# ArthurBrussee/brush

Measured on AMD Instinct MI355X. Metric: train views/sec @ 1M Gaussians, 1080p (fwd + L1/SSIM loss + bwd + Adam per view), higher is better.
Workload: dtype f32

## Files before the change

brush_amd/_ffi.py:

```python
import ctypes as C
import os

_DIR = os.path.dirname(os.path.abspath(__file__))
LIB_PATH = os.environ.get("BRUSH_HIP_LIB") or os.path.join(_DIR, "libbrush_hip.so")

FLAG_MIP = 1
FLAG_BWD_INFO = 2
FLAG_SMOOTH_CUTOFF = 4
FLAG_SLICED_LISTS = 8

fp = C.POINTER(C.c_float)
u32p = C.POINTER(C.c_uint32)


class BhCamera(C.Structure):
    _fields_ = [
        ("vm", C.c_float * 12),
        ("fx", C.c_float), ("fy", C.c_float), ("cx", C.c_float), ("cy", C.c_float),
        ("lim_pos_x", C.c_float), ("lim_pos_y", C.c_float),
        ("lim_neg_x", C.c_float), ("lim_neg_y", C.c_float),
        ("cam_pos", C.c_float * 3),
        ("img_w", C.c_uint32), ("img_h", C.c_uint32),
        ("tile_row_begin", C.c_uint32), ("tile_row_end", C.c_uint32),
        ("model", C.c_uint32), ("dist", C.c_float * 8), ("half_max_render_fov", C.c_float),
# ... 210 lines not shown
dp = C.POINTER(C.c_double)
POSE_SYMBOLS = {
    "bh_render_backward_pose_saved": (C.c_int, [C.c_void_p, C.POINTER(BhRenderOut)] + [C.c_void_p] * 9),
    "bh_train_set_pose_grad": (C.c_int, [C.c_void_p, C.c_void_p]),
    "bh_pose_twist": (C.c_int, [fp, fp, dp]),
    "bh_camera_apply_twist": (C.c_int, [C.POINTER(BhCamera), dp]),
}

EXPOSURE_SYMBOLS = {
    "bh_exposure_create": (C.c_int, [C.c_void_p, C.c_uint32, C.POINTER(C.c_void_p)]),
    "bh_exposure_destroy": (C.c_int, [C.c_void_p, C.c_void_p]),
    "bh_exposure_set_params": (C.c_int, [C.c_void_p, C.c_void_p, C.c_uint32, C.c_uint32, fp]),
    "bh_exposure_get_params": (C.c_int, [C.c_void_p, C.c_void_p, C.c_uint32, C.c_uint32, fp]),
    "bh_exposure_get_grad": (C.c_int, [C.c_void_p, C.c_void_p, C.c_uint32, C.c_uint32, fp]),
    "bh_exposure_get_state": (C.c_int, [C.c_void_p, C.c_void_p, C.c_uint32, dp, dp, u32p]),
    "bh_exposure_set_state": (C.c_int, [C.c_void_p, C.c_void_p, C.c_uint32, dp, dp, C.c_uint32]),
    "bh_exposure_set_adam": (C.c_int, [C.c_void_p, C.c_void_p, C.c_double, C.c_double, C.c_double, C.c_double]),
    "bh_exposure_apply": (C.c_int, [C.c_void_p, C.c_void_p, C.c_uint32, C.c_void_p, C.c_uint32, C.c_uint32, C.c_void_p]),
    "bh_exposure_backward": (C.c_int, [C.c_void_p, C.c_void_p, C.c_uint32, C.c_void_p, C.c_void_p, C.c_uint32, C.c_uint32, C.c_void_p, C.c_int]),
    "bh_train_set_exposure": (C.c_int, [C.c_void_p, C.c_void_p]),
}

DEPTH_LOSS_L1, DEPTH_LOSS_DISPARITY = 0, 1


class BhDepthTarget(C.Structure):
    _fields_ = [("gt", C.c_void_p), ("h", C.c_uint32), ("w", C.c_uint32), ("kind", C.c_uint32), ("weight", C.c_float),
                ("scale", C.c_float), ("offset", C.c_float)]


DEPTH_LOSS_SYMBOLS = {
    "bh_depth_loss_value_and_grad": (C.c_int, [C.c_void_p, C.c_void_p, C.POINTER(BhDepthTarget), C.c_void_p, C.c_void_p]),
    "bh_train_set_depth": (C.c_int, [C.c_void_p, C.POINTER(BhDepthTarget)]),
    "bh_eval_depth_metrics": (C.c_int, [C.c_void_p, C.c_void_p, C.POINTER(BhDepthTarget), C.c_void_p]),
}

NORMAL_ACCUMULATED, NORMAL_UNIT = 0, 1
NORMAL_SYMBOLS = {
    "bh_splat_normals": (C.c_int, [C.c_void_p, C.POINTER(BhCamera), C.c_void_p, C.c_uint64, C.c_void_p]),
    "bh_render_normal": (C.c_int, [C.c_void_p, C.POINTER(BhRenderOut), C.c_void_p, C.c_uint32, C.c_void_p]),
    "bh_render_backward_normal_saved": (C.c_int, [C.c_void_p, C.POINTER(BhRenderOut), C.c_void_p, C.c_void_p, C.c_uint32, C.c_void_p, C.c_uint32]
                                        + [C.c_void_p] * 7),
    "bh_depth_to_normal": (C.c_int, [C.c_void_p, C.POINTER(BhCamera), C.c_void_p, C.c_uint32, C.c_uint32, C.c_void_p]),
    "bh_depth_to_normal_backward": (C.c_int, [C.c_void_p, C.POINTER(BhCamera), C.c_void_p, C.c_void_p, C.c_uint32, C.c_uint32, C.c_void_p]),
}

class BhNormalTermConfig(C.Structure):
    _fields_ = [("weight", C.c_float), ("reserved", C.c_uint32 * 3)]


NORMAL_LOSS_SYMBOLS = {
    "bh_normal_consistency_value_and_grad": (C.c_int, [C.c_void_p, C.POINTER(BhCamera), C.c_void_p, C.c_void_p, C.c_void_p, C.c_uint32, C.c_uint32,
                                                       C.c_float, C.c_uint32, C.c_void_p, C.c_void_p, C.c_void_p]),
    "bh_train_set_normal": (C.c_int, [C.c_void_p, C.POINTER(BhNormalTermConfig)]),
}

DISTORTION_Z, DISTORTION_NDC = 0, 1


class BhDistortionConfig(C.Structure):
    _fields_ = [("kind", C.c_uint32), ("near_z", C.c_float), ("far_z", C.c_float), ("reserved", C.c_uint32)]


class BhDistortionTermConfig(C.Structure):
    _fields_ = [("weight", C.c_float), ("kind", C.c_uint32), ("near_z", C.c_float), ("far_z", C.c_float)]


DISTORTION_SYMBOLS = {
    "bh_render_distortion": (C.c_int, [C.c_void_p, C.POINTER(BhRenderOut), C.POINTER(BhDistortionConfig), C.c_void_p]),
    "bh_render_distortion_moments": (C.c_int, [C.c_void_p, C.POINTER(BhRenderOut), C.POINTER(BhDistortionConfig), C.c_void_p]),
    "bh_render_backward_distortion_saved": (C.c_int, [C.c_void_p, C.POINTER(BhRenderOut), C.c_void_p, C.c_void_p, C.c_uint32, C.c_void_p, C.c_uint32,
                                                      C.c_void_p, C.POINTER(BhDistortionConfig)] + [C.c_void_p] * 7),
    "bh_distortion_loss": (C.c_int, [C.c_void_p, C.c_void_p, C.c_uint32, C.c_uint32, C.c_uint32, C.c_float, C.c_void_p]),
    "bh_train_set_distortion": (C.c_int, [C.c_void_p, C.POINTER(BhDistortionTermConfig)]),
}

ABI_VERSION = 7
STRUCT_MIRRORS = (BhCamera, BhRenderOut, BhLossConfig, BhTrainConfig, BhTrainState, BhTrainBatch, BhTrainStats, BhRefineConfig, BhRefineStats, BhPlyInfo)

_lib = None
_lib_th = None
TEST_HOOKS_LIB_PATH = os.path.join(_DIR, "libbrush_hip_testhooks.so")
TEST_HOOK_SYMBOLS = {"bh_debug_fill_train_scratch": (C.c_int, [C.c_void_p, C.c_uint32]),
                     "bh_debug_split_counts": (C.c_int, [C.c_void_p, C.POINTER(C.c_uint32)])}


class BrushHipError(RuntimeError):
    pass


def _bind(path, symbols):
    if not os.path.exists(path):
        raise BrushHipError(
            "%s not found: build it with `python -c 'import __graft_entry__ as g; g.build()'` "
            "(hipcc --offload-arch=gfx950). There is no CPU fallback." % path)
    lib = C.CDLL(path)
    for name, (res, args) in symbols.items():
        fn = getattr(lib, name)
        fn.restype = res
        fn.argtypes = args
    if lib.bh_abi_version() != ABI_VERSION:
        raise BrushHipError("%s speaks ABI %d, this binding ABI %d" % (path, lib.bh_abi_version(), ABI_VERSION))
    for i, mirror in enumerate(STRUCT_MIRRORS):
        if lib.bh_struct_size(i) != C.sizeof(mirror):
            raise BrushHipError("%s: sizeof(%s) is %d in the library, %d in this binding" % (path, mirror.__name__, lib.bh_struct_size(i), C.sizeof(mirror)))
    return lib


def load():
    global _lib
    if _lib is None:
        _lib = _bind(LIB_PATH, dict(SYMBOLS, **LPIPS_SYMBOLS, **COMPRESSED_PLY_SYMBOLS, **IMAGE_SYMBOLS, **DEPTH_SYMBOLS, **POSE_SYMBOLS, **EXPOSURE_SYMBOLS, **DEPTH_LOSS_SYMBOLS, **NORMAL_SYMBOLS, **NORMAL_LOSS_SYMBOLS, **DISTORTION_SYMBOLS))
    return _lib


def load_test_hooks():
    global _lib_th
    if _lib_th is None:
        _lib_th = _bind(TEST_HOOKS_LIB_PATH, dict(SYMBOLS, **LPIPS_SYMBOLS, **COMPRESSED_PLY_SYMBOLS, **IMAGE_SYMBOLS, **DEPTH_SYMBOLS, **POSE_SYMBOLS, **EXPOSURE_SYMBOLS, **DEPTH_LOSS_SYMBOLS, **NORMAL_SYMBOLS, **NORMAL_LOSS_SYMBOLS, **DISTORTION_SYMBOLS,
                                                   **TEST_HOOK_SYMBOLS))
    return _lib_th
```

brush_amd/csrc/api.hip:

```cpp
#include <cmath>
#include <cstdlib>
#include <cstdio>
#include <algorithm>
#include <cstring>
#include <new>

#include "context.h"
#include "device_rng.h"

namespace bh {

int launch_image_loss_fused(bh_ctx* ctx, const float* img_hwc4, const uint32_t* gt, uint32_t h, uint32_t w, const BhLossConfig& cfg,
                            bool alpha_match, float dl_rgb, float dl_alpha, float* loss_out, float* v_output, float* loss_host = nullptr,
                            uint32_t* started_host = nullptr, uint32_t started_tag = 0);
int launch_image_loss_fused_window(bh_ctx* ctx, const float* img_hwc4, const uint32_t* gt, uint32_t h, uint32_t w, const BhLossConfig& cfg,
                                   bool alpha_match, float dl_rgb, float dl_alpha, uint32_t tile_y0, uint32_t tile_y1, float* loss_out,
                                   float* v_output, float* loss_host = nullptr, uint32_t* started_host = nullptr, uint32_t started_tag = 0);

__global__ __launch_bounds__(256) void zero_two_kernel(float4* __restrict__ a, size_t na, float4* __restrict__ b, size_t nb) {
    const size_t stride = (size_t)gridDim.x * 256;
    const float4 z = make_float4(0.0f, 0.0f, 0.0f, 0.0f);
    for (size_t i = (size_t)blockIdx.x * 256 + threadIdx.x; i < na + nb; i += stride) {
        if (i < na) a[i] = z;
        else b[i - na] = z;
    }
}

int set_error(bh_ctx* ctx, int code, const std::string& msg) {
    if (ctx) ctx->last_error = msg;
    return code;
}

int check_hip(bh_ctx* ctx, hipError_t e, const char* what) {
    if (e == hipSuccess) return 0;
    std::string m = std::string(what) + ": " + hipGetErrorString(e);
    (void)hipGetLastError();
    return set_error(ctx, e == hipErrorOutOfMemory ? BH_ERR_OOM : BH_ERR_HIP, m);
}

static inline void cpu_relax() {
#if defined(__x86_64__) || defined(__i386__)
    __builtin_ia32_pause();
#elif defined(__aarch64__)
    __asm__ __volatile__("yield");
#endif
}
int wait_host_tag(bh_ctx* ctx, const volatile uint32_t* word, uint32_t want, const char* what) {
    for (uint64_t it = 1; it < (1ull << 21); ++it) {
        if (*word == want) return 0;
        if ((it & 0x3FFFull) == 0ull) {
            const hipError_t q = hipStreamQuery(ctx->stream);
            if (q == hipSuccess) break;
            if (q != hipErrorNotReady) return check_hip(ctx, q, what);
        }
        cpu_relax();
    }
    if (*word == want) return 0;
    BH_HIP(ctx, hipEventRecord(ctx->readback_ev, ctx->stream));
    BH_HIP(ctx, hipEventSynchronize(ctx->readback_ev));
    if (*word == want) return 0;
    return set_error(ctx, BH_ERR_STATE, std::string(what) + ": the kernel that signals the host never stored its tag");
}

void* ensure(bh_ctx* ctx, Slot s, size_t bytes) {
    Buffer& b = ctx->slots[s];
    if (bytes == 0) bytes = 16;
    if (b.cap >= bytes) return b.ptr;
    if (b.ptr) {
        (void)hipStreamSynchronize(ctx->stream);
        (void)hipFree(b.ptr);
        b.ptr = nullptr;
        b.cap = 0;
    }
    {
        int best = -1;
        for (size_t i = 0; i < ctx->pool.size(); ++i)
            if (ctx->pool[i].cap >= bytes && ctx->pool[i].cap <= 2 * bytes + 4096 && (best < 0 || ctx->pool[i].cap < ctx->pool[(size_t)best].cap)) best = (int)i;
        if (best >= 0) {
            b = ctx->pool[(size_t)best];
            ctx->pool.erase(ctx->pool.begin() + best);
            return b.ptr;
        }
    }
    size_t cap = bytes + bytes / 4;
    cap = (cap + 255) & ~(size_t)255;
    void* p = nullptr;
    hipError_t e = hipMalloc(&p, cap);
    if (e != hipSuccess) {
        (void)hipGetLastError();
        cap = (bytes + 255) & ~(size_t)255;
        e = hipMalloc(&p, cap);
    }
    if (e != hipSuccess) {
        char msg[160];
        snprintf(msg, sizeof msg, "hipMalloc(%zu bytes) for scratch slot %d failed: %s", cap, (int)s, hipGetErrorString(e));
        (void)hipGetLastError();
        set_error(ctx, BH_ERR_OOM, msg);
        return nullptr;
    }
    b.ptr = p;
// ... 193 lines not shown
        BH_TRY(finish_far_slice(ctx, nullptr));
    }
    BH_HIP(ctx, hipStreamSynchronize(ctx->stream));
    deliver_pending_loss(ctx);
    return 0;
}

int bh_profile_enable(bh_ctx* ctx, int on) {
    if (!ctx) return BH_ERR_INVALID_ARG;
    ctx->prof.level = on < 0 ? 0 : (on > 2 ? 1 : on);
    return 0;
}

int bh_profile_fetch(bh_ctx* ctx, const char** names, float* ms, uint32_t* calls, int cap) {
    if (!ctx) return BH_ERR_INVALID_ARG;
    prof_resolve(ctx);
    Profiler& p = ctx->prof;
    const int n = p.count < cap ? p.count : cap;
    for (int i = 0; i < n; ++i) {
        names[i] = p.names[i];
        ms[i] = p.ms[i];
        calls[i] = p.calls[i];
    }
    p.count = 0;
    return n;
}

namespace {
bool parse_u32(const char* v, uint32_t lo, uint32_t hi, uint32_t* out) {
    if (!v || !*v) return false;
    char* end = nullptr;
    const unsigned long long x = strtoull(v, &end, 10);
    if (*end != '\0' || x < lo || x > hi) return false;
    *out = (uint32_t)x;
    return true;
}
bool parse_flag(const char* v, bool* out) {
    uint32_t x = 0;
    if (!parse_u32(v, 0, 1, &x)) return false;
    *out = x != 0;
    return true;
}
struct Option { const char* name; const char* help; bool (*apply)(bh_ctx* c, const char* v); };
const Option kOptions[] = {
    {"cut_min_pairs", "u32: a view whose last frame had fewer pairs keeps complete lists (= bh_set_list_cut_threshold)",
     [](bh_ctx* c, const char* v) { return parse_u32(v, 0, 0xFFFFFFFFu, &c->cut_min_pairs); }},
    {"cut_margin_pct", "0..10000: base margin behind a tile's last useful splat, % of its depth rank (default 150)",
     [](bh_ctx* c, const char* v) { return parse_u32(v, 0, 10000, &c->knob_cut_margin_pct); }},
    {"cut_margin_fixed", "0|1: the margin is cut_margin_pct for every frame instead of adaptive",
     [](bh_ctx* c, const char* v) { return parse_flag(v, &c->knob_fixed_margin); }},
    {"cut_ctrl", "up:down:floor:gap_exp — the margin controller's constants (default 1.5:0.998:0.5:0.3333)", [](bh_ctx* c, const char* v) {
        float a = 0, b = 0, d = 0, e = 0;
        if (sscanf(v, "%f:%f:%f:%f", &a, &b, &d, &e) != 4 || !(a >= 1.0f && b > 0.0f && b <= 1.0f && d > 0.0f && e >= 0.0f && e <= 1.0f)) return false;
        c->ctrl_up = a; c->ctrl_down = b; c->ctrl_floor = d; c->ctrl_gap_exp = e;
        return true;
    }},
    {"cut_sort_all", "0|1: with per-tile cuts, still depth-sort every visible splat",
     [](bh_ctx* c, const char* v) { return parse_flag(v, &c->knob_cut_sort_all); }},
    {"auto_exact_share", "0..1: a view whose last cut frame listed more than this share of its pairs renders complete lists (default 0.9; 0 = never)", [](bh_ctx* c, const char* v) {
        char* end = nullptr;
        const float x = strtof(v, &end);
        if (end == v || *end != '\0' || !(x >= 0.0f && x <= 1.0f)) return false;
        c->auto_exact_share = x;
        return true;
    }},
    {"no_view_hash", "0|1: frames without a view id share ONE table instead of being keyed by their camera",
     [](bh_ctx* c, const char* v) { return parse_flag(v, &c->knob_no_view_hash); }},
    {"k16_order", "0 index order | 1 by the view's last per-tile work | 2 dealt: the forward blend's tile order",
     [](bh_ctx* c, const char* v) { return parse_u32(v, 0, 2, &c->knob_k16_order); }},
    {"band_mode", "0|1: XCD bands of the blend kernels — contiguous eighths of the tile range, or dealt in chunks of 8 adjacent tiles (default 1)",
     [](bh_ctx* c, const char* v) { return parse_u32(v, 0, 1, &c->knob_band_mode); }},
    {"k16_waves", "0..8: forward blend: resident one-wave tiles per SIMD (0 = 8 = all resident at once; fewer: the lighter tiles are dispatched as the heavier ones finish)",
     [](bh_ctx* c, const char* v) { return parse_u32(v, 0, 8, &c->knob_k16_waves); }},
    {"k16_split", "0..1000: forward blend: a tile whose forecast work is at least max(256, k16_split / 100 x its band's mean) is blended by four quadrant waves (default 250; 0: no tile is split)",
     [](bh_ctx* c, const char* v) { return parse_u32(v, 0, 1000, &c->knob_k16_split); }},
    {"k16_split_of_max", "0..100: ... and at least this many percent of its band's heaviest tile (default 45)",
     [](bh_ctx* c, const char* v) { return parse_u32(v, 0, 100, &c->knob_k16_split_of_max); }},
    {"k16_split_min", "1..1023: a tile below this many blended splats (forecast) is never split (default 256)",
     [](bh_ctx* c, const char* v) { return parse_u32(v, 1, 1023, &c->knob_k16_split_min); }},
    {"k5_exact_spw", "16|32|64: splats per wave of the list builder for complete lists",
     [](bh_ctx* c, const char* v) { uint32_t u = 0; if (!parse_u32(v, 16, 64, &u) || !(u == 16 || u == 32 || u == 64)) return false; c->knob_k5_exact_spw = u; return true; }},
    {"bwd_jobs", "0|1: the blend backward works on checkpointed 128-entry segments of the tiles' lists (default 1) or on whole tiles",
     [](bh_ctx* c, const char* v) { return parse_flag(v, &c->knob_bwd_jobs); }},
    {"bwd_wide_rows", "0|1: the blend backward addresses the gradient accumulator in 64 bits, as it does by itself from 2^32 bytes of accumulator on (default 0)",
     [](bh_ctx* c, const char* v) { return parse_flag(v, &c->knob_bwd_wide_rows); }},
    {"no_lpt", "0|1: the blend backward takes its tiles in index order",
     [](bh_ctx* c, const char* v) { return parse_flag(v, &c->knob_no_lpt); }},
    {"lpt_classes", "log|linear: work classes of the backward's longest-first tile order — two per octave of blended splats, or 1/64 of the mean list length wide",
     [](bh_ctx* c, const char* v) { const std::string w(v); if (w == "log") { c->knob_lpt_linear = false; return true; } if (w == "linear") { c->knob_lpt_linear = true; return true; } return false; }},
    {"generic_depth_sort", "0|1: depth order by the generic radix sort + scan instead of the fused split sort",
     [](bh_ctx* c, const char* v) { return parse_flag(v, &c->knob_generic_depth_sort); }},
    {"dsort_splitters", "0|1: the fused depth sort splits at the 254 depth quantiles of the view's previous frame (default 1) or always linearly over the frame's key range",
     [](bh_ctx* c, const char* v) { return parse_flag(v, &c->knob_dsort_splitters); }},
    {"tile_sort", "auto|bucket|lsd: the forward's tile sort (auto: bucket sort unless the view's pairs are concentrated in few tiles)",
     [](bh_ctx* c, const char* v) { const std::string w(v); if (w == "auto") { c->knob_tile_sort = 0; return true; } if (w == "bucket") { c->knob_tile_sort = 1; return true; } if (w == "lsd") { c->knob_tile_sort = 2; return true; } return false; }},
    {"spec_k5", "0|1: queue the list builder before the host has read the frame's counts (default 1; 0: behind the count readback)",
     [](bh_ctx* c, const char* v) { return parse_flag(v, &c->knob_spec_k5); }},
    {"event_waits", "0|1: the host's mid-step waits use events behind the kernels instead of polled tag words",
     [](bh_ctx* c, const char* v) { return parse_flag(v, &c->knob_event_waits); }},
    {"readback_copy", "0|1: counts and gate word reach the host through copy launches",
     [](bh_ctx* c, const char* v) { return parse_flag(v, &c->knob_readback_copy); }},
    {"force_exchange", "0|1: a one-rank communicator still walks the whole gradient-exchange path (overhead measurement)",
     [](bh_ctx* c, const char* v) { return parse_flag(v, &c->knob_force_exchange); }},
    {"zero_grads", "0|1: the single-GPU train step zero-fills its gradient span like the exchange path",
     [](bh_ctx* c, const char* v) { return parse_flag(v, &c->knob_zero_grads); }},
    {"loss_bands", "0|1: the fused loss's blocks take their tiles by XCD column bands (1) or row-major (0)",
     [](bh_ctx* c, const char* v) { return parse_u32(v, 0, 1, &c->knob_loss_bands); }},
    {"update_rows", "0|64|128|256: splats per block of the update kernel (0 = default)",
     [](bh_ctx* c, const char* v) { uint32_t u = 0; if (!parse_u32(v, 0, 256, &u) || !(u == 0 || u == 64 || u == 128 || u == 256)) return false; c->knob_update_rows = u; return true; }},
    {"no_dormant", "0|1: the update kernel fetches and updates dormant splats like everyone else",
     [](bh_ctx* c, const char* v) { return parse_flag(v, &c->knob_no_dormant); }},
    {"sort_kpt", "0|4|8|16: keys per thread of the generic radix sort (0 = default)",
     [](bh_ctx* c, const char* v) { uint32_t u = 0; if (!parse_u32(v, 0, 16, &u) || !(u == 0 || u == 4 || u == 8 || u == 16)) return false; c->knob_sort_kpt = u; return true; }},
    {"grad_allreduce", "ring|direct: the dense gradient block's collective — ncclAllReduce, or reduce-scatter + all-gather over grouped send/recv",
     [](bh_ctx* c, const char* v) { const std::string w(v); if (w == "ring") { c->knob_direct_allreduce = false; return true; } if (w == "direct") { c->knob_direct_allreduce = true; return true; } return false; }},
    {"update_sparse", "0..256: an update block with at most this many non-dormant rows fetches them in one round trip (0: never; 256: every block that may skip dormant rows; default 64 at SH degree 0, else 0)",
     [](bh_ctx* c, const char* v) { uint32_t u = 0; if (!parse_u32(v, 0, 256, &u)) return false; c->knob_update_sparse = (int)u; return true; }},
};
constexpr int kOptionCount = (int)(sizeof(kOptions) / sizeof(kOptions[0]));
}

extern "C" int bh_option_count(void) { return kOptionCount; }
extern "C" const char* bh_option_name(int i) { return i >= 0 && i < kOptionCount ? kOptions[i].name : nullptr; }
extern "C" const char* bh_option_help(int i) { return i >= 0 && i < kOptionCount ? kOptions[i].help : nullptr; }

extern "C" int bh_set_option(bh_ctx* ctx, const char* key, const char* value) {
    if (!ctx) return BH_ERR_INVALID_ARG;
    if (!key || !value) return set_error(ctx, BH_ERR_INVALID_ARG, "set_option: null key or value");
    const std::string k(key);
    for (const Option& o : kOptions) {
        if (k != o.name) continue;
        if (!o.apply(ctx, value)) return set_error(ctx, BH_ERR_INVALID_ARG, "set_option: bad value '" + std::string(value) + "' for '" + k + "'");
        return 0;
    }
    return set_error(ctx, BH_ERR_INVALID_ARG, "set_option: unknown key '" + k + "' (bh_option_name lists the keys)");
}

namespace {
struct Kb4Law {
    double k[4];
    explicit Kb4Law(const float* d) { for (int i = 0; i < 4; ++i) k[i] = d ? (double)d[i] : 0.0; }
    double value(double th) const {
        const double t2 = th * th, t3 = t2 * th, t5 = t3 * t2, t7 = t5 * t2, t9 = t7 * t2;
        return th + k[0] * t3 + k[1] * t5 + k[2] * t7 + k[3] * t9;
    }
    double slope(double th) const {
        const double t2 = th * th, t4 = t2 * t2, t6 = t4 * t2, t8 = t6 * t2;
        return 1.0 + 3.0 * k[0] * t2 + 5.0 * k[1] * t4 + 7.0 * k[2] * t6 + 9.0 * k[3] * t8;
    }
    double invert(double target) const {
        if (target <= 0.0) return 0.0;
        const double pi = 3.14159265358979323846;
        double th = target < pi - 1e-6 ? target : pi - 1e-6;
        for (int it = 0; it < 50; ++it) {
            const double fp = slope(th);
            if (std::fabs(fp) < 1e-12) break;
            double next = th - (value(th) - target) / fp;
            next = next < 0.0 ? 0.0 : (next > pi ? pi : next);
            const bool done = std::fabs(next - th) < 1e-12;
            th = next;
            if (done) break;
        }
        return th;
    }
};
struct Rt8Law {
// ... 258 lines not shown
            BH_HIP(ctx, hipMemcpyAsync(hslots, counters, counter_read_bytes, hipMemcpyDeviceToHost, ctx->stream));
            BH_HIP(ctx, hipEventRecord(ctx->readback_ev, ctx->stream));
        }
        {
            ProfScope ps(ctx, "DepthSort");
            if (fused_scan) {
                cum_early = (uint32_t*)ensure(ctx, SLOT_CUM_TILES_HIT, npad * 4);
                if (!cum_early) return BH_ERR_OOM;
                if (poll_tag && ++ctx->readback_tag == 0u) ctx->readback_tag = 1u;
                bool* spl_written = nullptr;
                uint32_t* spl = view_splitters(view, cut_active, &spl_written);
                BH_TRY(depth_sort_scan(ctx, depth_keys, counters + COUNTER_MINMAX_WORD, cut_active ? near_counts : isect_counts, n, depths_sorted, f.gfc, cum_early,
                                       sums_on_device ? counters : nullptr, ctx->host_counters + 16, ctx->readback_ev, poll_tag ? ctx->readback_tag : 0u,
                                       sums_on_device ? dev_sums : nullptr, spl, spl_written));
            } else {
                BH_TRY(radix_argsort(ctx, depth_keys, nullptr, n, 32, depths_sorted, f.gfc));
            }
        }
        if (poll_tag && ctx->knob_spec_k5 && !(want_sliced && ctx->slice_fraction > 0.0f)) {
            const size_t cap_pairs = std::min(ctx->slots[SLOT_TILE_IDS].cap, ctx->slots[SLOT_ISECT_GIDS].cap) / 4;
            if (cap_pairs >= 4096) {
                spec_projected = (float*)ensure(ctx, SLOT_PROJECTED, npad * 9 * 4);
                spec_vc = f.bwd_info ? (float4*)ensure(ctx, SLOT_V_COMBINED, npad * 10 * 4 + 16) : nullptr;
                if (!spec_projected || (f.bwd_info && !spec_vc)) return BH_ERR_OOM;
                spec_tile_ids = (uint32_t*)ctx->slots[SLOT_TILE_IDS].ptr;
                spec_isect_gids = (uint32_t*)ctx->slots[SLOT_ISECT_GIDS].ptr;
                spec_pair_cap = (uint32_t)std::min<size_t>(cap_pairs, 0xFFFFFFFEull);
                ProfScope ps(ctx, "MapGaussiansToIntersect");
                BH_TRY(launch_map_gaussians(ctx, n, f.u, f.proj_by_gid, f.gfc, spec_projected, cum_early, spec_tile_ids, spec_isect_gids, spec_vc,
                                            spec_vc ? (uint32_t)(((size_t)n * 10 + 3) / 4) : 0u, 0xFFFFFFFFu, cut_active ? slice_tab : nullptr,
                                            cut_active ? vtab : nullptr, cut_active ? depths_sorted : nullptr, dev_sums + (cut_active ? 3 : 0), spec_pair_cap));
                k5_queued = true;
            }
        }
        if (poll_tag) BH_TRY(wait_host_tag(ctx, reinterpret_cast<const volatile uint32_t*>(hslots) + HOST_SUM_WORDS - 1u, ctx->readback_tag, "count readback"));
        else BH_HIP(ctx, hipEventSynchronize(ctx->readback_ev));
        if (ctx->gate_learn) {
            ctx->gate_learn = false;
            ctx->far_direct = reinterpret_cast<const volatile uint32_t*>(ctx->host_counters)[HOST_GATE_WORD] != 0u;
        }
        unsigned long long hc[4] = {0ull, 0ull, 0ull, 0ull};
        if (sums_on_device) {
            const volatile unsigned long long* hs = hslots;
            for (uint32_t c = 0; c < COUNTER_K1_U64; ++c) hc[c] = hs[c];
        } else {
            for (uint32_t k = 0; k < COUNTER_SLOTS; ++k)
                for (uint32_t c = 0; c < COUNTER_K1_U64; ++c) hc[c] += hslots[COUNTER_K1_U64 * k + c];
        }
        if (hc[1] > 0xFFFFFFFFull) return set_error(ctx, BH_ERR_UNSUPPORTED, "more than 2^32-1 tile intersections");
        nv_true = (uint32_t)hc[0];
        f.ni = (uint32_t)hc[1];
        near_total = cut_active ? (uint32_t)hc[2] : f.ni;
        f.nv = cut_active ? (uint32_t)hc[3] : nv_true;
    } else {
        BH_HIP(ctx, hipMemsetAsync(tile_offsets, 0, ((size_t)f.num_tiles * 2 + LPT_HEADER_WORDS) * 4, ctx->stream));
        if (visible_words) BH_HIP(ctx, hipMemsetAsync(f.visible, 0, visible_words * 4, ctx->stream));
    }

    const size_t nvpad = f.nv ? f.nv : 1, nipad = f.ni ? f.ni : 1;
    f.cum = fused_scan ? cum_early : (uint32_t*)ensure(ctx, SLOT_CUM_TILES_HIT, nvpad * 4);
    f.projected = (float*)ensure(ctx, SLOT_PROJECTED, nvpad * 9 * 4);
    f.tile_ids = (uint32_t*)ensure(ctx, SLOT_TILE_IDS, nipad * 4);
    f.isect_gids = (uint32_t*)ensure(ctx, SLOT_ISECT_GIDS, nipad * 4);
    f.tile_ids_sorted = (uint32_t*)ensure(ctx, SLOT_TILE_IDS_SORTED, nipad * 4);
    f.isect_gids_sorted = (uint32_t*)ensure(ctx, SLOT_ISECT_GIDS_SORTED, nipad * 4);
    const size_t pixels = (size_t)f.u.img_w * f.u.img_h;
    void* out_img = ensure(ctx, SLOT_OUT_IMG, pixels * (f.bwd_info ? 16 : 4));
    if (!f.cum || !f.projected || !f.tile_ids || !f.isect_gids || !f.tile_ids_sorted || !f.isect_gids_sorted || !out_img)
        return BH_ERR_OOM;
    if (k5_queued && ((cut_active ? near_total : f.ni) > spec_pair_cap || f.projected != spec_projected || f.tile_ids != spec_tile_ids || f.isect_gids != spec_isect_gids))
        k5_queued = false;

    f.budget = want_sliced && f.ni > 0 ? list_budget(ctx, cut_active ? view : nullptr, near_total, f.ni) : f.ni;
    const bool sliced = f.budget < f.ni;
    const bool by_cut = cut_active && sliced;
    const uint32_t* zcut_lists = cut_active ? vtab : nullptr;
    f.slice_info = slice_tab;
    f.done_bits = slice_tab ? slice_tab + SLICE_CTRL_WORDS : nullptr;
    f.tile_offsets_far = slice_tab ? slice_tab + SLICE_CTRL_WORDS + slice_bit_words : nullptr;
    f.far_group_totals = slice_tab ? slice_tab + SLICE_CTRL_WORDS + slice_bit_words + (size_t)f.num_tiles * 2 : nullptr;
    while (f.tile_bits < 32 && (f.num_tiles >> f.tile_bits) != 0) f.tile_bits++;
    if (bwd_jobs) {
        const uint32_t listed = cut_active ? near_total : f.ni;
        const uint32_t ckpt_cap = (uint32_t)std::min<uint64_t>((uint64_t)listed / BWD_SEG + f.num_tiles + 1u, BWD_CKPT_MAX_SLOTS);
        f.rs.jobs.ckpt = (float4*)ensure(ctx, SLOT_BWD_CKPT, (size_t)ckpt_cap * 256 * sizeof(float4));
        f.rs.jobs.ckpt_cap = ckpt_cap;
        f.rs.jobs.top_cap = band_slots(f.num_tiles) + ckpt_cap;
        f.rs.jobs.top_list = (uint32_t*)ensure(ctx, SLOT_BWD_TOPLIST, (size_t)8 * f.rs.jobs.top_cap * 4);
        if (!f.rs.jobs.ckpt || !f.rs.jobs.top_list) return BH_ERR_OOM;
    }
    if (view) {
        f.rs.zcut = vtab;
        f.rs.depth_keys_sorted = depths_sorted;
        f.rs.nv = f.nv;
        f.rs.cut_active = by_cut;
        f.rs.margin_pct = cut_margin_pct(ctx, view);
        f.rs.work = vtab + (size_t)f.num_tiles;
        f.rs.order = tile_order;
        f.rs.order_mode = ctx->knob_k16_order;
        f.rs.split = tile_split;
#ifdef BH_TEST_HOOKS
        ctx->last_split = tile_split;
#endif
    }
    const uint32_t win_tiles = f.u.tile_bw * (f.u.tile_y1 - f.u.tile_y0);
    const float class_width_raw = (float)f.ni / (float)(win_tiles ? win_tiles : 1u) / 64.0f;
    f.class_width = ctx->knob_lpt_linear ? (class_width_raw < 8.0f ? 8.0f : class_width_raw) : 0.0f;
    f.lpt = (f.bwd_info && !ctx->knob_no_lpt) ? tile_offsets + (size_t)f.num_tiles * 2 : nullptr;
    f.out_f32 = f.bwd_info ? (float*)out_img : nullptr;
    f.out_u8 = f.bwd_info ? nullptr : (uint32_t*)out_img;

    bool offsets_done = false;
    if (f.nv > 0) {
        if (!fused_scan) {
            ProfScope ps(ctx, "PrefixSumGaussHits");
            BH_TRY(prefix_sum(ctx, cut_active ? near_counts : isect_counts, f.gfc, f.nv, f.cum, false));
        }
        if (f.ni == 0) {
            ProfScope ps(ctx, "ProjectVisible");
            BH_TRY(launch_project_visible(ctx, f.nv, f.proj_by_gid, f.gfc, f.projected));
        }
        if (f.ni > 0) {
            {
                ProfScope ps(ctx, "MapGaussiansToIntersect");
                float4* vc = nullptr;
                if (f.bwd_info) {
                    vc = (float4*)ensure(ctx, SLOT_V_COMBINED, (size_t)f.nv * 10 * 4 + 16);
                    if (!vc) return BH_ERR_OOM;
                }
                if (zcut_lists && near_total == 0u) {
                } else if (k5_queued && (!f.bwd_info || vc == spec_vc)) {
                    ctx->clears.k5_cleared_accum(vc != nullptr);
                } else {
                    ctx->clears.k5_cleared_accum(vc != nullptr);
                    BH_TRY(launch_map_gaussians(ctx, f.nv, f.u, f.proj_by_gid, f.gfc, f.projected, f.cum, f.tile_ids, f.isect_gids, vc, vc ? (uint32_t)(((size_t)f.nv * 10 + 3) / 4) : 0u,
                                                (sliced && !by_cut) ? f.budget : 0xFFFFFFFFu, (sliced || zcut_lists) ? f.slice_info : nullptr, zcut_lists,
                                                zcut_lists ? depths_sorted : nullptr));
                }
            }
            {
                ProfScope ps(ctx, "TileSort");
                if ((zcut_lists || !sliced) && tile_sort_supported(f.tile_bits, zcut_lists ? near_total : f.ni) && !(ctx->knob_tile_sort == 2u)) {
                    BH_TRY(tile_sort_offsets(ctx, f.tile_ids, f.isect_gids, zcut_lists ? near_total : f.ni, f.tile_bits, f.num_tiles, f.tile_ids_sorted, f.isect_gids_sorted,
                                             tile_offsets, f.ni));
                    offsets_done = true;
                } else
                if (zcut_lists) BH_TRY(radix_argsort_dev(ctx, f.tile_ids, f.isect_gids, near_total, nullptr, nullptr, nullptr, f.tile_bits, f.tile_ids_sorted, f.isect_gids_sorted, f.ni));
                else if (sliced) BH_TRY(radix_argsort_dev(ctx, f.tile_ids, f.isect_gids, f.budget, f.slice_info + 1, nullptr, nullptr, f.tile_bits, f.tile_ids_sorted, f.isect_gids_sorted, f.ni));
                else BH_TRY(radix_argsort(ctx, f.tile_ids, f.isect_gids, f.ni, f.tile_bits, f.tile_ids_sorted, f.isect_gids_sorted));
            }
        }
    }
    if (!offsets_done) {
        ProfScope ps(ctx, "GetTileOffsets");
        if (zcut_lists) BH_TRY(launch_tile_offsets(ctx, f.tile_ids_sorted, near_total, f.num_tiles, tile_offsets, true));
        else if (sliced) BH_TRY(launch_tile_offsets_dev(ctx, f.tile_ids_sorted, f.budget, f.slice_info + 1, nullptr, nullptr, f.num_tiles, tile_offsets));
        else BH_TRY(launch_tile_offsets(ctx, f.tile_ids_sorted, f.ni, f.num_tiles, tile_offsets, true));
    }
    if (!sliced) {
        ProfScope ps(ctx, "Rasterize");
        BH_TRY(launch_rasterize(ctx, f.u, f.bg, f.bwd_info, f.smooth, f.isect_gids_sorted, tile_offsets, f.projected, f.gfc, f.out_f32, f.out_u8, f.visible, f.lpt,
                                f.class_width, 0, &f.rs));
    } else {
        auto* state = (float*)ensure(ctx, SLOT_SLICE_STATE, pixels * 16);
        f.far_counts = (uint32_t*)ensure(ctx, SLOT_SLICE_COUNTS, nvpad * 4);
        f.far_block_totals = (uint32_t*)ensure(ctx, SLOT_SLICE_CUM, (nvpad / 256 + 2) * 4);
        if (!state || !f.far_counts || !f.far_block_totals) return BH_ERR_OOM;
        f.rs.done_bits = f.done_bits;
        f.rs.unsat_count = f.slice_info + 2;
        if (!ctx->knob_readback_copy) {
            f.rs.gate_host = ctx->host_counters + HOST_GATE_WORD;
            *reinterpret_cast<volatile uint32_t*>(f.rs.gate_host) = 0u;
        }
        f.rs.state = state;
        f.rs.offsets_near = tile_offsets;
        f.rs.live_bands = f.slice_info + 4;
        {
            ProfScope ps(ctx, "Rasterize");
            BH_TRY(launch_rasterize(ctx, f.u, f.bg, f.bwd_info, f.smooth, f.isect_gids_sorted, tile_offsets, f.projected, f.gfc, f.out_f32, f.out_u8, f.visible, f.lpt,
                                    f.class_width, 1, &f.rs));
        }
        FarJob& j = ctx->far_job;
        j.frame = f;
        j.by_cut = by_cut;
        j.view = by_cut ? view : nullptr;
        j.view_shared = req.view_id == 0u && ctx->knob_no_view_hash;
        if (by_cut) j.req = req;
        if (ctx->knob_readback_copy)
            BH_HIP(ctx, hipMemcpyAsync(ctx->host_counters + HOST_GATE_WORD, f.slice_info + 2, 4, hipMemcpyDeviceToHost, ctx->stream));
        if (ctx->far_direct && !by_cut) {
            BH_TRY(enqueue_far_slice(ctx, j));
            ctx->gate_learn = true;
        } else {
            if (++ctx->gate_tag == 0u) ctx->gate_tag = 1u;
            j.gate_tag = ctx->gate_tag;
            ctx->gate_signal_queued = false;
            j.gate_event_recorded = !(req.defer_decision && !ctx->knob_event_waits && !ctx->knob_readback_copy);
            if (j.gate_event_recorded) BH_HIP(ctx, hipEventRecord(ctx->gate_ev, ctx->stream));
            j.pending = true;
            if (!req.defer_decision) {
                bool again = false;
                BH_TRY(finish_far_slice(ctx, &again));
                if (by_cut && again) {
                    *out = ctx->latest.out;
                    return 0;
                }
            }
        }
    }

    BhRenderOut r{};
    r.num_visible = nv_true;
    r.num_listed_splats = f.nv;
    r.num_intersections = f.ni;
    r.num_tiles = f.num_tiles;
    r.tile_bw = f.u.tile_bw;
    r.tile_bh = f.u.tile_bh;
    r.flags = flags;
    r.out_img = f.bwd_info ? (float*)out_img : nullptr;
    r.out_img_packed = f.bwd_info ? nullptr : (uint32_t*)out_img;
    r.visible = f.bwd_info ? f.visible : nullptr;
    r.max_radius = max_radius;
    r.tile_offsets = tile_offsets;
    r.projected = f.projected;
    r.compact_gid_from_isect = f.isect_gids_sorted;
    r.tile_id_from_isect = f.tile_ids_sorted;
    r.global_from_compact_gid = f.gfc;
    r.cum_tiles_hit = f.cum;
    r.intersect_counts = isect_counts;
    r.depths_sorted = (float*)depths_sorted;
    r.tile_offsets_far = sliced ? f.tile_offsets_far : nullptr;
    r.list_budget = f.budget;
    r.generation = ++ctx->generation;
    ctx->clears.stamp(r.generation);
    *out = r;
    ForwardState& latest = ctx->latest;
    latest.out = r;
    latest.uniforms = f.u;
    latest.n = n; latest.sh_degree = sh_degree; latest.flags = flags;
    latest.bg[0] = f.bg[0]; latest.bg[1] = f.bg[1]; latest.bg[2] = f.bg[2];
    latest.lpt = f.lpt;
    latest.jobs = f.rs.jobs;
    ctx->have_forward = true;
    if (view) view_rendered(view, f.ni);
    return 0;
}

extern "C" {

int bh_set_list_slicing(bh_ctx* ctx, float near_share) {
    if (!ctx) return BH_ERR_INVALID_ARG;
    if (near_share != near_share || near_share > 1.0f) return set_error(ctx, BH_ERR_INVALID_ARG, "set_list_slicing: the near slice's share must be <= 1 (<= 0: automatic)");
    ctx->slice_fraction = near_share > 0.0f ? near_share : 0.0f;
    return 0;
}

int bh_set_list_cut_threshold(bh_ctx* ctx, uint32_t min_pairs) {
    if (!ctx) return BH_ERR_INVALID_ARG;
    ctx->cut_min_pairs = min_pairs;
    return 0;
}

int bh_set_view_id(bh_ctx* ctx, uint32_t view_id) {
    if (!ctx) return BH_ERR_INVALID_ARG;
    ctx->view_id = view_id;
    return 0;
}

int bh_forget_views(bh_ctx* ctx) {
    if (!ctx) return BH_ERR_INVALID_ARG;
    BH_HIP(ctx, hipSetDevice(ctx->device));
    if (ctx->far_job.pending) BH_TRY(finish_far_slice(ctx, nullptr));
    if (ctx->dsort_spl) { BH_HIP(ctx, hipMemsetAsync(ctx->dsort_spl, 0, DSORT_SPL_STRIDE * 4, ctx->stream)); ctx->dsort_spl_written = false; }
    if (ctx->views.empty()) return 0;
    BH_HIP(ctx, hipStreamSynchronize(ctx->stream));
    deliver_pending_loss(ctx);
    for (auto& kv : ctx->views)
        if (kv.second.zcut) (void)hipFree(kv.second.zcut);
    ctx->views.clear();
    ctx->casual_views = 0;
    for (uint64_t& k : ctx->seen_keys) k = 0ull;
    ctx->far_job.view = nullptr;
    ctx->margin_scale = 1.0f;
    return 0;
}

float bh_last_list_share(bh_ctx* ctx) { return ctx ? ctx->last_slice_share : 0.0f; }
uint32_t bh_far_slices_queued(bh_ctx* ctx) { return ctx ? ctx->far_launches : 0u; }
uint32_t bh_view_table_count(bh_ctx* ctx) { return ctx ? (uint32_t)ctx->views.size() : 0u; }

}

namespace bh {

int backward_impl(bh_ctx* ctx, const ForwardState& fs, const float* v_output, const float* transforms, const float* sh_coeffs,
                  const float* raw_opacities, float* v_transforms, float* v_sh_coeffs, float* v_raw_opacities, float* v_refine_weight,
                  size_t span_floats, bool want_refine, const DepthTerm* depth, float* v_viewmat, const NormalTerm* normal,
                  const DistortionTerm* distortion) {
    const BhRenderOut& r = fs.out;
    const uint32_t n = fs.n, nv = r.num_listed_splats, C = (fs.sh_degree + 1) * (fs.sh_degree + 1);
    const size_t nvpad = nv ? nv : 1;
    auto* v_combined = (float*)ensure(ctx, SLOT_V_COMBINED, nvpad * 10 * 4 + 16);
    if (!v_combined) return BH_ERR_OOM;
    bool row_marks = false;
    const float* scatter_v_z = nullptr;
    {
        ProfScope ps(ctx, "ZeroGradBuffers");
        const bool one_span = n > 0 && span_floats;
        const bool vc_done = ctx->clears.take_accum(r.generation);
        const GradClears::Span span = ctx->clears.take_span(r.generation);
        row_marks = span == GradClears::ROW_MARKS;
        if (row_marks && !one_span) return set_error(ctx, BH_ERR_STATE, "internal: row-marked gradients without the train step's gradient span");
        const bool span_done = one_span && span != GradClears::NONE;
        if (one_span && (span_floats & 3u) == 0 && (reinterpret_cast<uintptr_t>(v_transforms) & 15u) == 0) {
            const size_t na = vc_done ? 0 : (nvpad * 10 + 3) / 4, nb = span_done ? 0 : span_floats / 4;
            if (na + nb) {
                hipLaunchKernelGGL(zero_two_kernel, dim3(2048), dim3(256), 0, ctx->stream, reinterpret_cast<float4*>(v_combined), na,
                                   reinterpret_cast<float4*>(v_transforms), nb);
                BH_LAUNCH_CHECK(ctx, "zero_two_kernel");
            }
        } else {
            if (!vc_done) BH_HIP(ctx, hipMemsetAsync(v_combined, 0, nvpad * 10 * 4, ctx->stream));
            if (n > 0) {
                if (one_span) {
                    BH_HIP(ctx, hipMemsetAsync(v_transforms, 0, span_floats * 4, ctx->stream));
                } else {
                    BH_HIP(ctx, hipMemsetAsync(v_transforms, 0, (size_t)n * 10 * 4, ctx->stream));
                    BH_HIP(ctx, hipMemsetAsync(v_sh_coeffs, 0, (size_t)n * C * 3 * 4, ctx->stream));
                    BH_HIP(ctx, hipMemsetAsync(v_raw_opacities, 0, (size_t)n * 4, ctx->stream));
                    BH_HIP(ctx, hipMemsetAsync(v_refine_weight, 0, (size_t)n * 4, ctx->stream));
                }
            }
        }
    }
    {
        ProfScope ps(ctx, "RasterizeBackwards", true);
        if (r.num_intersections > 0 && v_output)
            BH_TRY(launch_rasterize_backward(ctx, fs.uniforms, fs.bg, fs.flags & BH_FLAG_SMOOTH_CUTOFF,
                                             r.compact_gid_from_isect, r.tile_offsets, r.projected, r.out_img, v_output, v_combined, fs.lpt,
                                             r.tile_offsets_far, want_refine, &fs.jobs, nv));
        if (depth) BH_TRY(launch_depth_backward(ctx, fs, *depth, v_combined));
        if (normal) BH_TRY(launch_normal_backward(ctx, fs, *normal, transforms, v_combined));
        if (distortion) BH_TRY(launch_distortion_backward(ctx, fs, *distortion, v_combined, depth ? (float*)ctx->slots[SLOT_DEPTH].ptr : nullptr, &scatter_v_z));
    }
    {
        ProfScope ps(ctx, "ProjectBackwards");
        BH_TRY(launch_project_backward(ctx, fs.uniforms, nv, fs.flags & BH_FLAG_MIP, fs.sh_degree, transforms, sh_coeffs,
                                       raw_opacities, r.global_from_compact_gid, v_combined, v_transforms, v_sh_coeffs,
                                       v_raw_opacities, v_refine_weight, row_marks, r.projected));
        if (depth || distortion) BH_TRY(launch_depth_vz_scatter(ctx, fs, v_transforms, row_marks, v_sh_coeffs, v_raw_opacities, v_refine_weight, scatter_v_z));
        if (normal) BH_TRY(launch_normal_vn_scatter(ctx, fs, transforms, v_transforms, row_marks, v_sh_coeffs, v_raw_opacities, v_refine_weight));
    }
    if (v_viewmat) {
        ProfScope ps(ctx, "PoseGrad");
        BH_TRY(launch_pose_grad(ctx, fs.uniforms, nv, fs.flags & BH_FLAG_MIP, fs.sh_degree, transforms, sh_coeffs, r.global_from_compact_gid,
                                v_combined, v_viewmat));
    }
    return 0;
}

int find_saved_bwd_forward(bh_ctx* ctx, const BhRenderOut* saved, int not_bwd_code, const char* who, const ForwardState** fs) {
    if (!(saved->flags & BH_FLAG_BWD_INFO)) return set_error(ctx, not_bwd_code, std::string(who) + ": the saved forward was not a BH_FLAG_BWD_INFO forward");
    BH_HIP(ctx, hipSetDevice(ctx->device));
    if (ctx->far_job.pending) BH_TRY(finish_far_slice(ctx, nullptr));
    for (const Retained& rt : ctx->retained)
        if (rt.fs.out.generation == saved->generation && rt.fs.out.out_img == saved->out_img) { *fs = &rt.fs; return 0; }
    if (ctx->have_forward && saved->generation == ctx->latest.out.generation && saved->out_img == ctx->latest.out.out_img) { *fs = &ctx->latest; return 0; }
    char msg[288];
    snprintf(msg, sizeof msg, "%s: forward #%llu is stale (the context's buffers now hold forward #%llu); call bh_render_retain "
                              "on a forward that must outlive the next one", who, (unsigned long long)saved->generation, (unsigned long long)ctx->generation);
    return set_error(ctx, BH_ERR_STATE, msg);
}

static const Slot kRetainSlots[RETAIN_SLOTS] = {SLOT_OUT_IMG, SLOT_VISIBLE, SLOT_MAX_RADIUS, SLOT_TILE_OFFSETS, SLOT_PROJECTED, SLOT_ISECT_GIDS_SORTED,
                                                SLOT_TILE_IDS_SORTED, SLOT_GLOBAL_FROM_COMPACT, SLOT_CUM_TILES_HIT, SLOT_ISECT_COUNTS, SLOT_DEPTHS_SORTED,
                                                SLOT_SLICE, SLOT_BWD_CKPT, SLOT_BWD_TOPLIST};

}

extern "C" {

int bh_render_backward(bh_ctx* ctx, const float* v_output, const float* transforms, const float* sh_coeffs,
                       const float* raw_opacities, float* v_transforms, float* v_sh_coeffs, float* v_raw_opacities,
                       float* v_refine_weight) {
    if (!ctx) return BH_ERR_INVALID_ARG;
    if (!ctx->have_forward || !(ctx->latest.flags & BH_FLAG_BWD_INFO))
        return set_error(ctx, BH_ERR_STATE, "render_backward needs a preceding BH_FLAG_BWD_INFO forward on this context");
    if (!v_output || !v_transforms || !v_sh_coeffs || !v_raw_opacities || !v_refine_weight)
        return set_error(ctx, BH_ERR_INVALID_ARG, "render_backward: null argument");
    BH_HIP(ctx, hipSetDevice(ctx->device));
    if (ctx->far_job.pending) BH_TRY(finish_far_slice(ctx, nullptr));
    return backward_impl(ctx, ctx->latest, v_output, transforms, sh_coeffs, raw_opacities, v_transforms, v_sh_coeffs, v_raw_opacities,
                         v_refine_weight, 0, true);
}

int bh_render_backward_saved(bh_ctx* ctx, const BhRenderOut* saved, const float* v_output, const float* transforms, const float* sh_coeffs,
                             const float* raw_opacities, float* v_transforms, float* v_sh_coeffs, float* v_raw_opacities,
                             float* v_refine_weight) {
    if (!ctx) return BH_ERR_INVALID_ARG;
    if (!saved || !v_output || !v_transforms || !v_sh_coeffs || !v_raw_opacities || !v_refine_weight)
        return set_error(ctx, BH_ERR_INVALID_ARG, "render_backward_saved: null argument");
    const ForwardState* fs = nullptr;
    BH_TRY(find_saved_bwd_forward(ctx, saved, BH_ERR_STATE, "render_backward_saved", &fs));
    return backward_impl(ctx, *fs, v_output, transforms, sh_coeffs, raw_opacities, v_transforms, v_sh_coeffs, v_raw_opacities, v_refine_weight,
                         0, true);
}

int bh_render_retain(bh_ctx* ctx, const BhRenderOut* out) {
    if (!ctx || !out) return BH_ERR_INVALID_ARG;
    BH_HIP(ctx, hipSetDevice(ctx->device));
    if (ctx->far_job.pending) BH_TRY(finish_far_slice(ctx, nullptr));
    if (!ctx->have_forward || out->generation != ctx->latest.out.generation || out->out_img != ctx->latest.out.out_img || out->out_img_packed != ctx->latest.out.out_img_packed)
        return set_error(ctx, BH_ERR_STATE, "render_retain: only the context's most recent forward can be retained (and only once)");
    Retained rt;
    rt.fs = ctx->latest;
    for (int i = 0; i < RETAIN_SLOTS; ++i) {
        rt.blocks[i] = ctx->slots[kRetainSlots[i]];
        ctx->slots[kRetainSlots[i]] = Buffer{};
    }
    ctx->retained.push_back(rt);
    ctx->have_forward = false;
    ctx->latest.lpt = nullptr;
    return 0;
// ... 103 lines not shown
    BH_HIP(ctx, hipSetDevice(ctx->device));
    return launch_gather_stats(ctx, refine_weight_norm, vis_weight, max_screen_size, refine_weight, visible, screen_radius, n);
}

void bh_philox4x32_10(const uint32_t ctr[4], const uint32_t key[2], uint32_t out[4]) {
    const Philox4 r = philox4x32_10(ctr[0], ctr[1], ctr[2], ctr[3], key[0], key[1]);
    out[0] = r.x; out[1] = r.y; out[2] = r.z; out[3] = r.w;
}

void bh_sample_background(uint64_t seed, uint32_t step, const float base[3], float strength, float out[3]) {
    float u[3] = {0.5f, 0.5f, 0.5f};
    if (strength > 0.0f) {
        const Philox4 r = philox4x32_10(0u, step, 0u, RNG_STREAM_BACKGROUND, (uint32_t)seed, (uint32_t)(seed >> 32));
        u[0] = unit_open(r.x); u[1] = unit_open(r.y); u[2] = unit_open(r.z);
    }
    for (int k = 0; k < 3; ++k) {
        const float v = strength > 0.0f ? base[k] + (2.0f * u[k] - 1.0f) * strength : base[k];
        out[k] = v < 0.0f ? 0.0f : (v > 1.0f ? 1.0f : v);
    }
}

int bh_normal_samples(bh_ctx* ctx, uint64_t seed, uint32_t step, uint64_t n, float* out) {
    if (!ctx) return BH_ERR_INVALID_ARG;
    if (n > 0 && !out) return set_error(ctx, BH_ERR_INVALID_ARG, "normal_samples: null argument");
    if (n > 0xFFFFFFFFull) return set_error(ctx, BH_ERR_INVALID_ARG, "normal_samples: n must fit 32 bits (the splat index is one counter word)");
    BH_HIP(ctx, hipSetDevice(ctx->device));
    return launch_normal_samples(ctx, out, n, seed, step);
}

int bh_fold_min_scale(bh_ctx* ctx, const float* transforms, const float* raw_opacities, const float* min_scale, uint32_t n,
                      float* out_transforms, float* out_raw_opacities) {
    if (!ctx) return BH_ERR_INVALID_ARG;
    if (n > 0 && (!transforms || !raw_opacities || !min_scale || !out_transforms || !out_raw_opacities))
        return set_error(ctx, BH_ERR_INVALID_ARG, "fold_min_scale: null argument");
    BH_HIP(ctx, hipSetDevice(ctx->device));
    return launch_fold_min_scale(ctx, transforms, raw_opacities, min_scale, n, out_transforms, out_raw_opacities);
}

int bh_fold_min_scale_backward(bh_ctx* ctx, const float* transforms, const float* raw_opacities, const float* min_scale, uint32_t n,
                               float* v_transforms, float* v_raw_opacities) {
    if (!ctx) return BH_ERR_INVALID_ARG;
    if (n > 0 && (!transforms || !raw_opacities || !min_scale || !v_transforms || !v_raw_opacities))
        return set_error(ctx, BH_ERR_INVALID_ARG, "fold_min_scale_backward: null argument");
    BH_HIP(ctx, hipSetDevice(ctx->device));
    return launch_fold_min_scale_backward(ctx, transforms, raw_opacities, min_scale, n, v_transforms, v_raw_opacities);
}

int bh_compute_min_scale(bh_ctx* ctx, const float* transforms, uint32_t n, const float* view_cams, uint32_t num_views, float factor,
                         float* out) {
    if (!ctx) return BH_ERR_INVALID_ARG;
    if (!(factor > 0.0f) || num_views == 0) return set_error(ctx, BH_ERR_INVALID_ARG, "compute_min_scale: needs factor > 0 and at least one view camera");
    if (!view_cams || (n > 0 && (!transforms || !out))) return set_error(ctx, BH_ERR_INVALID_ARG, "compute_min_scale: null argument");
    BH_HIP(ctx, hipSetDevice(ctx->device));
    return launch_compute_min_scale(ctx, transforms, n, view_cams, num_views, factor, out);
}

}

extern "C" int bh_tile_sort_offsets(bh_ctx* ctx, const uint32_t* tile_ids, const uint32_t* compact_gids, uint32_t n, uint32_t num_tiles,
                                    uint32_t* tile_ids_sorted, uint32_t* compact_gids_sorted, uint32_t* tile_offsets) {
    if (!ctx) return BH_ERR_INVALID_ARG;
    if (!tile_offsets || (n > 0 && (!tile_ids || !compact_gids || !tile_ids_sorted || !compact_gids_sorted)))
        return set_error(ctx, BH_ERR_INVALID_ARG, "tile_sort_offsets: null argument");
    if (num_tiles == 0) return set_error(ctx, BH_ERR_INVALID_ARG, "tile_sort_offsets: num_tiles == 0");
    BH_HIP(ctx, hipSetDevice(ctx->device));
    uint32_t bits = 0;
    while (bits < 32 && (num_tiles >> bits) != 0) bits++;
    BH_HIP(ctx, hipMemsetAsync(tile_offsets, 0, (size_t)num_tiles * 2 * 4, ctx->stream));
    if (n == 0) return 0;
    if (tile_sort_supported(bits, n) && !(ctx->knob_tile_sort == 2u))
        return tile_sort_offsets(ctx, tile_ids, compact_gids, n, bits, num_tiles, tile_ids_sorted, compact_gids_sorted, tile_offsets);
    BH_TRY(radix_argsort(ctx, tile_ids, compact_gids, n, bits, tile_ids_sorted, compact_gids_sorted));
    return launch_tile_offsets(ctx, tile_ids_sorted, n, num_tiles, tile_offsets, true);
}

#ifdef BH_TEST_HOOKS
extern "C" int bh_debug_split_counts(bh_ctx* ctx, uint32_t* out) {
    if (!ctx || !out) return BH_ERR_INVALID_ARG;
    if (!ctx->last_split) return 0;
    BH_HIP(ctx, hipSetDevice(ctx->device));
    BH_HIP(ctx, hipMemcpyAsync(out, ctx->last_split, 8 * 4, hipMemcpyDeviceToHost, ctx->stream));
    BH_HIP(ctx, hipStreamSynchronize(ctx->stream));
    return 1;
}
extern "C" int bh_debug_fill_train_scratch(bh_ctx* ctx, uint32_t pattern) {
    if (!ctx) return BH_ERR_INVALID_ARG;
    const Buffer& s = ctx->slots[SLOT_GRADS];
    if (!s.ptr || s.cap < 4) return set_error(ctx, BH_ERR_STATE, "debug_fill_train_scratch: no train step on this context yet");
    BH_HIP(ctx, hipSetDevice(ctx->device));
    BH_HIP(ctx, hipMemsetD32Async(reinterpret_cast<hipDeviceptr_t>(s.ptr), (int)pattern, s.cap / 4, ctx->stream));
    return 0;
}
#endif

static int train_step_impl(bh_ctx* ctx, const BhTrainConfig* cfg, BhTrainState* st, const BhTrainBatch* batch,
                           bh_grad_hook hook, void* hook_user, float grad_scale, BhTrainStats* stats);

extern "C" int bh_train_step(bh_ctx* ctx, const BhTrainConfig* cfg, BhTrainState* st, const BhTrainBatch* batch,
                             bh_grad_hook hook, void* hook_user, float grad_scale, BhTrainStats* stats) {
    if (!ctx) return BH_ERR_INVALID_ARG;
    const int rc = train_step_impl(ctx, cfg, st, batch, hook, hook_user, grad_scale, stats);
    if (rc != 0) {
        drop_far_job(ctx);
        ctx->have_forward = false;
        ctx->clears.begin_forward();
    }
    return rc;
}

static int train_step_impl(bh_ctx* ctx, const BhTrainConfig* cfg, BhTrainState* st, const BhTrainBatch* batch,
                           bh_grad_hook hook, void* hook_user, float grad_scale, BhTrainStats* stats) {
    if (!cfg || !st || !batch || !stats) return set_error(ctx, BH_ERR_INVALID_ARG, "train_step: null argument");
    if (!st->transforms || !st->sh_coeffs || !st->raw_opacities || !st->m1_transforms || !st->m2_transforms || !st->m1_sh ||
        !st->m2_sh || !st->m1_opac || !st->m2_opac || !st->refine_weight_norm || !st->vis_weight || !st->max_screen_size ||
        !batch->gt_packed)
        return set_error(ctx, BH_ERR_INVALID_ARG, "train_step: null state tensor");
    bh_exposure* const exposure = ctx->exposure;
    if (exposure) {
        if (batch->view_id == 0u || batch->view_id > exposure_views(exposure))
            return set_error(ctx, BH_ERR_INVALID_ARG, "train_step: with an exposure table the batch's view_id must be 1 .. n_views");
        const ViewUniforms eu = make_uniforms(batch->camera);
        if (batch->image_hook || eu.tile_y0 != 0u || eu.tile_y1 != eu.tile_bh)
            return set_error(ctx, BH_ERR_INVALID_ARG, "train_step: the exposure term needs the whole frame on this rank (no tile-row partition)");
    }
    const BhDepthTarget* const depth_target = (ctx->depth_attached && ctx->depth_target.weight > 0.0f) ? &ctx->depth_target : nullptr;
    if (depth_target) {
        if (!depth_target->gt) return set_error(ctx, BH_ERR_INVALID_ARG, "train_step: the depth target has no depth map");
        if (depth_target->h != batch->camera.img_h || depth_target->w != batch->camera.img_w)
            return set_error(ctx, BH_ERR_INVALID_ARG, "train_step: the depth target's size differs from the camera's");
        if (depth_target->kind > BH_DEPTH_LOSS_DISPARITY) return set_error(ctx, BH_ERR_INVALID_ARG, "train_step: unknown depth loss kind");
        const ViewUniforms du = make_uniforms(batch->camera);
        if (batch->image_hook || du.tile_y0 != 0u || du.tile_y1 != du.tile_bh)
            return set_error(ctx, BH_ERR_INVALID_ARG, "train_step: the depth term needs the whole frame on this rank (no tile-row partition)");
        if (ctx->pose_grad)
            return set_error(ctx, BH_ERR_INVALID_ARG, "train_step: a depth target and a pose-gradient buffer cannot be attached together (the pose pass does not carry the depth term's gradient)");
    }
    const bool normal_wanted = ctx->normal_attached && ctx->normal_term.weight > 0.0f;
    if (normal_wanted) {
        if (batch->camera.model != BH_CAMERA_PINHOLE)
            return set_error(ctx, BH_ERR_INVALID_ARG, "train_step: the normal term needs a pinhole camera (the normals of a depth map are defined for it alone)");
        const ViewUniforms nu = make_uniforms(batch->camera);
        if (batch->image_hook || nu.tile_y0 != 0u || nu.tile_y1 != nu.tile_bh)
            return set_error(ctx, BH_ERR_INVALID_ARG, "train_step: the normal term needs the whole frame on this rank (no tile-row partition)");
        if (ctx->pose_grad)
            return set_error(ctx, BH_ERR_INVALID_ARG, "train_step: a normal term and a pose-gradient buffer cannot be attached together (the pose pass does not carry the normal term's gradient)");
    }
    const bool distortion_wanted = ctx->distortion_attached;
    if (distortion_wanted) {
        const ViewUniforms xu = make_uniforms(batch->camera);
        if (batch->image_hook || xu.tile_y0 != 0u || xu.tile_y1 != xu.tile_bh)
            return set_error(ctx, BH_ERR_INVALID_ARG, "train_step: the distortion term needs the whole frame on this rank (no tile-row partition)");
        if (ctx->pose_grad)
            return set_error(ctx, BH_ERR_INVALID_ARG, "train_step: a distortion term and a pose-gradient buffer cannot be attached together (the pose pass does not carry the distortion term's gradient)");
    }
    BH_HIP(ctx, hipSetDevice(ctx->device));
    const uint32_t n = st->n, C = (st->sh_degree + 1) * (st->sh_degree + 1);
    const uint32_t W = batch->camera.img_w, H = batch->camera.img_h;
    const uint32_t step = st->step_count + 1;

    auto pad4 = [](size_t x) { return (x + 3) & ~(size_t)3; };
    const size_t o_tr = pad4(n), o_sh = o_tr + pad4((size_t)n * 10), o_op = o_sh + pad4((size_t)n * 3 * C), o_ref = o_op + pad4(n);
    const size_t exch_count = o_ref + pad4(n);
    auto* exch = (float*)ensure(ctx, SLOT_GRADS, (exch_count ? exch_count : 4) * 4);
    auto* s_radius = (float*)ensure(ctx, SLOT_STATS, (size_t)(n ? n : 1) * 4);
    if (!exch || !s_radius) return BH_ERR_OOM;
    float* s_visible = exch;
    float* s_refine = exch + o_ref;

    const float* r_transforms = st->transforms;
    const float* r_raw_opac = st->raw_opacities;
    if (st->min_scale && n > 0) {
        ProfScope ps(ctx, "FoldMinScale");
        auto* ft = (float*)ensure(ctx, SLOT_FOLDED_TRANSFORMS, (size_t)n * 10 * 4);
        auto* fo = (float*)ensure(ctx, SLOT_FOLDED_RAW_OPAC, (size_t)n * 4);
        if (!ft || !fo) return BH_ERR_OOM;
        BH_TRY(launch_fold_min_scale(ctx, st->transforms, st->raw_opacities, st->min_scale, n, ft, fo));
        r_transforms = ft;
        r_raw_opac = fo;
    }

    BhRenderOut ro;
    ForwardRequest fwd;
    fwd.cam = batch->camera;
    fwd.n = n; fwd.sh_degree = st->sh_degree;
    fwd.flags = BH_FLAG_BWD_INFO | (cfg->render_mip ? BH_FLAG_MIP : 0) | (cfg->exact_lists ? 0 : BH_FLAG_SLICED_LISTS);
    fwd.transforms = r_transforms; fwd.sh_coeffs = st->sh_coeffs; fwd.raw_opacities = r_raw_opac;
    fwd.bg[0] = batch->background[0]; fwd.bg[1] = batch->background[1]; fwd.bg[2] = batch->background[2];
    fwd.view_id = batch->view_id;
    fwd.visible = s_visible;
    fwd.visible_floats = o_tr;
    fwd.max_radius = s_radius;
    fwd.grad_begin = exch + o_tr;
    fwd.grad_floats = exch_count - o_tr;
    const bool exchanging = hook || (ctx->comm && (ctx->comm_world > 1 || ctx->knob_force_exchange));
    const ViewUniforms win_u = make_uniforms(batch->camera);
    const bool window_partial = win_u.tile_y0 != 0u || win_u.tile_y1 != win_u.tile_bh;
    const bool native_tiles = !batch->image_hook && window_partial && ctx->comm != nullptr && !hook && (batch->strip_loss || ctx->comm_world > 1);
    if (native_tiles && !batch->strip_loss)
        return set_error(ctx, BH_ERR_INVALID_ARG, "train_step: a tile-row window without an image hook needs strip_loss = 1 (the library exchanges the strips' halos, not whole frames)");
    const bool tile_mode = batch->image_hook != nullptr || native_tiles;
    const bool lpips_on = ctx->lpips != nullptr && ctx->lpips_weight > 0.0f;
    if (lpips_on && (tile_mode || window_partial))
        return set_error(ctx, BH_ERR_INVALID_ARG, "train_step: the LPIPS term needs the whole frame on this rank (no tile-row partition)");
    const bool masked_grads = !exchanging && !tile_mode && !ctx->knob_zero_grads && n > 0;
    if (masked_grads) {
        fwd.grad_begin = exch + o_ref;
        fwd.grad_floats = exch_count - o_ref;
    }
    fwd.defer_decision = !tile_mode;
    BH_TRY(render_forward(ctx, fwd, &ro));

    if (tile_mode) {
        ProfScope ps(ctx, "ImageExchange");
        const ViewUniforms& wu = win_u;
        const uint32_t r0 = wu.tile_y0 * TILE_WIDTH, r1 = wu.tile_y1 * TILE_WIDTH < H ? wu.tile_y1 * TILE_WIDTH : H;
        if (native_tiles) BH_TRY(comm_exchange_strip_halos(ctx, ro.out_img, H, W, r0, r1));
        else if (batch->image_hook(batch->image_hook_user, ro.out_img, H, W, r0, r1) != 0) return set_error(ctx, BH_ERR_STATE, "image hook failed");
    }

    const bool ssim_on = cfg->ssim_weight > 0.0f;
    BhLossConfig lc{};
    lc.l1_weight = ssim_on ? 1.0f - cfg->ssim_weight : 1.0f;
    lc.ssim_weight = ssim_on ? -cfg->ssim_weight : 0.0f;
    const bool bg_nonzero = batch->background[0] != 0.0f || batch->background[1] != 0.0f || batch->background[2] != 0.0f;
    lc.composite_bg = (batch->has_alpha && bg_nonzero) ? 1 : 0;
    lc.bg[0] = batch->background[0]; lc.bg[1] = batch->background[1]; lc.bg[2] = batch->background[2];
    lc.mask = batch->alpha_is_mask ? 1 : 0;
    const bool alpha_match = batch->has_alpha && !batch->alpha_is_mask && cfg->match_alpha_weight > 0.0f;
    const size_t hw = (size_t)W * H;
    auto* v_output = (float*)ensure(ctx, SLOT_V_OUTPUT, hw * 16);
    auto* loss_dev = (float*)ensure(ctx, SLOT_LOSS_SCALAR, 16);
    if (!v_output || !loss_dev) return BH_ERR_OOM;
    float* exposed = nullptr;
    if (exposure && !(exposed = (float*)ensure(ctx, SLOT_EXPOSED, hw * 16))) return BH_ERR_OOM;
    float* loss_host = reinterpret_cast<float*>(ctx->host_counters) + HOST_LOSS_WORD;
    const float dl_rgb = 1.0f / (float)(hw * 3);
    const float dl_alpha = alpha_match ? cfg->match_alpha_weight / (float)hw : 0.0f;
    auto queue_loss = [&]() -> int {
        uint32_t* started_host = nullptr;
        uint32_t started_tag = 0u;
        if (ctx->far_job.pending && !ctx->far_job.gate_event_recorded && !ctx->gate_signal_queued) {
            started_host = ctx->host_counters + HOST_GATE_TAG_WORD;
            started_tag = ctx->far_job.gate_tag;
            ctx->gate_signal_queued = true;
        }
        if (tile_mode && batch->strip_loss) {
            const ViewUniforms wu = make_uniforms(batch->camera);
            return launch_image_loss_fused_window(ctx, ro.out_img, batch->gt_packed, H, W, lc, alpha_match, dl_rgb, dl_alpha, wu.tile_y0, wu.tile_y1,
                                                  loss_dev, v_output, loss_host, started_host, started_tag);
        }
        if (exposed) {
            ProfScope ps(ctx, "Exposure");
            BH_TRY(launch_exposure_apply(ctx, exposure, batch->view_id, ro.out_img, H, W, exposed));
        }
        return launch_image_loss_fused(ctx, exposed ? exposed : ro.out_img, batch->gt_packed, H, W, lc, alpha_match, dl_rgb, dl_alpha, loss_dev, v_output, loss_host, started_host,
                                       started_tag);
    };
#ifdef BH_TEST_HOOKS
    if (ctx->knob_fail_loss_at && ++ctx->train_steps_seen == ctx->knob_fail_loss_at)
        return set_error(ctx, BH_ERR_OOM, "train_step: injected failure between the forward and the loss (BH_TEST_FAIL_LOSS_AT)");
#endif
    if (far_job_decides_first(ctx)) {
        BH_TRY(finish_far_slice(ctx, nullptr));
        ro = ctx->latest.out;
    }
    BH_TRY(queue_loss());
    if (ctx->far_job.pending) {
        bool far_ran = false;
        BH_TRY(finish_far_slice(ctx, &far_ran));
        if (far_ran) {
            ro = ctx->latest.out;
            BH_TRY(queue_loss());
        }
    }
    if (lpips_on) BH_TRY(lpips_train_term(ctx, exposed ? exposed : ro.out_img, batch->gt_packed, H, W, lc.composite_bg ? lc.bg : nullptr, v_output, loss_dev, loss_host));
    if (exposed) {
        ProfScope ps(ctx, "Exposure");
        BH_TRY(launch_exposure_backward(ctx, exposure, batch->view_id, ro.out_img, v_output, H, W, v_output, true));
    }

    DepthTerm depth_term;
    NormalTerm normal_term;
    const bool frame_listed = ctx->latest.out.num_intersections > 0 && n > 0;
    const bool depth_on = depth_target != nullptr && frame_listed;
    const bool normal_on = normal_wanted && frame_listed;
    if (depth_on || normal_on) {
        ProfScope ps(ctx, "DepthTerm");
        auto* e_map = (float*)ensure(ctx, SLOT_DEPTH_TERM, (hw * 2 + 4) * 4);
        if (!e_map) return BH_ERR_OOM;
        float* v_depth = e_map + hw;
        BH_TRY(launch_depth_forward(ctx, ctx->latest, BH_DEPTH_EXPECTED, e_map));
        if (depth_on) BH_TRY(launch_depth_loss(ctx, e_map, *depth_target, v_depth + hw, v_depth, loss_dev, loss_host));
        depth_term.v_depth = v_depth;
        depth_term.mode = BH_DEPTH_EXPECTED;
        if (normal_on) {
            ProfScope pn(ctx, "NormalTerm");
            auto* n_map = (float*)ensure(ctx, SLOT_NORMAL_TERM, (hw * 6 + 4) * 4);
            if (!n_map) return BH_ERR_OOM;
            float* v_normal = n_map + hw * 3;
            BH_TRY(launch_normal_map(ctx, ctx->latest, r_transforms, BH_NORMAL_ACCUMULATED, n_map));
            BH_TRY(launch_normal_loss(ctx, batch->camera, n_map, e_map, ctx->latest.out.out_img, H, W, ctx->normal_term.weight, depth_on,
                                      v_normal + hw * 3, v_normal, v_depth, loss_dev, loss_host));
            normal_term.v_normal = v_normal;
            normal_term.mode = BH_NORMAL_ACCUMULATED;
        }
    }
    DistortionTerm distortion_term;
    const bool distortion_on = distortion_wanted && frame_listed && ctx->latest.out.num_listed_splats > 0;
    if (distortion_on) {
        ProfScope pd(ctx, "DistortionTerm");
        auto* moments = (float*)ensure(ctx, SLOT_DISTORTION_TERM, (hw * 4 + 4) * 4);
        if (!moments) return BH_ERR_OOM;
        const BhDistortionTermConfig& dc = ctx->distortion_term;
        distortion_term.kind = dc.kind;
        distortion_term.near_z = dc.near_z;
        distortion_term.far_z = dc.far_z;
        distortion_term.gain = (float)((double)dc.weight / (double)hw);
        BH_TRY(launch_distortion_map(ctx, ctx->latest, distortion_term, true, moments));
        BH_TRY(launch_distortion_loss(ctx, moments, H, W, 4u, dc.weight, moments + hw * 4, loss_dev, loss_host));
        distortion_term.moments = moments;
    }

    auto sum_over_ranks = [&](float* p, uint64_t cnt) -> int {
        if (hook) return hook(hook_user, p, cnt) == 0 ? 0 : set_error(ctx, BH_ERR_STATE, "gradient hook failed");
        return comm_allreduce(ctx, p, cnt, false);
    };
    const bool keyed = exchanging && batch->exchange_mode == 1 && n > 0;
    uint32_t* union_idx = nullptr;
    float* compact = nullptr;
    bool flags_on_side = false;
    if (keyed) {
        ProfScope ps(ctx, "FlagExchange");
        const uint32_t nblk = (n + 4095u) / 4096u;
        auto* blocks = (uint32_t*)ensure(ctx, SLOT_EXCH_BLOCKS, ((size_t)nblk + 2) * 4);
        union_idx = (uint32_t*)ensure(ctx, SLOT_EXCH_IDX, (size_t)n * 4);
        if (!blocks || !union_idx) return BH_ERR_OOM;
        flags_on_side = !hook && ctx->comm_stream != nullptr;
        hipStream_t main_stream = ctx->stream;
        if (flags_on_side) {
// ... 94 lines not shown
```

brush_amd/csrc/context.h:

```cpp
#pragma once
#include <hip/hip_runtime.h>
#include <stdint.h>

#include <memory>
#include <string>
#include <unordered_map>
#include <vector>

#include "../../include/brush_hip.h"
#include "../../include/brush_hip_lpips.h"
#include "../../include/brush_hip_image.h"
#include "../../include/brush_hip_exposure.h"
#include "../../include/brush_hip_depth_loss.h"
#include "../../include/brush_hip_normal_loss.h"
#include "../../include/brush_hip_distortion.h"
#include "device_math.h"

namespace bh {

enum Slot : int {
    SLOT_COUNTERS = 0,
    SLOT_DEPTH_KEYS,
    SLOT_ISECT_COUNTS,
    SLOT_MAX_RADIUS,
// ... 38 lines not shown
    SLOT_SLICE_STATE,
    SLOT_SLICE_COUNTS,
    SLOT_SLICE_CUM,
    SLOT_NEAR_COUNTS,
    SLOT_TILE_ORDER,
    SLOT_LOD_GRADS,
    SLOT_LOD_FOLDED,
    SLOT_LOD_LOSS,
    SLOT_LOD_SORT,
    SLOT_KNN,
    SLOT_EVAL,
    SLOT_LPIPS,
    SLOT_PLY_COMPRESS,
    SLOT_IMAGE,
    SLOT_DEPTH,
    SLOT_POSE,
    SLOT_EXPOSURE,
    SLOT_EXPOSED,
    SLOT_DEPTH_LOSS,
    SLOT_DEPTH_TERM,
    SLOT_NORMAL,
    SLOT_NORMAL_LOSS,
    SLOT_NORMAL_TERM,
    SLOT_DISTORTION,
    SLOT_DISTORTION_LOSS,
    SLOT_DISTORTION_TERM,
    SLOT_COUNT
};

struct Buffer {
    void* ptr = nullptr;
    size_t cap = 0;
};

constexpr int MAX_PROF = 32;

constexpr uint32_t COUNTER_SLOTS = 128;
constexpr uint32_t COUNTER_K1_U64 = 4;
constexpr size_t COUNTER_SET_BYTES = COUNTER_SLOTS * 8 * COUNTER_K1_U64 + COUNTER_SLOTS * 8;
constexpr uint32_t COUNTER_SET_U64 = (uint32_t)(COUNTER_SET_BYTES / 8);
constexpr uint32_t COUNTER_MINMAX_WORD = COUNTER_SLOTS * 2 * COUNTER_K1_U64;
constexpr uint32_t SLICE_CTRL_WORDS = 8;
constexpr uint32_t SORT_GROUP_BLOCKS = 32;
constexpr uint32_t FAR_GROUP_BLOCKS = 64;
constexpr size_t COUNTER_READ_BYTES = COUNTER_SLOTS * 8 * COUNTER_K1_U64;
constexpr uint32_t HOST_SUM_WORDS = 2 * COUNTER_K1_U64 + 1;
constexpr size_t HOST_LOSS_WORD = 16 + COUNTER_READ_BYTES / 4;
constexpr size_t HOST_GATE_WORD = HOST_LOSS_WORD + 16;
constexpr size_t HOST_GATE_TAG_WORD = HOST_GATE_WORD + 1;
constexpr size_t HOST_COUNTERS_BYTES = 64 + COUNTER_READ_BYTES + 64 + 64;

struct Profiler {
    int level = 0;
    const char* names[MAX_PROF];
    float ms[MAX_PROF];
    uint32_t calls[MAX_PROF];
    int count = 0;
    struct Pending { int idx; hipEvent_t a, b; };
    std::vector<Pending> pending;
    std::vector<hipEvent_t> pool;
    hipEvent_t ext_a = nullptr, ext_b = nullptr;
};

constexpr uint32_t ZCUT_ALL = 0xFFFFFFFEu;
BH_DEV bool zcut_near(uint32_t key, uint32_t cut) { return (key >> 1) <= (cut >> 1); }
struct ViewState {
    uint32_t* zcut = nullptr;
    uint32_t tile_bw = 0, tile_bh = 0;
    bool seeded = false;
    uint32_t exact_frames = 0;
    uint32_t penalty = 0;
    uint64_t last_used = 0;
    uint32_t gap = 0;
    uint32_t last_pairs = 0;
    uint32_t complete_frames = 0;
    bool spl_written[2] = {false, false};
    bool casual = false;
};
constexpr uint32_t CUT_MIN_PAIRS = 1500000u;
constexpr uint32_t LPT_CLASSES = 64;
constexpr uint32_t LPT_HEADER_WORDS = 8 * LPT_CLASSES + 64;
constexpr uint32_t BWD_SEG = 128;
constexpr uint32_t BWD_MAX_SEGS = 64;
struct BwdJobs {
    float4* ckpt = nullptr;
    uint32_t ckpt_cap = 0;
    uint32_t* top_list = nullptr;
    uint32_t top_cap = 0;
};
constexpr uint32_t BAND_CHUNK = 4;
inline __host__ __device__ uint32_t band_slots(uint32_t num_tiles) {
    const uint32_t p = (num_tiles + 7u) / 8u;
    return ((p + BAND_CHUNK - 1u) / BAND_CHUNK) * BAND_CHUNK;
}
inline __host__ __device__ uint32_t band_tile(uint32_t band, uint32_t i, uint32_t per, uint32_t mode) {
    return mode ? ((i / BAND_CHUNK) * 8u + band) * BAND_CHUNK + (i % BAND_CHUNK) : band * per + i;
}
BH_DEV uint32_t tile_of_block(uint32_t b, uint32_t num_tiles, uint32_t band_mode) {
    const uint32_t per = band_slots(num_tiles);
    const uint32_t i = b >> 3;
    return i < per ? band_tile(b & 7u, i, per, band_mode) : 0xFFFFFFFFu;
}
constexpr uint32_t SPLIT_MAX = 128;
constexpr uint32_t SPLIT_MIN_WORK = 256;
constexpr uint32_t SPLIT_TAIL_WORDS = 8u + 8u * SPLIT_MAX * 4u;
constexpr uint32_t BWD_CKPT_MAX_SLOTS = 96u * 1024u;
constexpr uint32_t DSORT_SPL_STRIDE = 260;
constexpr uint32_t VIEW_SPL_WORDS = 2 * DSORT_SPL_STRIDE;
constexpr size_t MAX_VIEW_STATES = 4096;
constexpr uint64_t DIRECT_ALLREDUCE_MIN_FLOATS = 1u << 16;
constexpr uint32_t AUTO_EXACT_FRAMES = 12;
constexpr size_t CASUAL_VIEW_STATES = 32;
constexpr size_t SEEN_KEYS = 64;
constexpr size_t VIEW_TABLE_BYTES = (size_t)256 << 20;

struct RasterSlice {
    uint32_t* done_bits = nullptr;
    uint32_t* unsat_count = nullptr;
    uint32_t* gate_host = nullptr;
    float* state = nullptr;
    const uint32_t* offsets_near = nullptr;
    uint32_t* zcut = nullptr;
    const uint32_t* depth_keys_sorted = nullptr;
    uint32_t nv = 0;
    bool cut_active = false;
    uint32_t* live_bands = nullptr;
    uint32_t* work = nullptr;
    const uint32_t* order = nullptr;
    uint32_t order_mode = 1;
    uint32_t* split = nullptr;
    uint32_t margin_pct = 150;
    BwdJobs jobs{};
};

struct ForwardRequest {
    BhCamera cam{};
    uint32_t n = 0, sh_degree = 0, flags = 0;
    const float* transforms = nullptr;
    const float* sh_coeffs = nullptr;
    const float* raw_opacities = nullptr;
    float bg[3] = {0, 0, 0};
    uint32_t view_id = 0;
    float* visible = nullptr;
    float* max_radius = nullptr;
    size_t visible_floats = 0;
    float* grad_begin = nullptr;
    size_t grad_floats = 0;
    bool defer_decision = false;
    bool allow_cut = true;
};

struct Frame {
    ViewUniforms u{};
    float bg[3] = {0, 0, 0};
    bool bwd_info = false, smooth = false;
    uint32_t nv = 0, ni = 0, budget = 0, num_tiles = 0, tile_bits = 0;
    float* proj_by_gid = nullptr;
    uint32_t* gfc = nullptr;
    float* projected = nullptr;
    uint32_t* cum = nullptr;
    uint32_t* slice_info = nullptr;
    uint32_t* done_bits = nullptr;
    uint32_t* tile_offsets_far = nullptr;
    uint32_t* far_counts = nullptr;
    uint32_t* far_block_totals = nullptr;
    uint32_t* far_group_totals = nullptr;
    uint32_t* tile_ids = nullptr;
    uint32_t* isect_gids = nullptr;
    uint32_t* tile_ids_sorted = nullptr;
    uint32_t* isect_gids_sorted = nullptr;
    float* out_f32 = nullptr;
    uint32_t* out_u8 = nullptr;
    float* visible = nullptr;
    uint32_t* lpt = nullptr;
    float class_width = 8.0f;
    RasterSlice rs{};
};

struct FarJob {
    bool pending = false;
    Frame frame{};
    bool gate_event_recorded = false;
    uint32_t gate_tag = 0;
    bool by_cut = false;
    ViewState* view = nullptr;
    bool view_shared = false;
    ForwardRequest req{};
};

struct GradClears {
    enum Span : uint8_t { NONE = 0, ZEROED, ROW_MARKS };
    Span span = NONE;
    bool accum = false;
    uint64_t generation = 0;
    void begin_forward() { span = NONE; accum = false; generation = 0; }
    void k1_cleared_span() { span = ZEROED; }
    void k5_cleared_accum(bool yes) { accum = yes; }
    void stamp(uint64_t gen) { generation = gen; }
    void mark_rows() { span = ROW_MARKS; }
    bool valid_for(uint64_t gen) const { return generation != 0 && generation == gen; }
    Span take_span(uint64_t gen) { const Span s = valid_for(gen) ? span : NONE; span = NONE; return s; }
    bool take_accum(uint64_t gen) { const bool a = valid_for(gen) && accum; accum = false; return a; }
};

struct ForwardState {
    BhRenderOut out{};
    ViewUniforms uniforms{};
    uint32_t n = 0, sh_degree = 0, flags = 0;
    float bg[3] = {0, 0, 0};
    uint32_t* lpt = nullptr;
    BwdJobs jobs{};
};
constexpr int RETAIN_SLOTS = 14;
struct Retained {
    ForwardState fs;
    Buffer blocks[RETAIN_SLOTS];
};

struct DepthTerm {
    const float* v_depth = nullptr;
    uint32_t mode = 0;
};

struct NormalTerm {
    const float* v_normal = nullptr;
    uint32_t mode = 0;
};

struct DistortionTerm {
    const float* v_distortion = nullptr;
    float gain = 0.0f;
    uint32_t kind = 0;
    float near_z = 0.0f, far_z = 0.0f;
    const float* moments = nullptr;
};

}


struct bh_ctx {
    int device = 0;
    hipStream_t stream = nullptr;
    bool owns_stream = false;
    std::string last_error;
    bh::Buffer slots[bh::SLOT_COUNT];
    uint32_t* host_counters = nullptr;
    hipEvent_t readback_ev = nullptr;
    hipEvent_t gate_ev = nullptr;
    bool counters_ready = false;
    uint32_t counter_phase = 0;
    bool have_forward = false;
    bh::ForwardState latest;
    uint64_t generation = 0;
    std::vector<bh::Retained> retained;
    std::vector<bh::Buffer> pool;
    bh::GradClears clears;
    float* pending_loss_dst = nullptr;
    void* image_tab_host = nullptr;
    size_t image_tab_cap = 0;
    hipEvent_t image_tab_ev = nullptr;
    const bh_lpips* lpips = nullptr;
    float lpips_weight = 0.0f;
    float* pose_grad = nullptr;
    bool depth_attached = false;
    BhDepthTarget depth_target{};
    bool normal_attached = false;
    BhNormalTermConfig normal_term{};
    bool distortion_attached = false;
    BhDistortionTermConfig distortion_term{};
    bh_exposure* exposure = nullptr;
    std::vector<bh_exposure*> exposures;
    void* comm = nullptr;
    hipStream_t comm_stream = nullptr;
    hipEvent_t comm_ev = nullptr;
    int comm_rank = 0, comm_world = 1;
    float slice_fraction = 0.0f;
    float last_slice_share = 1.0f;
    bool far_direct = false;
    uint32_t readback_tag = 0;
    uint32_t gate_tag = 0;
    bool gate_signal_queued = false;
    bool gate_learn = false;
    uint32_t far_launches = 0;
    std::unordered_map<uint64_t, bh::ViewState> views;
    uint64_t seen_keys[bh::SEEN_KEYS] = {};
    uint32_t seen_pos = 0;
    uint32_t casual_views = 0;
    uint32_t view_id = 0;
    uint64_t view_clock = 0;
    float margin_scale = 1.0f;
    float ctrl_up = 1.5f, ctrl_down = 0.998f, ctrl_floor = 0.5f, ctrl_gap_exp = 1.0f / 3.0f;
    uint32_t cut_min_pairs = bh::CUT_MIN_PAIRS;
    bool knob_spec_k5 = true;
    bool knob_event_waits = false;
    bool knob_readback_copy = false;
    bool knob_no_view_hash = false;
    bool knob_fixed_margin = false;
    bool knob_cut_sort_all = false;
    uint32_t knob_band_mode = 1;
    uint32_t knob_k16_waves = 0;
    uint32_t knob_k16_split = 250;
    uint32_t knob_k16_split_min = bh::SPLIT_MIN_WORK;
    uint32_t knob_k16_split_of_max = 45;
    const uint32_t* last_split = nullptr;
    uint32_t knob_k16_order = 1;
    uint32_t knob_cut_margin_pct = 150;
    bh::FarJob far_job;
    uint32_t refine_n = 0, refine_new_n = 0;
    bool dsort_lds_raised = false;
    uint32_t* sort_groups = nullptr;
    size_t sort_groups_cap = 0, sort_groups_dirty = 0;
    uint32_t sort_groups_cur = 0;
    uint32_t* dsort_spl = nullptr;
    bool dsort_spl_written = false;
    bool knob_dsort_splitters = true;
    bool adam_lds_raised = false;
    uint32_t update_lds_raised = 0;
    size_t lds_optin_max = 0;
    bool knob_no_lpt = false;
    bool knob_bwd_wide_rows = false;
    bool knob_bwd_jobs = true;
    bool knob_lpt_linear = false;
    bool knob_force_exchange = false;
    bool knob_break_allreduce = false;
    bool knob_generic_depth_sort = false;
    bool knob_zero_grads = false;
    uint32_t knob_fail_loss_at = 0;
    uint32_t train_steps_seen = 0;
    uint32_t knob_loss_bands = 1;
    uint32_t knob_tile_sort = 0;
    float auto_exact_share = 0.9f;
    bool knob_direct_allreduce = false;
    uint32_t knob_k5_exact_spw = 32;
    bool knob_no_dormant = false;
    int knob_update_sparse = -1;
    uint32_t knob_update_rows = 0;
    uint32_t knob_sort_kpt = 0;
    const void* marks_m2_sh = nullptr; const void* marks_m1_t = nullptr; uint32_t marks_n = 0, marks_step = 0;
    bh::Profiler prof;
};

namespace bh {

int set_error(bh_ctx* ctx, int code, const std::string& msg);
int forward_impl(bh_ctx* ctx, const ForwardRequest& req, BhRenderOut* out);
int wait_host_tag(bh_ctx* ctx, const volatile uint32_t* word, uint32_t want, const char* what);
int find_saved_bwd_forward(bh_ctx* ctx, const BhRenderOut* saved, int not_bwd_code, const char* who, const ForwardState** fs);
int backward_impl(bh_ctx* ctx, const ForwardState& fs, const float* v_output, const float* transforms, const float* sh_coeffs,
                  const float* raw_opacities, float* v_transforms, float* v_sh_coeffs, float* v_raw_opacities, float* v_refine_weight,
                  size_t span_floats, bool want_refine, const DepthTerm* depth = nullptr, float* v_viewmat = nullptr,
                  const NormalTerm* normal = nullptr, const DistortionTerm* distortion = nullptr);
int launch_depth_backward(bh_ctx* ctx, const ForwardState& fs, const DepthTerm& term, float* v_combined);
int launch_depth_vz_scatter(bh_ctx* ctx, const ForwardState& fs, float* v_transforms, bool mark_rows = false, float* v_sh_coeffs = nullptr,
                            float* v_raw_opacities = nullptr, float* v_refine_weight = nullptr, const float* v_z = nullptr);
int launch_depth_forward(bh_ctx* ctx, const ForwardState& fs, uint32_t mode, float* out_depth);
int launch_normal_backward(bh_ctx* ctx, const ForwardState& fs, const NormalTerm& term, const float* transforms, float* v_combined);
int launch_normal_vn_scatter(bh_ctx* ctx, const ForwardState& fs, const float* transforms, float* v_transforms, bool mark_rows = false,
                             float* v_sh_coeffs = nullptr, float* v_raw_opacities = nullptr, float* v_refine_weight = nullptr);
int launch_normal_map(bh_ctx* ctx, const ForwardState& fs, const float* transforms, uint32_t mode, float* out);
int launch_normal_loss(bh_ctx* ctx, const BhCamera& cam, const float* normal, const float* depth, const float* image, uint32_t h, uint32_t w, float weight,
                       bool accumulate_v_depth, float* loss, float* v_normal, float* v_depth, float* accum, float* accum_host);
int launch_distortion_backward(bh_ctx* ctx, const ForwardState& fs, const DistortionTerm& term, float* v_combined, float* depth_v_z, const float** v_z_out);
int launch_distortion_map(bh_ctx* ctx, const ForwardState& fs, const DistortionTerm& term, bool moments, float* out);
int check_distortion_kind(bh_ctx* ctx, uint32_t kind, float near_z, float far_z, const char* who);
int launch_distortion_loss(bh_ctx* ctx, const float* map, uint32_t h, uint32_t w, uint32_t channels, float weight, float* loss, float* accum,
                           float* accum_host);
int launch_depth_loss(bh_ctx* ctx, const float* depth, const BhDepthTarget& t, float* loss, float* v_depth, float* accum, float* accum_host);
int launch_loss_pair_final(bh_ctx* ctx, uint32_t rows, const double* partials, float c, float* loss, float* accum, float* accum_host);
int launch_pose_grad(bh_ctx* ctx, const ViewUniforms& u, uint32_t nv, bool mip, uint32_t sh_degree, const float* transforms,
                     const float* sh, const uint32_t* gid, const float* v_combined, float* v_viewmat);
uint32_t exposure_views(const bh_exposure* tab);
int launch_exposure_apply(bh_ctx* ctx, const bh_exposure* tab, uint32_t view, const float* img, uint32_t h, uint32_t w, float* out);
int launch_exposure_backward(bh_ctx* ctx, bh_exposure* tab, uint32_t view, const float* img, const float* v_exposed, uint32_t h, uint32_t w,
                             float* v_img, bool update);
void exposure_free_all(bh_ctx* ctx);

ViewState* frame_view(bh_ctx* ctx, const ForwardRequest& req, uint32_t tile_bw, uint32_t tile_bh, bool casual);
bool cut_this_frame(const bh_ctx* ctx, ViewState* vs, bool allow_cut);
uint32_t* view_table(const ViewState* vs);
uint32_t* view_splitters(ViewState* vs, bool cut, bool** written);
uint32_t cut_margin_pct(const bh_ctx* ctx, const ViewState* vs);
uint32_t list_budget(bh_ctx* ctx, ViewState* cut_view, uint32_t near_total, uint32_t ni);
void view_rendered(ViewState* vs, uint32_t ni);
int enqueue_far_slice(bh_ctx* ctx, const FarJob& j);
int finish_far_slice(bh_ctx* ctx, bool* launched);
bool far_job_decides_first(const bh_ctx* ctx);
void drop_far_job(bh_ctx* ctx);
inline void deliver_pending_loss(bh_ctx* ctx) {
    if (ctx->pending_loss_dst) {
        *ctx->pending_loss_dst = reinterpret_cast<const volatile float*>(ctx->host_counters)[HOST_LOSS_WORD];
        ctx->pending_loss_dst = nullptr;
    }
}
int check_hip(bh_ctx* ctx, hipError_t e, const char* what);
int lpips_train_term(bh_ctx* ctx, const float* img_hwc4, const uint32_t* gt_packed, uint32_t h, uint32_t w, const float* bg, float* v_output,
                     float* loss, float* loss_host);
std::string ply_header_comments(uint32_t sh_degree, bool render_mip, const float* up_axis);
enum ResizeOut : int { RESIZE_OUT_U8 = 0, RESIZE_OUT_PACKED = 1, RESIZE_OUT_PACKED_PREMUL = 2 };
size_t resize_table_bytes(uint32_t src, uint32_t dst, uint32_t filter);
void build_resize_table(uint32_t src, uint32_t dst, uint32_t filter, void* host);
using ResizeTable = std::shared_ptr<const std::vector<uint8_t>>;
ResizeTable resize_table(uint32_t src, uint32_t dst, uint32_t filter);
hipError_t enqueue_resize(hipStream_t st, const uint8_t* src, uint32_t w, uint32_t h, uint32_t channels, uint32_t nw, uint32_t nh,
// ... 21 lines not shown
        if (_rc != 0) return _rc; \
    } while (0)
#define BH_LAUNCH_CHECK(ctx, what)                                      \
    do {                                                                \
        hipError_t _e = hipGetLastError();                              \
        if (_e != hipSuccess) return bh::check_hip(ctx, _e, what);      \
    } while (0)

ViewUniforms make_uniforms(const BhCamera& c);


struct ForwardPrep {
    unsigned long long* next_counters = nullptr;
    uint32_t* visible = nullptr;
    uint32_t visible_words = 0;
    uint32_t* tile_table = nullptr;
    uint32_t tile_words = 0;
    float4* span = nullptr;
    uint32_t span_f4 = 0;
    uint32_t* slice_table = nullptr;
    uint32_t slice_words = 0;
    const uint32_t* order_work = nullptr;
    uint32_t* order_out = nullptr;
    uint32_t order_tiles = 0, order_tile_begin = 0;
    uint32_t order_mode = 1;
    uint32_t band_mode = 0;
    uint32_t* split_out = nullptr;
    float split_factor = 2.5f;
    uint32_t split_min = SPLIT_MIN_WORK;
    float split_of_max = 0.45f;
    bool list_all_visible = false;
};
int launch_project_forward(bh_ctx* ctx, const ViewUniforms& u, uint32_t n, bool mip, uint32_t sh_degree, const float* transforms,
                           const float* sh, const float* raw_opac, uint32_t* depth_keys, uint32_t* isect_counts, float* max_radius,
                           float* projected_by_gid, uint32_t* counters, const ForwardPrep& prep, uint32_t* zcut = nullptr,
                           uint32_t* near_counts = nullptr);
int launch_project_visible(bh_ctx* ctx, uint32_t nv, const float* projected_by_gid, const uint32_t* gid, float* projected);
int launch_map_gaussians(bh_ctx* ctx, uint32_t nv, const ViewUniforms& u, const float* projected_by_gid, const uint32_t* gid,
                         float* projected, const uint32_t* cum_tiles_hit, uint32_t* tile_ids, uint32_t* isect_gids,
                         float4* zero_span = nullptr, uint32_t zero_f4 = 0, uint32_t budget = 0xFFFFFFFFu, uint32_t* slice_info = nullptr,
                         const uint32_t* zcut = nullptr, const uint32_t* depth_keys_sorted = nullptr, const uint32_t* nv_dev = nullptr, uint32_t pair_cap = 0xFFFFFFFFu);
int launch_map_gaussians_far(bh_ctx* ctx, uint32_t nv, const ViewUniforms& u, const float* projected_by_gid, const uint32_t* gid,
                             float* projected, const uint32_t* cum_tiles_hit, uint32_t budget, const uint32_t* done_bits, const uint32_t* gate,
                             uint32_t* counts, uint32_t* block_totals, uint32_t* group_totals, uint32_t* slice_info, uint32_t* tile_ids, uint32_t* isect_gids);
int launch_project_backward(bh_ctx* ctx, const ViewUniforms& u, uint32_t nv, bool mip, uint32_t sh_degree,
                            const float* transforms, const float* sh, const float* raw_opac, const uint32_t* gid,
                            float* v_combined, float* v_transforms, float* v_sh, float* v_raw_opac,
                            float* v_refine, bool mark_written = false, const float* projected = nullptr);
struct SortGroups {
    uint32_t* sums = nullptr;
    uint32_t* stale = nullptr;
    uint32_t stale_words = 0;
};
inline uint32_t sort_group_count(uint32_t nblocks) { return (nblocks + SORT_GROUP_BLOCKS - 1u) / SORT_GROUP_BLOCKS; }
int sort_groups_next(bh_ctx* ctx, size_t words, SortGroups* out);
constexpr uint32_t SORT_DIRECT_GROUPS = 32;
inline bool sort_groups_scanned(uint32_t ngroups) { return ngroups > SORT_DIRECT_GROUPS; }
int sort_groups_scan(bh_ctx* ctx, uint32_t* sums, uint32_t ngroups, uint32_t tables, uint32_t* totals);
int radix_argsort(bh_ctx* ctx, const uint32_t* keys, const uint32_t* vals, uint32_t n, uint32_t bits,
                  uint32_t* out_keys, uint32_t* out_vals);
int radix_argsort_dev(bh_ctx* ctx, const uint32_t* keys, const uint32_t* vals, uint32_t n_max, const uint32_t* n_dev, const uint32_t* gate,
                      const uint32_t* out_base, uint32_t bits, uint32_t* out_keys, uint32_t* out_vals, uint32_t alloc_n = 0);
bool tile_sort_supported(uint32_t bits, uint32_t n);
int tile_sort_offsets(bh_ctx* ctx, const uint32_t* keys, const uint32_t* vals, uint32_t n, uint32_t bits, uint32_t num_tiles,
                      uint32_t* out_keys, uint32_t* out_vals, uint32_t* tile_offsets, uint32_t alloc_n = 0);
bool depth_sort_supported(uint32_t n);
int depth_sort_scan(bh_ctx* ctx, const uint32_t* keys, const uint32_t* minmax, const uint32_t* counts, uint32_t n, uint32_t* out_keys,
                    uint32_t* out_vals, uint32_t* cum, const uint32_t* rb_set = nullptr, uint32_t* rb_host = nullptr, hipEvent_t rb_done = nullptr,
                    uint32_t rb_tag = 0, uint32_t* rb_dev = nullptr, uint32_t* spl = nullptr, bool* spl_written = nullptr);
int prefix_sum(bh_ctx* ctx, const uint32_t* in, const uint32_t* gather, uint32_t n, uint32_t* out, bool exclusive, const uint32_t* gate = nullptr);
int launch_tile_offsets(bh_ctx* ctx, const uint32_t* tile_ids_sorted, uint32_t num_isect, uint32_t num_tiles,
                        uint32_t* tile_offsets, bool pre_zeroed = false);
int launch_tile_offsets_dev(bh_ctx* ctx, const uint32_t* tile_ids_sorted, uint32_t n_max, const uint32_t* n_dev, const uint32_t* gate,
                            const uint32_t* base, uint32_t num_tiles, uint32_t* tile_offsets);

int launch_rasterize(bh_ctx* ctx, const ViewUniforms& u, const float bg[3], bool bwd_info, bool smooth,
                     const uint32_t* isect_gids, uint32_t* tile_offsets, const float* projected,
                     const uint32_t* global_from_compact, float* out_img, uint32_t* out_packed, float* visible,
                     uint32_t* lpt, float class_width, int phase = 0, const RasterSlice* slice = nullptr);
int launch_rasterize_backward(bh_ctx* ctx, const ViewUniforms& u, const float bg[3], bool smooth,
                              const uint32_t* isect_gids, const uint32_t* tile_offsets, const float* projected,
                              const float* out_img, const float* v_output, float* v_combined, const uint32_t* lpt,
                              const uint32_t* tile_offsets_far = nullptr, bool want_refine = true, const BwdJobs* jobs = nullptr,
                              uint32_t accum_rows = 0u);
int launch_image_loss_forward(bh_ctx* ctx, const float* pred, const uint32_t* gt, uint32_t channels, uint32_t h,
                              uint32_t w, const BhLossConfig& cfg, float* loss_map);
int launch_image_loss_backward(bh_ctx* ctx, const float* pred, const uint32_t* gt, const float* dl_dmap,
                               float dl_const, uint32_t channels, uint32_t h, uint32_t w, const BhLossConfig& cfg,
                               float* dl_dpred);
int launch_adam(bh_ctx* ctx, float* param, const float* grad, float* m1, float* m2, uint64_t rows, uint32_t row_len,
                const float* col_scale, float lr, uint32_t t, bool reduce_m2, float beta1, float beta2, float eps);
struct NoiseArgs { uint64_t seed; uint32_t step; float scale, clamp_abs; };
struct UpdateCall {
    const float *g_transforms, *g_sh, *g_opac;
    const float *refine_weight, *visible, *screen_radius;
    float gscale;
    bool vis_clamp;
    float tab_t[10];
    float lr_sh, sh_rest_scale, lr_opac;
    uint32_t t;
    float beta1, beta2, eps;
    const NoiseArgs* noise;
    bool masked_rows;
};
int launch_train_update(bh_ctx* ctx, const BhTrainState* st, const UpdateCall& c);
int launch_gather_stats(bh_ctx* ctx, float* refine_weight_norm, float* vis_weight, float* max_screen_size,
                        const float* refine_weight, const float* visible, const float* screen_radius, uint64_t n);
int launch_mean_noise(bh_ctx* ctx, float* transforms, const float* raw_opac, const float* visible,
                      const float* samples, uint64_t n, float noise_scale, float clamp_abs, uint64_t seed = 0, uint32_t step = 0);
int launch_normal_samples(bh_ctx* ctx, float* out, uint64_t n, uint64_t seed, uint32_t step);

int launch_fold_min_scale(bh_ctx* ctx, const float* transforms, const float* raw_opac, const float* min_scale, uint32_t n,
                          float* out_transforms, float* out_raw_opac);
int launch_fold_min_scale_backward(bh_ctx* ctx, const float* transforms, const float* raw_opac, const float* min_scale, uint32_t n,
                                   float* v_transforms, float* v_raw_opac);
int launch_compute_min_scale(bh_ctx* ctx, const float* transforms, uint32_t n, const float* view_cams, uint32_t k, float factor, float* out);

int comm_allreduce(bh_ctx* ctx, float* buf, uint64_t count, bool max_op);
int comm_exchange_strip_halos(bh_ctx* ctx, float* img, uint32_t h, uint32_t w, uint32_t row_begin_px, uint32_t row_end_px);

int launch_union_index(bh_ctx* ctx, const float* visible_sum, uint32_t n, uint32_t* block_scratch , uint32_t* count_dev,
                       uint32_t* idx);
int launch_exchange_rows(bh_ctx* ctx, bool gather, const uint32_t* idx, uint32_t count, uint32_t c3, float* g_tr, float* g_sh, float* g_op,
                         float* g_ref , float* compact);

}
```

brush_amd/csrc/loss_fused.hip:

```cpp
#include <cmath>
#include <cstdio>
#include <cstring>

#include "context.h"

#pragma clang fp contract(fast)

namespace bh {

namespace {

constexpr int LB = 16;
constexpr int HALO = 5;
constexpr float SSIM_C1 = 0.01f * 0.01f;
constexpr float SSIM_C2 = 0.03f * 0.03f;
constexpr float INV_255 = 1.0f / 255.0f;

struct Taps { float w[11]; };

Taps gauss_taps() {
    Taps g;
    const float sigma = 1.5f;
    float sum = 0.0f;
    for (int i = 0; i < 11; ++i) {
        const float x = (float)i - 5.0f;
        g.w[i] = expf(-x * x / (2.0f * sigma * sigma));
        sum += g.w[i];
    }
    for (int i = 0; i < 11; ++i) g.w[i] /= sum;
    return g;
}

#define BH_TAP_0 0x1.0d957p-10f
#define BH_TAP_1 0x1.f1fe04p-8f
#define BH_TAP_2 0x1.26eb18p-5f
#define BH_TAP_3 0x1.bff1p-4f
#define BH_TAP_4 0x1.b43c4p-3f
#define BH_TAP_5 0x1.106562p-2f
constexpr float TAP_TABLE[11] = {BH_TAP_0, BH_TAP_1, BH_TAP_2, BH_TAP_3, BH_TAP_4, BH_TAP_5, BH_TAP_4, BH_TAP_3, BH_TAP_2, BH_TAP_1, BH_TAP_0};
BH_DEV constexpr float tap(int i) { return TAP_TABLE[i]; }
BH_DEV float in_vgpr(float x) {
    asm volatile("" : "+v"(x));
    return x;
}

int taps_mismatch() {
    const Taps g = gauss_taps();
    for (int i = 0; i < 11; ++i)
        if (memcmp(&g.w[i], &TAP_TABLE[i], sizeof(float)) != 0) return i;
    return -1;
}

struct FusedArgs {
    uint32_t h, w;
    float l1_w, ssim_w;
    float bg[3];
    int composite, mask, alpha_match;
    float dl_rgb, dl_alpha;
    uint32_t ty_base;
    uint32_t row_end;
    const float* sum_src;
    int sum_n;
    float* loss_out;
    float* loss_host;
    uint32_t* started_host;
    uint32_t started_tag;
    uint32_t gx, gy_blocks, band_w;
};

BH_DEV bool loss_tile(const FusedArgs& a, uint32_t& bx, uint32_t& by, uint32_t& linear) {
    if (a.band_w == 0u) {
        bx = blockIdx.x; by = blockIdx.y;
        linear = by * a.gx + bx;
        return true;
    }
    const uint32_t b = blockIdx.x, xcd = b & 7u, j = b >> 3;
    const uint32_t x0 = xcd * a.band_w;
    if (x0 >= a.gx) return false;
    const uint32_t wb = min(a.band_w, a.gx - x0);
    by = j / wb;
    bx = x0 + (j - by * wb);
    linear = b;
    return by < a.gy_blocks;
}

BH_DEV float gt_ch(uint32_t val, uint32_t c) { return (float)((val >> (c * 8u)) & 0xffu) * INV_255; }

}

namespace {
constexpr int TW = 16, TH = 32;
constexpr int SW = TW + 2 * HALO;
constexpr int SR = TH + 2 * HALO;
#define BH_LOSS_HP 88
#define BH_LOSS_H2P 24
constexpr int HP = BH_LOSS_HP;
constexpr int H2P = BH_LOSS_H2P;
}

__global__ __launch_bounds__(256) void loss_fused_forward_kernel(const float* __restrict__ img ,
                                                                const uint32_t* __restrict__ gt,
                                                                float* __restrict__ partials ,
                                                                float* __restrict__ block_sums , uint32_t gy, FusedArgs a) {
    __shared__ float2 s_tile[3][SR * SW];
    __shared__ float s_h[(SR - 1) * HP + TW * 5];
    float* s_red = s_h;
    if (a.started_host && blockIdx.x == 0 && blockIdx.y == 0 && threadIdx.x == 0 && threadIdx.y == 0)
        *reinterpret_cast<volatile uint32_t*>(a.started_host) = a.started_tag;
    uint32_t bx, by, blin;
    if (!loss_tile(a, bx, by, blin)) return;
    const int tx0 = (int)bx * TW, ty0 = (int)a.ty_base * LB + (int)by * TH;
    const int lx = threadIdx.x, ly = threadIdx.y;
    const int rank = ly * TW + lx;
    const size_t plane = (size_t)a.h * a.w;
    constexpr int TILE_LOADS = (SR * SW + 255) / 256;
    float lx3[TILE_LOADS][3];
    uint32_t lval[TILE_LOADS];
    bool lin[TILE_LOADS];
    const int pxx = tx0 + lx;
    const int py[2] = {ty0 + 2 * ly, ty0 + 2 * ly + 1};
    const bool inside[2] = {pxx < (int)a.w && py[0] < (int)a.h, pxx < (int)a.w && py[1] < (int)a.h};
    uint32_t own_val[2] = {0u, 0u};
#pragma unroll
    for (int k = 0; k < TILE_LOADS; ++k) {
        const int i = rank + 256 * k;
        const int r = i / SW, q = i - r * SW;
        const int y = ty0 + r - HALO, x = tx0 + q - HALO;
        lin[k] = i < SR * SW && y >= 0 && x >= 0 && y < (int)a.h && x < (int)a.w;
        const int yc = y < 0 ? 0 : (y >= (int)a.h ? (int)a.h - 1 : y), xc = x < 0 ? 0 : (x >= (int)a.w ? (int)a.w - 1 : x);
        const size_t p = (size_t)yc * a.w + (size_t)xc;
        const float* ip = &img[p * 4];
        lx3[k][0] = ip[0]; lx3[k][1] = ip[1]; lx3[k][2] = ip[2];
        lval[k] = gt[p];
    }
#pragma unroll
    for (int o = 0; o < 2; ++o) {
        const int yc = py[o] >= (int)a.h ? (int)a.h - 1 : py[o], xc = pxx >= (int)a.w ? (int)a.w - 1 : pxx;
        own_val[o] = gt[(size_t)yc * a.w + (size_t)xc];
    }
#pragma unroll
    for (int k = 0; k < TILE_LOADS; ++k) {
        const int i = rank + 256 * k;
        if (i < SR * SW) {
            float g0 = 0.f, g1 = 0.f, g2 = 0.f;
            if (!lin[k]) lx3[k][0] = lx3[k][1] = lx3[k][2] = 0.0f;
            if (lin[k]) {
                const uint32_t val = lval[k];
                const float ga = gt_ch(val, 3);
                g0 = gt_ch(val, 0); g1 = gt_ch(val, 1); g2 = gt_ch(val, 2);
                if (a.composite) {
                    g0 = g0 + (1.0f - ga) * a.bg[0];
                    g1 = g1 + (1.0f - ga) * a.bg[1];
                    g2 = g2 + (1.0f - ga) * a.bg[2];
                }
            }
            s_tile[0][i] = make_float2(lx3[k][0], g0);
            s_tile[1][i] = make_float2(lx3[k][1], g1);
            s_tile[2][i] = make_float2(lx3[k][2], g2);
        }
    }
    float ga[2] = {0.f, 0.f}, chain[2] = {0.f, 0.f};
#pragma unroll
    for (int o = 0; o < 2; ++o) {
        if (inside[o]) {
            ga[o] = gt_ch(own_val[o], 3);
            chain[o] = a.mask ? a.dl_rgb * ga[o] : a.dl_rgb;
        }
    }
    float acc_rgb = 0.0f;
    const float tap4 = in_vgpr(tap(4)), l1_w = in_vgpr(a.l1_w), ssim_w = in_vgpr(a.ssim_w);
#pragma unroll 1
    for (int c = 0; c < 3; ++c) {
        __syncthreads();
        const int probe_rows = SR * (TW / 2);
        for (int i = rank; i < probe_rows; i += 256) {
            const int r = i / (TW / 2), pair = i - r * (TW / 2);
            const float2* row = &s_tile[c][r * SW + 2 * pair];
            float x[12], y[12], xx[12], yy[12], xy[12];
#pragma unroll
            for (int k = 0; k < 12; ++k) {
                const float2 v = row[k];
                x[k] = v.x; y[k] = v.y;
                xx[k] = v.x * v.x; yy[k] = v.y * v.y; xy[k] = v.x * v.y;
            }
#pragma unroll
            for (int o = 0; o < 2; ++o) {
                const int cc = HALO + o;
                float sx = 0, sx2 = 0, sy = 0, sy2 = 0, sxy = 0;
#pragma unroll
                for (int d = 1; d < 6; ++d) {
                    const float wd = d == 1 ? tap4 : tap(5 - d);
// ... 173 lines not shown
            for (int i = rank; i < SR * SW; i += 256) {
                const int r = i / SW, q = i - r * SW;
                const int y = ty0 + r - HALO, x = tx0 + q - HALO;
                const bool in = y >= 0 && x >= 0 && y < (int)a.h && x < (int)a.w;
                const size_t p = in ? (size_t)y * a.w + (size_t)x : 0;
                s_part[0][i] = in ? pc[p] : 0.0f;
                s_part[1][i] = in ? pc[plane + p] : 0.0f;
                s_part[2][i] = in ? pc[2 * plane + p] : 0.0f;
            }
        }
        __syncthreads();
        {
            const float* src = &s_part[0][0] + (rank >> 3) * SW + 2 * (rank & 7);
            float* dst = &s_h2[0][0] + (rank >> 3) * H2P + 2 * (rank & 7);
#pragma unroll
            for (int n = 0; n < 4; ++n) {
                if (n == 3 && rank >= 8 * (3 * SR - 96)) break;
                const float2* row = reinterpret_cast<const float2*>(src + 32 * n * SW);
                float x[12];
#pragma unroll
                for (int k = 0; k < 6; ++k) {
                    const float2 t = row[k];
                    x[2 * k] = t.x; x[2 * k + 1] = t.y;
                }
                float res[2];
#pragma unroll
                for (int o = 0; o < 2; ++o) {
                    const int cc = HALO + o;
                    float acc = 0.0f;
#pragma unroll
                    for (int d = 1; d < 6; ++d) acc += (x[cc - d] + x[cc + d]) * (d == 1 ? tap4 : tap(5 - d));
                    acc += x[cc] * tap(5);
                    res[o] = acc;
                }
                *reinterpret_cast<float2*>(dst + 32 * n * H2P) = make_float2(res[0], res[1]);
            }
        }
        __syncthreads();
        float v[3][12];
#pragma unroll
        for (int j = 0; j < 3; ++j)
#pragma unroll
            for (int r = 0; r < 12; ++r) v[j][r] = s_h2[j][(2 * ly + r) * H2P + lx];
#pragma unroll
        for (int o = 0; o < 2; ++o) {
            float sres[3];
#pragma unroll
            for (int j = 0; j < 3; ++j) {
                float acc = 0.0f;
#pragma unroll
                for (int d = 1; d < 6; ++d) acc += (v[j][o + 5 - d] + v[j][o + 5 + d]) * (d == 1 ? tap4 : tap(5 - d));
                acc += v[j][o + 5] * tap(5);
                sres[j] = acc;
            }
            const float ga = gt_ch(val[o], 3);
            float chain_c = a.dl_rgb;
            if (a.mask) chain_c = chain_c * ga;
            float ge = gt_ch(val[o], c);
            if (a.composite) ge = ge + (1.0f - ga) * a.bg[c];
            const float p1 = c == 0 ? pv[o].x : (c == 1 ? pv[o].y : pv[o].z);
            const float ssim_grad = sres[0] + (2.0f * p1) * sres[1] + ge * sres[2];
            const float diff = p1 - ge;
            const float l1_sign = diff > 0.0f ? 1.0f : (diff < 0.0f ? -1.0f : 0.0f);
            out[o][c] = __builtin_fmaf(ssim_w, ssim_grad, l1_w * l1_sign * chain_c);
        }
    }
#pragma unroll
    for (int o = 0; o < 2; ++o) {
        if (!inside[o]) continue;
        if (a.alpha_match) {
            const float ga = gt_ch(val[o], 3);
            const float diff = pv[o].w - ga;
            const float sign = diff > 0.0f ? 1.0f : (diff < 0.0f ? -1.0f : 0.0f);
            float chain = a.dl_alpha;
            if (a.mask) chain = chain * ga;
            out[o][3] = sign * chain;
        }
        *reinterpret_cast<float4*>(&v_output[((size_t)py[o] * a.w + (size_t)pxx) * 4]) = make_float4(out[o][0], out[o][1], out[o][2], out[o][3]);
    }
}

int launch_image_loss_fused_window(bh_ctx* ctx, const float* img_hwc4, const uint32_t* gt, uint32_t h, uint32_t w, const BhLossConfig& cfg,
                                   bool alpha_match, float dl_rgb, float dl_alpha, uint32_t tile_y0, uint32_t tile_y1, float* loss_out,
                                   float* v_output, float* loss_host, uint32_t* started_host, uint32_t started_tag) {
    const uint32_t gx = (w + LB - 1) / LB, gy = (h + LB - 1) / LB;
    if (tile_y1 > gy) tile_y1 = gy;
    if (tile_y0 >= tile_y1) return set_error(ctx, BH_ERR_INVALID_ARG, "image loss: empty tile-row window");
    static const int bad_tap = taps_mismatch();
    if (bad_tap >= 0) {
        char msg[160];
        snprintf(msg, sizeof msg, "image loss: Gaussian tap %d is %a on this host, the kernels' table holds %a", bad_tap, (double)gauss_taps().w[bad_tap],
                 (double)TAP_TABLE[bad_tap]);
        return set_error(ctx, BH_ERR_UNSUPPORTED, msg);
    }
    const uint32_t a0 = tile_y0 > 0 ? tile_y0 - 1 : 0, a1 = tile_y1 < gy ? tile_y1 + 1 : gy;
    const dim3 block(TW, 16);
    const bool banded = ctx->knob_loss_bands != 0u && gx >= 16u;
    const size_t hw = (size_t)h * w;
    auto* partials = (float*)ensure(ctx, SLOT_LOSS_MAP, hw * 12 * sizeof(float));
    auto* block_sums = (float*)ensure(ctx, SLOT_MISC, (size_t)gx * gy * sizeof(float));
    if (!partials || !block_sums) return BH_ERR_OOM;
    FusedArgs a;
    a.h = h; a.w = w;
    a.l1_w = cfg.l1_weight; a.ssim_w = cfg.ssim_weight;
    a.bg[0] = cfg.bg[0]; a.bg[1] = cfg.bg[1]; a.bg[2] = cfg.bg[2];
    a.composite = cfg.composite_bg; a.mask = cfg.mask; a.alpha_match = alpha_match ? 1 : 0;
    a.dl_rgb = dl_rgb; a.dl_alpha = dl_alpha;
    {
        ProfScope ps(ctx, "ImageLoss");
        a.ty_base = a0;
        a.row_end = h;
        a.sum_src = nullptr; a.sum_n = 0; a.loss_out = nullptr; a.loss_host = nullptr;
        a.started_host = started_host; a.started_tag = started_tag;
        a.gx = gx; a.gy_blocks = (a1 - a0 + 1) / 2;
        a.band_w = banded ? (gx + 7u) / 8u : 0u;
        const dim3 grid_a = banded ? dim3(8u * a.band_w * a.gy_blocks) : dim3(gx, a.gy_blocks);
        hipLaunchKernelGGL(loss_fused_forward_kernel, grid_a, block, 0, ctx->stream, img_hwc4, gt, partials, block_sums, a1, a);
        BH_LAUNCH_CHECK(ctx, "loss_fused_forward_kernel");
    }
    {
        ProfScope ps(ctx, "ImageLossBackward");
        a.ty_base = tile_y0;
        a.row_end = tile_y1 * LB < h ? tile_y1 * LB : h;
        a.sum_src = block_sums + (size_t)tile_y0 * gx;
        a.sum_n = (int)((tile_y1 - tile_y0) * gx);
        a.loss_out = loss_out;
        a.loss_host = loss_host;
        a.started_host = nullptr; a.started_tag = 0;
        a.gy_blocks = (tile_y1 - tile_y0 + 1) / 2;
        const dim3 grid_b = banded ? dim3(8u * a.band_w * a.gy_blocks) : dim3(gx, a.gy_blocks);
        hipLaunchKernelGGL(loss_fused_backward_kernel, grid_b, block, 0, ctx->stream, img_hwc4, gt, partials, v_output, a);
        BH_LAUNCH_CHECK(ctx, "loss_fused_backward_kernel");
    }
    return 0;
}

int launch_image_loss_fused(bh_ctx* ctx, const float* img_hwc4, const uint32_t* gt, uint32_t h, uint32_t w, const BhLossConfig& cfg,
                            bool alpha_match, float dl_rgb, float dl_alpha, float* loss_out, float* v_output, float* loss_host, uint32_t* started_host,
                            uint32_t started_tag) {
    return launch_image_loss_fused_window(ctx, img_hwc4, gt, h, w, cfg, alpha_match, dl_rgb, dl_alpha, 0, (h + LB - 1) / LB, loss_out, v_output, loss_host,
                                          started_host, started_tag);
}

}
```

brush_amd/csrc/rasterize.hip:

```cpp
#include <hip/hip_ext.h>

#include <type_traits>

#include "context.h"
#include "device_blend.h"

namespace bh {

struct OffsetsDyn {
    const uint32_t* n_dev = nullptr;
    const uint32_t* gate = nullptr;
    const uint32_t* base = nullptr;
};
__global__ __launch_bounds__(256) void tile_offsets_kernel(const uint32_t* __restrict__ tile_ids, uint32_t num_isect,
                                                          uint32_t num_tiles, uint32_t* __restrict__ tile_offsets, OffsetsDyn dyn) {
    uint32_t ofs = 0;
    if (dyn.gate && *dyn.gate == 0u) return;
    if (dyn.n_dev) { const uint32_t v = *dyn.n_dev; num_isect = v < num_isect ? v : num_isect; }
    if (dyn.base) { ofs = *dyn.base; tile_ids += ofs; }
    const uint32_t i0 = (blockIdx.x * 256 + threadIdx.x) * 4u;
    if (i0 >= num_isect) return;
    uint32_t t[4];
    if (i0 + 4u <= num_isect && (ofs & 3u) == 0u) {
        const uint4 v = *reinterpret_cast<const uint4*>(&tile_ids[i0]);
        t[0] = v.x; t[1] = v.y; t[2] = v.z; t[3] = v.w;
    } else {
#pragma unroll
        for (uint32_t k = 0; k < 4u; ++k) t[k] = i0 + k < num_isect ? tile_ids[i0 + k] : 0xFFFFFFFFu;
    }
    uint32_t prev = i0 > 0u ? tile_ids[i0 - 1u] : 0xFFFFFFFFu;
#pragma unroll
    for (uint32_t k = 0; k < 4u; ++k) {
        const uint32_t i = i0 + k;
        if (i < num_isect) {
            const uint32_t tid = t[k];
            if (tid < num_tiles) {
                if (i == num_isect - 1u) tile_offsets[tid * 2 + 1] = ofs + i + 1u;
                if (i == 0u) {
                    tile_offsets[tid * 2] = ofs;
                } else if (tid != prev) {
                    if (prev < num_tiles) tile_offsets[prev * 2 + 1] = ofs + i;
                    tile_offsets[tid * 2] = ofs + i;
                }
            } else if (i > 0u && prev < num_tiles) {
                tile_offsets[prev * 2 + 1] = ofs + i;
            }
            prev = tid;
        }
    }
}

int launch_tile_offsets(bh_ctx* ctx, const uint32_t* tile_ids_sorted, uint32_t num_isect, uint32_t num_tiles,
                        uint32_t* tile_offsets, bool pre_zeroed) {
    if (!pre_zeroed) BH_HIP(ctx, hipMemsetAsync(tile_offsets, 0, ((size_t)num_tiles * 2 + 8 * LPT_CLASSES) * 4, ctx->stream));
    if (num_isect == 0) return 0;
    hipLaunchKernelGGL(tile_offsets_kernel, dim3((num_isect + 1023) / 1024), dim3(256), 0, ctx->stream, tile_ids_sorted, num_isect, num_tiles, tile_offsets, OffsetsDyn{});
    BH_LAUNCH_CHECK(ctx, "tile_offsets_kernel");
    return 0;
}

int launch_tile_offsets_dev(bh_ctx* ctx, const uint32_t* tile_ids_sorted, uint32_t n_max, const uint32_t* n_dev, const uint32_t* gate,
                            const uint32_t* base, uint32_t num_tiles, uint32_t* tile_offsets) {
    if (n_max == 0) return 0;
    OffsetsDyn dyn;
    dyn.n_dev = n_dev;
    dyn.gate = gate;
    dyn.base = base;
    hipLaunchKernelGGL(tile_offsets_kernel, dim3((n_max + 1023) / 1024), dim3(256), 0, ctx->stream, tile_ids_sorted, n_max, num_tiles, tile_offsets, dyn);
    BH_LAUNCH_CHECK(ctx, "tile_offsets_kernel");
    return 0;
}

struct RasterUniforms {
    uint32_t tile_bw, num_tiles, img_w, img_h;
    uint32_t tile_begin;
    float bg_r, bg_g, bg_b;
    float rcp_class_width;
    uint32_t band_mode;
};

BH_DEV uint32_t lpt_band_tiles(uint32_t num_tiles) { return band_slots(num_tiles); }
BH_DEV size_t lpt_list_offset(uint32_t num_tiles, uint32_t band, uint32_t cls) {
    return (size_t)LPT_HEADER_WORDS + ((size_t)band * LPT_CLASSES + cls) * lpt_band_tiles(num_tiles);
}
BH_DEV uint32_t ckpt_slot(uint32_t range_lo, uint32_t tile, uint32_t seg) { return range_lo / BWD_SEG + tile + seg - 1u; }
constexpr uint32_t JOB_TILE_MASK = 0x00FFFFFFu, JOB_SEG_SHIFT = 24u, JOB_SEG_MASK = 0x3Fu, JOB_LAST_BIT = 1u << 30;

constexpr int SPLAT_STRIDE = 12;
constexpr int BATCH = 64;
constexpr uint32_t SPLIT_GROUP = 4;



template <bool SMOOTH, bool HALF_CONIC, uint32_t GID_SCALE = 1u>
BH_DEV uint32_t stage_batch(const uint32_t* __restrict__ isect_gids, const float* __restrict__ projected,
                            uint32_t batch_start, uint32_t cnt, int lane, float* s_splat) {
    uint32_t cg = 0;
    if ((uint32_t)lane < cnt) {
        cg = isect_gids[batch_start + lane];
        const float* p = projected + (size_t)cg * 9;
        float v[9];
#pragma unroll
        for (int k = 0; k < 9; ++k) v[k] = p[k];
        const float cut = blend_sigma_cut<SMOOTH>(v[5]);
        const uint32_t gate = (v[6] >= 0.0f ? 1u : 0u) | (v[7] >= 0.0f ? 2u : 0u) | (v[8] >= 0.0f ? 4u : 0u);
        float4* d = reinterpret_cast<float4*>(s_splat + lane * SPLAT_STRIDE);
        const float diag = HALF_CONIC ? 0.5f : 1.0f;
        d[0] = make_float4(v[0], v[1], diag * v[2], v[3]);
        d[1] = make_float4(diag * v[4], v[5], __builtin_fmaxf(v[6], 0.0f), __builtin_fmaxf(v[7], 0.0f));
        d[2] = make_float4(__builtin_fmaxf(v[8], 0.0f), cut, u2f(gate), u2f(cg * GID_SCALE));
    }
    return cg;
}


struct SliceArgs {
    uint32_t* done_bits = nullptr;
    uint32_t* unsat_count = nullptr;
    uint32_t* gate_host = nullptr;
    float* state = nullptr;
    const uint32_t* offsets_near = nullptr;
    uint32_t* zcut = nullptr;
    const uint32_t* depth_keys_sorted = nullptr;
    uint32_t nv = 0;
    uint32_t cut_active = 0;
    uint32_t* live_bands = nullptr;
    uint32_t tile_bh = 0;
    uint32_t margin_pct = 150;
    const uint32_t* order = nullptr;
    uint32_t order_mode = 1;
    uint32_t* split = nullptr;
    uint32_t* work = nullptr;
    BwdJobs jobs{};
};

template <bool BWD_INFO, bool SMOOTH, int PHASE, int NQ>
BH_DEV void blend_tile(const RasterUniforms& u, const uint32_t* __restrict__ isect_gids, uint32_t* __restrict__ tile_offsets,
                       const float* __restrict__ projected, const uint32_t* __restrict__ global_from_compact, float* __restrict__ out_img,
                       uint32_t* __restrict__ out_packed, float* __restrict__ visible, uint32_t* __restrict__ lpt, const SliceArgs& sl,
                       float* s_splat, const uint32_t local_tile, const uint32_t qsel, uint32_t* split_row) {
    constexpr int NK = NQ == 4 ? 2 : 1;
    const uint32_t bidx = blockIdx.x;
    const uint32_t tile = u.tile_begin + local_tile;
    if (PHASE == 2) {
        if (*sl.unsat_count == 0u) return;
        if ((sl.done_bits[tile >> 5] >> (tile & 31u)) & 1u) return;
    }
    const int lane = threadIdx.x;
    const uint32_t tx0 = (tile % u.tile_bw) * TILE_WIDTH + (NQ == 1 ? 8u * (qsel & 1u) : 0u);
    const uint32_t ty0 = (tile / u.tile_bw) * TILE_WIDTH + (NQ == 1 ? 8u * (qsel >> 1) : 0u);
    const uint32_t px0 = tx0 + (lane & 7), py0 = ty0 + (lane >> 3);
    float pcx[NK], pcy[NK];
#pragma unroll
    for (int k = 0; k < NK; ++k) {
        pcx[k] = (float)(px0 + 8 * k) + 0.5f;
        pcy[k] = (float)(py0 + 8 * k) + 0.5f;
    }
    float tr[NQ], pr[NQ], pg[NQ], pb[NQ];
    auto any_live = [&]() {
        bool l = false;
#pragma unroll
        for (int q = 0; q < NQ; ++q) l = l || tr[q] > 0.0f;
        return l;
    };
#pragma unroll
    for (int q = 0; q < NQ; ++q) {
        const uint32_t px = px0 + 8 * (q & 1), py = py0 + 8 * (q >> 1);
        const bool inside = px < u.img_w && py < u.img_h;
        tr[q] = inside ? 1.0f : -1.0f;
        pr[q] = pg[q] = pb[q] = 0.0f;
        if (PHASE == 2 && inside) {
            const float4 st = *reinterpret_cast<const float4*>(&sl.state[((size_t)px + (size_t)py * u.img_w) * 4]);
            pr[q] = st.x; pg[q] = st.y; pb[q] = st.z; tr[q] = st.w;
        }
    }
    const uint32_t range_lo = tile_offsets[tile * 2];
    const uint32_t range_hi = tile_offsets[tile * 2 + 1];
    uint32_t last_useful = range_lo;
    uint32_t reached = range_lo;
    uint32_t sign_mask = 0x80000000u;
    asm volatile("" : "+v"(sign_mask));

    uint32_t batch_start = range_lo;
    for (; batch_start < range_hi; batch_start += BATCH) {
        const bool live = any_live();
        if (__ballot(live) == 0ull) break;
        const uint32_t cnt = min((uint32_t)BATCH, range_hi - batch_start);
        if (BWD_INFO && PHASE != 2) {
            const uint32_t done = batch_start - range_lo;
            if (sl.jobs.ckpt && done != 0u && (done % BWD_SEG) == 0u && done / BWD_SEG < BWD_MAX_SEGS) {
                const uint32_t slot = ckpt_slot(range_lo, tile, done / BWD_SEG);
                if (slot < sl.jobs.ckpt_cap) {
                    float4* ck = sl.jobs.ckpt + (size_t)slot * 256u + (uint32_t)lane;
// ... 198 lines not shown
                    const uint32_t r8 = (uint32_t)clampf(fr * 255.0f, 0.0f, 255.0f);
                    const uint32_t g8 = (uint32_t)clampf(fg * 255.0f, 0.0f, 255.0f);
                    const uint32_t b8 = (uint32_t)clampf(fb * 255.0f, 0.0f, 255.0f);
                    const uint32_t a8 = (uint32_t)clampf(fa * 255.0f, 0.0f, 255.0f);
                    out_packed[pix] = r8 | (g8 << 8) | (b8 << 16) | (a8 << 24);
                }
            }
        }
    };
    auto park_pixels = [&]() {
#pragma unroll
        for (int q = 0; q < NQ; ++q) {
            const uint32_t px = px0 + 8 * (q & 1), py = py0 + 8 * (q >> 1);
            if (px < u.img_w && py < u.img_h)
                *reinterpret_cast<float4*>(&sl.state[((size_t)px + (size_t)py * u.img_w) * 4]) = make_float4(pr[q], pg[q], pb[q], tr[q]);
        }
    };
    if (NQ == 1) {
        if (BWD_INFO && PHASE != 2 && sl.jobs.ckpt) {
            uint32_t done = ((batch_start - range_lo + BWD_SEG - 1u) / BWD_SEG) * BWD_SEG;
            if (done == 0u) done = BWD_SEG;
            for (; done < range_hi - range_lo && done / BWD_SEG < BWD_MAX_SEGS; done += BWD_SEG) {
                const uint32_t slot = ckpt_slot(range_lo, tile, done / BWD_SEG);
                if (slot >= sl.jobs.ckpt_cap) break;
                sl.jobs.ckpt[(size_t)slot * 256u + qsel * 64u + (uint32_t)lane] = make_float4(pr[0], pg[0], pb[0], tr[0]);
            }
        }
        if (PHASE == 1 && !near_complete) park_pixels();
        store_pixels();
        uint32_t ticket = 0u, m_useful = 0u, m_reached = 0u, m_unsat = 0u;
        if (lane == 0) {
            if (last_useful > range_lo) atomicMax(&split_row[1], last_useful);
            if (reached > range_lo) atomicMax(&split_row[2], reached);
            if (!saturated) atomicOr(&split_row[3], 1u);
            __threadfence();
            ticket = atomicAdd(&split_row[0], 1u);
            if (ticket == 3u) {
                m_useful = atomicOr(&split_row[1], 0u);
                m_reached = atomicOr(&split_row[2], 0u);
                m_unsat = atomicOr(&split_row[3], 0u);
            }
        }
        ticket = __builtin_amdgcn_readfirstlane(ticket);
        if (ticket != 3u) return;
        last_useful = max(range_lo, (uint32_t)__builtin_amdgcn_readfirstlane(m_useful));
        reached = max(range_lo, (uint32_t)__builtin_amdgcn_readfirstlane(m_reached));
        saturated = __builtin_amdgcn_readfirstlane(m_unsat) == 0u;
    }
    if (PHASE == 1 && !saturated && !near_complete) {
        if (NQ == 4) park_pixels();
        if (lane == 0) {
            if (BWD_INFO) tile_offsets[tile * 2 + 1] = last_useful;
            atomicAdd(sl.unsat_count, 1u);
            if (sl.gate_host) {
                *reinterpret_cast<volatile uint32_t*>(sl.gate_host) = 1u;
                __threadfence_system();
            }
            if (sl.live_bands) {
                const uint32_t ttx = tile % u.tile_bw, tty = tile / u.tile_bw;
                atomicOr(&sl.live_bands[0], 1u << ((ttx * 32u) / u.tile_bw));
                atomicOr(&sl.live_bands[1], 1u << ((tty * 32u) / sl.tile_bh));
            }
        }
        return;
    }

    if (NQ == 4) store_pixels();
    if (BWD_INFO && PHASE != 2 && lpt && sl.jobs.ckpt) {
        const uint32_t jwork = last_useful - range_lo;
        const uint32_t last_batch = reached > range_lo ? ((reached - 1u - range_lo) / BATCH) * BATCH : 0u;
        const uint32_t ck_span = NQ == 1 ? (range_hi > range_lo ? range_hi - 1u - range_lo : 0u) : last_batch;
        uint32_t n_ck = min(ck_span / BWD_SEG, BWD_MAX_SEGS - 1u);
        const uint32_t slot0 = ckpt_slot(range_lo, tile, 1u);
        n_ck = slot0 < sl.jobs.ckpt_cap ? min(n_ck, sl.jobs.ckpt_cap - slot0) : 0u;
        const uint32_t nj = min((jwork + BWD_SEG - 1u) / BWD_SEG, n_ck + 1u);
        if ((uint32_t)lane < nj) {
            const uint32_t lo = (uint32_t)lane * BWD_SEG;
            const bool last = (uint32_t)lane + 1u == nj;
            const uint32_t size = (last ? jwork : lo + BWD_SEG) - lo;
            const uint32_t cls = size >= BWD_SEG ? LPT_CLASSES - 1u : (size * (LPT_CLASSES - 1u)) / BWD_SEG;
            const uint32_t band = bidx & 7u;
            const uint32_t pos = atomicAdd(&lpt[band * LPT_CLASSES + cls], 1u);
            const uint32_t entry = local_tile | ((uint32_t)lane << JOB_SEG_SHIFT) | (last ? JOB_LAST_BIT : 0u);
            if (cls == LPT_CLASSES - 1u) sl.jobs.top_list[(size_t)band * sl.jobs.top_cap + pos] = entry;
            else lpt[lpt_list_offset(u.num_tiles, band, cls) + pos] = entry;
        }
    }
    if (lane == 0) {
        if (PHASE == 1) atomicOr(&sl.done_bits[tile >> 5], 1u << (tile & 31u));
        uint32_t work = (BWD_INFO ? last_useful : reached) - range_lo;
        if (PHASE == 2) {
            const uint32_t n_lo = sl.offsets_near[tile * 2], n_hi = sl.offsets_near[tile * 2 + 1];
            work += n_hi - n_lo;
        }
        if (sl.work) sl.work[tile] = work;
        if (BWD_INFO) {
            tile_offsets[tile * 2 + 1] = last_useful;
            if (lpt && !sl.jobs.ckpt) {
                uint32_t cls;
                if (u.rcp_class_width > 0.0f) {
                    cls = min(LPT_CLASSES - 1u, (uint32_t)((float)work * u.rcp_class_width));
                } else if (work < 8u) {
                    cls = 0u;
                } else {
                    const uint32_t p = 28u - (uint32_t)__builtin_clz(work);
                    cls = min(LPT_CLASSES - 1u, 1u + 8u * p + ((work >> p) & 7u));
                }
                const uint32_t list = (bidx & 7u) * LPT_CLASSES + cls;
                const uint32_t pos = atomicAdd(&lpt[list], 1u);
                lpt[lpt_list_offset(u.num_tiles, bidx & 7u, cls) + pos] = local_tile | JOB_LAST_BIT;
            }
        }
        if (sl.zcut) {
            uint32_t newcut = ZCUT_ALL;
            if (saturated && sl.nv) {
                const uint32_t stop = BWD_INFO ? last_useful : reached;
                uint32_t g = 0xFFFFFFFFu;
                if (stop > range_lo) g = isect_gids[stop - 1u];
                if (g != 0xFFFFFFFFu) {
                    const unsigned long long mraw = (unsigned long long)g * sl.margin_pct / 100ull;
                    const uint32_t margin = mraw > 128ull ? (mraw < 0x7FFFFFFFull ? (uint32_t)mraw : 0x7FFFFFFFu) : 128u;
                    const uint32_t g2 = (unsigned long long)g + margin < sl.nv ? g + margin : sl.nv - 1u;
                    newcut = sl.depth_keys_sorted[g2] & ~1u;
                }
            }
            sl.zcut[tile] = newcut;
        }
    }
}

template <bool BWD_INFO, bool SMOOTH, int PHASE>
__global__ __launch_bounds__(64, 8) void rasterize_kernel(RasterUniforms u, const uint32_t* __restrict__ isect_gids,
                                                      uint32_t* __restrict__ tile_offsets, const float* __restrict__ projected,
                                                      const uint32_t* __restrict__ global_from_compact,
                                                      float* __restrict__ out_img, uint32_t* __restrict__ out_packed,
                                                      float* __restrict__ visible, uint32_t* __restrict__ lpt, SliceArgs sl) {
    __shared__ __attribute__((aligned(16))) float s_splat[BATCH * SPLAT_STRIDE];
    const uint32_t bidx = blockIdx.x;
    uint32_t local_tile, qsel = 4u;
    uint32_t* split_row = nullptr;
    if (sl.order) {
        const uint32_t per = band_slots(u.num_tiles);
        uint32_t j = bidx >> 3;
        if (PHASE != 2 && sl.split) {
            const uint32_t band = bidx & 7u;
            const uint32_t h = sl.split[band];
            if (j < 4u * h) {
                qsel = j & 3u;
                j >>= 2;
                split_row = sl.split + 8u + (band * SPLIT_MAX + j) * 4u;
            } else {
                j -= 3u * h;
            }
        } else if (sl.order_mode == 2u) {
            const uint32_t seg = (per + 7u) / 8u;
            j = (j & 7u) * seg + (j >> 3);
        }
        local_tile = j < per ? sl.order[(bidx & 7u) * per + j] : 0xFFFFFFFFu;
    } else {
        local_tile = tile_of_block(bidx, u.num_tiles, u.band_mode);
    }
    if (local_tile >= u.num_tiles) return;
    if (PHASE != 2 && qsel < 4u)
        blend_tile<BWD_INFO, SMOOTH, PHASE, 1>(u, isect_gids, tile_offsets, projected, global_from_compact, out_img, out_packed, visible, lpt, sl, s_splat, local_tile, qsel, split_row);
    else
        blend_tile<BWD_INFO, SMOOTH, PHASE, 4>(u, isect_gids, tile_offsets, projected, global_from_compact, out_img, out_packed, visible, lpt, sl, s_splat, local_tile, 0u, nullptr);
}

template <bool BWD_INFO, bool SMOOTH>
static void launch_rasterize_phase(int phase, dim3 grid, uint32_t lds_pad, hipStream_t stream, const RasterUniforms& u, const uint32_t* isect_gids, uint32_t* tile_offsets,
                                   const float* projected, const uint32_t* gfc, float* out_img, uint32_t* out_packed, float* visible, uint32_t* lpt,
                                   const SliceArgs& sl) {
    const dim3 block(64);
    if (phase == 1) hipLaunchKernelGGL((rasterize_kernel<BWD_INFO, SMOOTH, 1>), grid, block, lds_pad, stream, u, isect_gids, tile_offsets, projected, gfc, out_img, out_packed, visible, lpt, sl);
    else if (phase == 2) hipLaunchKernelGGL((rasterize_kernel<BWD_INFO, SMOOTH, 2>), grid, block, lds_pad, stream, u, isect_gids, tile_offsets, projected, gfc, out_img, out_packed, visible, lpt, sl);
    else hipLaunchKernelGGL((rasterize_kernel<BWD_INFO, SMOOTH, 0>), grid, block, lds_pad, stream, u, isect_gids, tile_offsets, projected, gfc, out_img, out_packed, visible, lpt, sl);
}

int launch_rasterize(bh_ctx* ctx, const ViewUniforms& vu, const float bg[3], bool bwd_info, bool smooth,
                     const uint32_t* isect_gids, uint32_t* tile_offsets, const float* projected,
                     const uint32_t* global_from_compact, float* out_img, uint32_t* out_packed, float* visible,
                     uint32_t* lpt, float class_width, int phase, const RasterSlice* slice) {
    RasterUniforms u;
    u.band_mode = ctx->knob_band_mode;
    u.rcp_class_width = class_width > 0.0f ? 1.0f / (class_width > 1.0f ? class_width : 1.0f) : 0.0f;
    u.tile_bw = vu.tile_bw;
    u.num_tiles = vu.tile_bw * (vu.tile_y1 - vu.tile_y0);
    u.tile_begin = vu.tile_bw * vu.tile_y0;
    u.img_w = vu.img_w;
    u.img_h = vu.img_h;
    u.bg_r = bg[0]; u.bg_g = bg[1]; u.bg_b = bg[2];
    SliceArgs sl;
    if (slice) {
        sl.done_bits = slice->done_bits;
        sl.unsat_count = slice->unsat_count;
        sl.gate_host = phase == 1 ? slice->gate_host : nullptr;
        sl.state = slice->state;
        sl.offsets_near = slice->offsets_near;
        sl.zcut = slice->zcut;
        sl.depth_keys_sorted = slice->depth_keys_sorted;
        sl.nv = slice->nv;
        sl.cut_active = slice->cut_active ? 1u : 0u;
        sl.live_bands = slice->live_bands;
        sl.tile_bh = vu.tile_bh;
        sl.margin_pct = slice->margin_pct;
        sl.order = slice->order;
        sl.order_mode = slice->order_mode;
        sl.split = (phase != 2 && slice->order && slice->order_mode == 1u) ? slice->split : nullptr;
        sl.work = slice->work;
        if (bwd_info && phase != 2 && lpt) sl.jobs = slice->jobs;
    }
    if (sl.zcut && (!sl.depth_keys_sorted && sl.nv)) sl.zcut = nullptr;
    if (phase != 0 && (!sl.done_bits || !sl.unsat_count || !sl.state || (phase == 2 && !sl.offsets_near)))
        return set_error(ctx, BH_ERR_INVALID_ARG, "launch_rasterize: sliced phase without its scratch");
    uint32_t nblocks = band_slots(u.num_tiles) * 8u;
    if (sl.order && sl.order_mode == 2u) nblocks = ((band_slots(u.num_tiles) + 7u) / 8u) * 64u;
    if (sl.split) nblocks += 8u * 3u * SPLIT_MAX;
    const dim3 grid(nblocks);
    uint32_t lds_pad = 0;
    if (ctx->knob_k16_waves >= 1u && ctx->knob_k16_waves < 8u && sl.order && sl.order_mode == 1u && phase != 2) {
        const uint32_t per_block = (160u * 1024u) / (4u * ctx->knob_k16_waves);
        const uint32_t fixed = BATCH * SPLAT_STRIDE * 4u;
        lds_pad = per_block > fixed + 64u ? ((per_block - fixed - 64u) & ~63u) : 0u;
    }
    if (bwd_info && smooth) launch_rasterize_phase<true, true>(phase, grid, lds_pad, ctx->stream, u, isect_gids, tile_offsets, projected, global_from_compact, out_img, out_packed, visible, lpt, sl);
    else if (bwd_info) launch_rasterize_phase<true, false>(phase, grid, lds_pad, ctx->stream, u, isect_gids, tile_offsets, projected, global_from_compact, out_img, out_packed, visible, lpt, sl);
    else launch_rasterize_phase<false, false>(phase, grid, lds_pad, ctx->stream, u, isect_gids, tile_offsets, projected, global_from_compact, out_img, out_packed, visible, lpt, sl);
    BH_LAUNCH_CHECK(ctx, "rasterize_kernel");
    return 0;
}



BH_DEV float blend_exp_bwd(float x) {
    return exp_blend(x);
}

constexpr int BWD_WAVES = 5;
template <bool SMOOTH, bool REFINE, bool JOBS, bool WIDE>
__global__ __launch_bounds__(64, (BWD_WAVES - (SMOOTH ? 1 : 0) + (REFINE ? 0 : 1))) void rasterize_backward_kernel(RasterUniforms u, const uint32_t* __restrict__ isect_gids,
                                                               const uint32_t* __restrict__ tile_offsets,
                                                               const float* __restrict__ projected,
                                                               const float* __restrict__ out_img,
                                                               const float* __restrict__ v_output,
                                                               float* __restrict__ v_combined, const uint32_t* __restrict__ lpt,
                                                               const uint32_t* __restrict__ tile_offsets_far, BwdJobs jb) {
    __shared__ __attribute__((aligned(16))) float s_splat[BATCH * SPLAT_STRIDE];
  for (uint32_t jidx = blockIdx.x >> 3;; jidx += gridDim.x >> 3) {
    uint32_t local_tile, seg = 0u;
    bool to_end = true;
    if (lpt) {
        const uint32_t xcd = blockIdx.x & 7u;
        uint32_t j = jidx;
        const uint32_t* cnt = lpt + xcd * LPT_CLASSES;
        uint32_t cls = LPT_CLASSES;
        bool found = false;
        static_assert(LPT_CLASSES % 8u == 0u, "classes are walked in groups of eight");
        for (uint32_t base = LPT_CLASSES; base > 0u && !found; base -= 8u) {
            uint32_t k[8];
#pragma unroll
            for (uint32_t i = 0; i < 8u; ++i) k[i] = cnt[base - 1u - i];
#pragma unroll
            for (uint32_t i = 0; i < 8u; ++i) {
                if (!found) {
                    if (j < k[i]) { cls = base - 1u - i; found = true; }
                    else j -= k[i];
                }
            }
        }
        if (!found) return;
        const uint32_t entry = (JOBS && cls == LPT_CLASSES - 1u) ? jb.top_list[(size_t)xcd * jb.top_cap + j] : lpt[lpt_list_offset(u.num_tiles, xcd, cls) + j];
        local_tile = entry & JOB_TILE_MASK;
        if (JOBS) { seg = (entry >> JOB_SEG_SHIFT) & JOB_SEG_MASK; to_end = (entry & JOB_LAST_BIT) != 0u; }
    } else {
        local_tile = tile_of_block(blockIdx.x, u.num_tiles, u.band_mode);
        if (local_tile >= u.num_tiles) return;
    }
    const uint32_t tile = u.tile_begin + local_tile;
    uint32_t seg_lo0 = tile_offsets[tile * 2], seg_hi0 = tile_offsets[tile * 2 + 1];
    const uint32_t list_lo = seg_lo0;
    uint32_t seg_lo1 = 0, seg_hi1 = 0;
    if (!JOBS && tile_offsets_far) { seg_lo1 = tile_offsets_far[tile * 2]; seg_hi1 = tile_offsets_far[tile * 2 + 1]; }
    if (JOBS) {
        seg_lo0 += seg * BWD_SEG;
        if (!to_end) seg_hi0 = seg_lo0 + BWD_SEG;
        if (seg_hi0 <= seg_lo0) continue;
    } else if (seg_hi0 <= seg_lo0 && seg_hi1 <= seg_lo1) return;
    int lane = threadIdx.x;
    if (JOBS) asm volatile("" : "+v"(lane));
    const uint32_t tx0 = (tile % u.tile_bw) * TILE_WIDTH, ty0 = (tile / u.tile_bw) * TILE_WIDTH;
    const uint32_t px0 = tx0 + (lane & 7), py0 = ty0 + (lane >> 3);
    const float pcx[2] = {(float)px0 + 0.5f, (float)(px0 + 8) + 0.5f};
    const float pcy[2] = {(float)py0 + 0.5f, (float)(py0 + 8) + 0.5f};
    const float img_w_f = (float)u.img_w, img_h_f = (float)u.img_h;
    float sS[4], sw[4];
    float vox[4], voy[4], voz[4], w2q[4], h2q[4];
    float4 o4[4], vo4[4];
#pragma unroll
    for (int q = 0; q < 4; ++q) {
        const uint32_t px = px0 + 8 * (q & 1), py = py0 + 8 * (q >> 1);
        const uint32_t pxc = px < u.img_w ? px : u.img_w - 1u, pyc = py < u.img_h ? py : u.img_h - 1u;
        const size_t pix = ((size_t)pxc + (size_t)pyc * u.img_w) * 4;
        o4[q] = *reinterpret_cast<const float4*>(&out_img[pix]);
        vo4[q] = *reinterpret_cast<const float4*>(&v_output[pix]);
    }
#pragma unroll
    for (int q = 0; q < 4; ++q) {
        const uint32_t px = px0 + 8 * (q & 1), py = py0 + 8 * (q >> 1);
        if (px < u.img_w && py < u.img_h) {
            const float4 o = o4[q];
            const float4 vo = vo4[q];
            const float t_final = 1.0f - o.w;
            const float v_o_w = (vo.w - (u.bg_r * vo.x + u.bg_g * vo.y + u.bg_b * vo.z)) * t_final;
            sS[q] = __builtin_fmaf(o.z - t_final * u.bg_b, vo.z, __builtin_fmaf(o.y - t_final * u.bg_g, vo.y, (o.x - t_final * u.bg_r) * vo.x)) - v_o_w;
            sw[q] = 1.0f;
            vox[q] = vo.x; voy[q] = vo.y; voz[q] = vo.z;
            if (REFINE) {
                const float inv_fa = 1.0f / __builtin_fmaxf(o.w, 1.0e-5f);
                w2q[q] = (img_w_f * inv_fa) * (img_w_f * inv_fa);
                h2q[q] = (img_h_f * inv_fa) * (img_h_f * inv_fa);
            } else {
                w2q[q] = h2q[q] = 0.0f;
            }
        } else {
            sS[q] = sw[q] = 0.0f;
            vox[q] = voy[q] = voz[q] = 0.0f;
            w2q[q] = h2q[q] = 0.0f;
        }
    }
    if (JOBS && seg != 0u) {
        const float4* ck = jb.ckpt + (size_t)ckpt_slot(list_lo, tile, seg) * 256u + (uint32_t)lane;
        float4 c4[4];
#pragma unroll
        for (int q = 0; q < 4; ++q) c4[q] = ck[q * 64];
#pragma unroll
        for (int q = 0; q < 4; ++q) {
            sS[q] -= __builtin_fmaf(c4[q].z, voz[q], __builtin_fmaf(c4[q].y, voy[q], c4[q].x * vox[q]));
            sw[q] = (sw[q] != 0.0f && c4[q].w > 0.0f) ? c4[q].w : 0.0f;
        }
    }

    float aP = 0.f, aQ = 0.f, aR2 = 0.f, aR3 = 0.f, aR4 = 0.f, aCr = 0.f, aCg = 0.f, aCb = 0.f, aVs = 0.f, aRf = 0.f;
    const uint32_t ri = (uint32_t)lane & 15u, rrow = (uint32_t)lane >> 4;
    const uint32_t rsel = ((rrow & 1u) << 1) | (rrow >> 1);
    const uint32_t in_k2 = 0u - (((ri >> 2) & 1u) ^ 1u);
    const uint32_t comp4 = ((in_k2 & (8u + (rrow >> 1))) | (~in_k2 & ((ri >> 3) * 4u + rsel))) * 4u;
    const bool sends = ((ri & 3u) == 0u) & (ri != 8u) & ((ri != 0u) | ((rrow & 1u) == 0u));
    auto run_batch = [&](auto clamp_tag, const uint32_t cnt) {
        constexpr bool CLAMP = decltype(clamp_tag)::value;
        for (uint32_t t = 0; t < cnt; ++t) {
            const float4 s0 = *reinterpret_cast<const float4*>(&s_splat[t * SPLAT_STRIDE]);
            const float4 s1 = *reinterpret_cast<const float4*>(&s_splat[t * SPLAT_STRIDE + 4]);
            const float2 s2 = *reinterpret_cast<const float2*>(&s_splat[t * SPLAT_STRIDE + 8]);
            const float h00 = s0.z, c01 = s0.w, h11 = s1.x, color_a = s1.y;
            const float cr = s1.z, cgc = s1.w, cb = s2.x;
            const uint32_t cut_bits = f2u(s2.y);
            float dxp[2], dyp[2], a_xx[2], b_x[2], c_y[2], e_x[2], e_y[2];
#pragma unroll
            for (int k = 0; k < 2; ++k) {
                dxp[k] = pcx[k] - s0.x;
                e_x[k] = h00 * dxp[k];
                a_xx[k] = e_x[k] * dxp[k];
                b_x[k] = c01 * dxp[k];
                dyp[k] = pcy[k] - s0.y;
                c_y[k] = h11 * dyp[k];
                e_y[k] = c01 * dyp[k];
            }
            bool any = false;
#pragma unroll
            for (int q = 0; q < 4; ++q) {
                const int k = q & 1, m = q >> 1;
                const float half_qv = __builtin_fmaf(c_y[m], dyp[m], a_xx[k]);
                const float sigma = __builtin_fmaf(b_x[k], dyp[m], half_qv);
                const bool pre = sw[q] > 0.0f && f2u(sigma) <= cut_bits;
                if (__ballot(pre) != 0ull) {
                    const float gaussian = blend_exp_bwd(-sigma);
                    const float alpha_raw = color_a * gaussian;
                    const float alpha = CLAMP ? __builtin_fminf(0.999f, alpha_raw) : alpha_raw;
                    const float w_cut = SMOOTH ? alpha_cutoff_weight(alpha) : 1.0f;
                    const bool ok = pre && (SMOOTH ? (w_cut > 0.0f) : (alpha >= ALPHA_CUTOFF_MID));
                    const float alpha_eff = SMOOTH ? alpha * w_cut : alpha;
                    const float one_m = 1.0f - alpha_eff;
                    const float T = sw[q];
                    const float next_t = T * one_m;
                    const bool live = !(next_t <= 1.0e-4f);
                    sw[q] = (ok && !live) ? 0.0f : T;
                    if (ok && live) {
                        __asm__ volatile("" ::: "memory");
                        const float vis = alpha_eff * T;
                        aCr = __builtin_fmaf(vis, vox[q], aCr);
                        aCg = __builtin_fmaf(vis, voy[q], aCg);
                        aCb = __builtin_fmaf(vis, voz[q], aCb);
                        const float ra = __builtin_amdgcn_rcpf(one_m);
                        const float cv = __builtin_fmaf(cb, voz[q], __builtin_fmaf(cgc, voy[q], cr * vox[q]));
                        const float v_alpha_eff = __builtin_fmaf(T, cv, -sS[q]) * ra;
                        const float v_alpha = SMOOTH ? v_alpha_eff * (w_cut + alpha * alpha_cutoff_weight_deriv(alpha)) : v_alpha_eff;
                        const float v_sigma = (!CLAMP || alpha_raw <= 0.999f) ? -alpha * v_alpha : 0.0f;
                        const float ux = v_sigma * dxp[k], uy = v_sigma * dyp[m];
                        aP += ux;
                        aQ += uy;
                        aR2 = __builtin_fmaf(ux, dxp[k], aR2);
                        aR3 = __builtin_fmaf(ux, dyp[m], aR3);
                        aR4 = __builtin_fmaf(uy, dyp[m], aR4);
                        aVs += v_sigma;
                        if (REFINE) {
                            const float ex = __builtin_fmaf(2.0f, e_x[k], e_y[m]), ey = __builtin_fmaf(2.0f, c_y[m], b_x[k]);
                            const float n2 = __builtin_fmaf(h2q[q] * ey, ey, w2q[q] * (ex * ex));
                            aRf = __builtin_fmaf(__builtin_fabsf(v_sigma), __builtin_amdgcn_sqrtf(n2), aRf);
                        }
                        sS[q] = __builtin_fmaf(-vis, cv, sS[q]);
                        sw[q] = next_t;
                        any = true;
                    }
                }
            }
            if (__ballot(any) != 0ull) {
                const float h0 = swap32_add(aP, aQ), h1 = swap32_add(aR2, aR3), h2 = swap32_add(aR4, aCr);
                const float h3 = swap32_add(aCg, aCb), h4 = swap32_add(aVs, REFINE ? aRf : 0.0f);
                const float mine = row_allreduce3_folded(swap16_add(h0, h1), swap16_add(h2, h3), swap16_add(h4, 0.0f));
                const uint32_t row = f2u(s_splat[t * SPLAT_STRIDE + 11]);
                if (sends) {
                    if (!WIDE) unsafeAtomicAdd(reinterpret_cast<float*>(reinterpret_cast<char*>(v_combined) + (size_t)(uint32_t)(row + comp4)), mine);
                    else unsafeAtomicAdd(reinterpret_cast<float*>(reinterpret_cast<char*>(v_combined) + ((size_t)row * 40u + comp4)), mine);
                }
                aP = aQ = aR2 = aR3 = aR4 = aCr = aCg = aCb = aVs = aRf = 0.0f;
            }
        }
    };

#pragma nounroll
    for (int part = 0; part < (JOBS ? 1 : 2); ++part) {
        const uint32_t range_lo = part ? seg_lo1 : seg_lo0, range_hi = part ? seg_hi1 : seg_hi0;
        for (uint32_t batch_start = range_lo; batch_start < range_hi; batch_start += BATCH) {
            const uint32_t cnt = min((uint32_t)BATCH, range_hi - batch_start);
            __syncthreads();
            stage_batch<SMOOTH, true, WIDE ? 1u : 40u>(isect_gids, projected, batch_start, cnt, lane, s_splat);
            __syncthreads();
            const bool mine_clamps = (uint32_t)lane < cnt && s_splat[lane * SPLAT_STRIDE + 5] > 0.999f;
            if (__ballot(mine_clamps) != 0ull) run_batch(std::true_type{}, cnt);
            else run_batch(std::false_type{}, cnt);
        }
    }
    if (!JOBS) return;
  }
}

template <bool SMOOTH, bool REFINE, bool JOBS, bool WIDE>
static void launch_rasterize_backward_t(hipStream_t stream, dim3 grid, hipEvent_t ea, hipEvent_t eb, const RasterUniforms& u, const uint32_t* isect_gids,
                                        const uint32_t* tile_offsets, const float* projected, const float* out_img, const float* v_output, float* v_combined,
                                        const uint32_t* lpt, const uint32_t* tile_offsets_far, const BwdJobs& jb) {
    const dim3 block(64);
    if (ea)
        hipExtLaunchKernelGGL((rasterize_backward_kernel<SMOOTH, REFINE, JOBS, WIDE>), grid, block, 0, stream, ea, eb, 0, u, isect_gids, tile_offsets, projected, out_img, v_output, v_combined, lpt, tile_offsets_far, jb);
    else
        hipLaunchKernelGGL((rasterize_backward_kernel<SMOOTH, REFINE, JOBS, WIDE>), grid, block, 0, stream, u, isect_gids, tile_offsets, projected, out_img, v_output, v_combined, lpt, tile_offsets_far, jb);
}

int launch_rasterize_backward(bh_ctx* ctx, const ViewUniforms& vu, const float bg[3], bool smooth,
                              const uint32_t* isect_gids, const uint32_t* tile_offsets, const float* projected,
                              const float* out_img, const float* v_output, float* v_combined, const uint32_t* lpt,
                              const uint32_t* tile_offsets_far, bool want_refine, const BwdJobs* jobs, uint32_t accum_rows) {
    RasterUniforms u;
    u.band_mode = ctx->knob_band_mode;
    u.rcp_class_width = 1.0f;
    u.tile_bw = vu.tile_bw;
    u.num_tiles = vu.tile_bw * (vu.tile_y1 - vu.tile_y0);
    u.tile_begin = vu.tile_bw * vu.tile_y0;
    u.img_w = vu.img_w;
    u.img_h = vu.img_h;
    u.bg_r = bg[0]; u.bg_g = bg[1]; u.bg_b = bg[2];
    const bool by_jobs = jobs && jobs->ckpt && lpt;
    const BwdJobs jb = by_jobs ? *jobs : BwdJobs{};
    const uint32_t per = band_slots(u.num_tiles);
    const uint32_t nblocks = (by_jobs ? 2u : 1u) * per * 8u;
    const dim3 grid(nblocks);
    const bool wide = ctx->knob_bwd_wide_rows || accum_rows == 0u || (uint64_t)accum_rows * 40ull > (1ull << 32);
    hipEvent_t ea = ctx->prof.ext_a, eb = ctx->prof.ext_b;
    ctx->prof.ext_a = ctx->prof.ext_b = nullptr;
#define BH_K17_W(S, R, J, W) launch_rasterize_backward_t<S, R, J, W>(ctx->stream, grid, ea, eb, u, isect_gids, tile_offsets, projected, out_img, v_output, v_combined, lpt, tile_offsets_far, jb)
#define BH_K17(S, R, J) do { if (wide) BH_K17_W(S, R, J, true); else BH_K17_W(S, R, J, false); } while (0)
    if (by_jobs) {
        if (smooth && want_refine) BH_K17(true, true, true);
        else if (smooth) BH_K17(true, false, true);
        else if (want_refine) BH_K17(false, true, true);
        else BH_K17(false, false, true);
    } else {
        if (smooth && want_refine) BH_K17(true, true, false);
        else if (smooth) BH_K17(true, false, false);
        else if (want_refine) BH_K17(false, true, false);
        else BH_K17(false, false, false);
    }
#undef BH_K17
#undef BH_K17_W
    BH_LAUNCH_CHECK(ctx, "rasterize_backward_kernel");
    return 0;
}

}
```

Before: 1321.

## Flatten backward job lists in the loss kernel into per-band record arrays

Job entries become 16-byte records carrying tile/segment, list range and checkpoint slot. The fused loss kernel now flattens each band's class lists into one contiguous array. In the non-smooth case the blend backward reads its job directly from that array instead of searching class counters and re-reading tile offsets. It also prefetches the next record, the checkpoint and the first batch's splat rows. This adds work and LDS synchronisation to the loss kernel, plus extra buffer space and template variants.

```diff
diff --git a/brush_amd/_ffi.py b/brush_amd/_ffi.py
--- a/brush_amd/_ffi.py
+++ b/brush_amd/_ffi.py
@@ -316,7 +316,9 @@
 _lib_th = None
 TEST_HOOKS_LIB_PATH = os.path.join(_DIR, "libbrush_hip_testhooks.so")
 TEST_HOOK_SYMBOLS = {"bh_debug_fill_train_scratch": (C.c_int, [C.c_void_p, C.c_uint32]),
-                     "bh_debug_split_counts": (C.c_int, [C.c_void_p, C.POINTER(C.c_uint32)])}
+                     "bh_debug_split_counts": (C.c_int, [C.c_void_p, C.POINTER(C.c_uint32)]),
+                     "bh_debug_bwd_jobs": (C.c_int, [C.c_void_p, C.c_uint32, C.c_uint32, C.c_uint32, C.c_void_p, C.c_uint64]),
+                     "bh_debug_set_ckpt_cap": (C.c_int, [C.c_void_p, C.c_uint32])}
 
 
 class BrushHipError(RuntimeError):
diff --git a/brush_amd/csrc/api.hip b/brush_amd/csrc/api.hip
--- a/brush_amd/csrc/api.hip
+++ b/brush_amd/csrc/api.hip
@@ -12,10 +12,11 @@
 
 int launch_image_loss_fused(bh_ctx* ctx, const float* img_hwc4, const uint32_t* gt, uint32_t h, uint32_t w, const BhLossConfig& cfg,
                             bool alpha_match, float dl_rgb, float dl_alpha, float* loss_out, float* v_output, float* loss_host = nullptr,
-                            uint32_t* started_host = nullptr, uint32_t started_tag = 0);
+                            uint32_t* started_host = nullptr, uint32_t started_tag = 0, const FlattenJobs* flatten = nullptr);
 int launch_image_loss_fused_window(bh_ctx* ctx, const float* img_hwc4, const uint32_t* gt, uint32_t h, uint32_t w, const BhLossConfig& cfg,
                                    bool alpha_match, float dl_rgb, float dl_alpha, uint32_t tile_y0, uint32_t tile_y1, float* loss_out,
-                                   float* v_output, float* loss_host = nullptr, uint32_t* started_host = nullptr, uint32_t started_tag = 0);
+                                   float* v_output, float* loss_host = nullptr, uint32_t* started_host = nullptr, uint32_t started_tag = 0,
+                                   const FlattenJobs* flatten = nullptr);
 
 __global__ __launch_bounds__(256) void zero_two_kernel(float4* __restrict__ a, size_t na, float4* __restrict__ b, size_t nb) {
     const size_t stride = (size_t)gridDim.x * 256;
@@ -375,6 +376,9 @@
      [](bh_ctx* c, const char* v) { uint32_t u = 0; if (!parse_u32(v, 16, 64, &u) || !(u == 16 || u == 32 || u == 64)) return false; c->knob_k5_exact_spw = u; return true; }},
     {"bwd_jobs", "0|1: the blend backward works on checkpointed 128-entry segments of the tiles' lists (default 1) or on whole tiles",
      [](bh_ctx* c, const char* v) { return parse_flag(v, &c->knob_bwd_jobs); }},
+    {"bwd_flat_jobs", "0|1: the train step's blend backward takes its jobs from one flat record array per band, flattened by the loss kernel (default 1), "
+                      "or looks each job up through the class counters and lists",
+     [](bh_ctx* c, const char* v) { return parse_flag(v, &c->knob_bwd_flat_jobs); }},
     {"bwd_wide_rows", "0|1: the blend backward addresses the gradient accumulator in 64 bits, as it does by itself from 2^32 bytes of accumulator on (default 0)",
      [](bh_ctx* c, const char* v) { return parse_flag(v, &c->knob_bwd_wide_rows); }},
     {"no_lpt", "0|1: the blend backward takes its tiles in index order",
@@ -799,12 +803,17 @@
     while (f.tile_bits < 32 && (f.num_tiles >> f.tile_bits) != 0) f.tile_bits++;
     if (bwd_jobs) {
         const uint32_t listed = cut_active ? near_total : f.ni;
-        const uint32_t ckpt_cap = (uint32_t)std::min<uint64_t>((uint64_t)listed / BWD_SEG + f.num_tiles + 1u, BWD_CKPT_MAX_SLOTS);
+        uint32_t ckpt_cap = (uint32_t)std::min<uint64_t>((uint64_t)listed / BWD_SEG + f.num_tiles + 1u, BWD_CKPT_MAX_SLOTS);
+        if (ctx->debug_ckpt_cap && ctx->debug_ckpt_cap < ckpt_cap) ckpt_cap = ctx->debug_ckpt_cap;
         f.rs.jobs.ckpt = (float4*)ensure(ctx, SLOT_BWD_CKPT, (size_t)ckpt_cap * 256 * sizeof(float4));
         f.rs.jobs.ckpt_cap = ckpt_cap;
         f.rs.jobs.top_cap = band_slots(f.num_tiles) + ckpt_cap;
-        f.rs.jobs.top_list = (uint32_t*)ensure(ctx, SLOT_BWD_TOPLIST, (size_t)8 * f.rs.jobs.top_cap * 4);
+        const size_t top_recs = (size_t)8 * f.rs.jobs.top_cap, low_recs = (size_t)8 * (LPT_CLASSES - 1u) * band_slots(f.num_tiles);
+        f.rs.jobs.top_list = (BwdJobRec*)ensure(ctx, SLOT_BWD_TOPLIST, (2 * top_recs + low_recs) * sizeof(BwdJobRec) + 8 * sizeof(uint32_t));
         if (!f.rs.jobs.ckpt || !f.rs.jobs.top_list) return BH_ERR_OOM;
+        f.rs.jobs.flat = f.rs.jobs.top_list + top_recs;
+        f.rs.jobs.cls_list = f.rs.jobs.flat + top_recs;
+        f.rs.jobs.flat_total = reinterpret_cast<uint32_t*>(f.rs.jobs.cls_list + low_recs);
     }
     if (view) {
         f.rs.zcut = vtab;
@@ -958,6 +967,7 @@
     latest.bg[0] = f.bg[0]; latest.bg[1] = f.bg[1]; latest.bg[2] = f.bg[2];
     latest.lpt = f.lpt;
     latest.jobs = f.rs.jobs;
+    latest.flat_valid = false;
     ctx->have_forward = true;
     if (view) view_rendered(view, f.ni);
     return 0;
@@ -1055,7 +1065,7 @@
         if (r.num_intersections > 0 && v_output)
             BH_TRY(launch_rasterize_backward(ctx, fs.uniforms, fs.bg, fs.flags & BH_FLAG_SMOOTH_CUTOFF,
                                              r.compact_gid_from_isect, r.tile_offsets, r.projected, r.out_img, v_output, v_combined, fs.lpt,
-                                             r.tile_offsets_far, want_refine, &fs.jobs, nv));
+                                             r.tile_offsets_far, want_refine, &fs.jobs, nv, fs.flat_valid && ctx->knob_bwd_flat_jobs));
         if (depth) BH_TRY(launch_depth_backward(ctx, fs, *depth, v_combined));
         if (normal) BH_TRY(launch_normal_backward(ctx, fs, *normal, transforms, v_combined));
         if (distortion) BH_TRY(launch_distortion_backward(ctx, fs, *distortion, v_combined, depth ? (float*)ctx->slots[SLOT_DEPTH].ptr : nullptr, &scatter_v_z));
@@ -1325,6 +1335,40 @@
     BH_HIP(ctx, hipMemcpyAsync(out, ctx->last_split, 8 * 4, hipMemcpyDeviceToHost, ctx->stream));
     BH_HIP(ctx, hipStreamSynchronize(ctx->stream));
     return 1;
+}
+extern "C" int bh_debug_bwd_jobs(bh_ctx* ctx, uint32_t what, uint32_t band, uint32_t cls, uint32_t* out, uint64_t cap_words) {
+    if (!ctx || !out || band >= 8u || cls >= LPT_CLASSES - 1u) return BH_ERR_INVALID_ARG;
+    if (!ctx->have_forward) return set_error(ctx, BH_ERR_STATE, "debug_bwd_jobs: no forward on this context yet");
+    const ForwardState& fs = ctx->latest;
+    const BwdJobs& jb = fs.jobs;
+    const bool by_jobs = jb.ckpt && fs.lpt;
+    const uint32_t per = band_slots(fs.uniforms.tile_bw * (fs.uniforms.tile_y1 - fs.uniforms.tile_y0));
+    const void* src = nullptr;
+    uint64_t words = 0;
+    uint32_t info[6] = {jb.top_cap, per, fs.flat_valid ? 1u : 0u, jb.ckpt_cap, fs.out.num_tiles, by_jobs ? 1u : 0u};
+    switch (what) {
+    case 0: words = 6; break;
+    case 1: src = fs.lpt; words = fs.lpt ? 8u * LPT_CLASSES : 0u; break;
+    case 2: src = by_jobs ? jb.flat_total : nullptr; words = 8; break;
+    case 3: src = by_jobs ? jb.flat + (size_t)band * jb.top_cap : nullptr; words = (uint64_t)jb.top_cap * 4; break;
+    case 4: src = by_jobs ? jb.top_list + (size_t)band * jb.top_cap : nullptr; words = (uint64_t)jb.top_cap * 4; break;
+    case 5: src = by_jobs ? jb.cls_list + ((size_t)band * (LPT_CLASSES - 1u) + cls) * per : nullptr; words = (uint64_t)per * 4; break;
+    case 6: src = fs.out.tile_offsets; words = (uint64_t)fs.out.num_tiles * 2; break;
+    default: return BH_ERR_INVALID_ARG;
+    }
+    if (words > cap_words || words > 0x7FFFFFFFull) return set_error(ctx, BH_ERR_INVALID_ARG, "debug_bwd_jobs: output buffer too small");
+    if (what == 0) { memcpy(out, info, sizeof info); return (int)words; }
+    if (!src) return set_error(ctx, BH_ERR_STATE, "debug_bwd_jobs: the last forward filed no such list");
+    BH_HIP(ctx, hipSetDevice(ctx->device));
+    if (ctx->far_job.pending) BH_TRY(finish_far_slice(ctx, nullptr));
+    BH_HIP(ctx, hipMemcpyAsync(out, src, words * 4, hipMemcpyDeviceToHost, ctx->stream));
+    BH_HIP(ctx, hipStreamSynchronize(ctx->stream));
+    return (int)words;
+}
+extern "C" int bh_debug_set_ckpt_cap(bh_ctx* ctx, uint32_t cap) {
+    if (!ctx) return BH_ERR_INVALID_ARG;
+    ctx->debug_ckpt_cap = cap;
+    return 0;
 }
 extern "C" int bh_debug_fill_train_scratch(bh_ctx* ctx, uint32_t pattern) {
     if (!ctx) return BH_ERR_INVALID_ARG;
@@ -1487,17 +1531,29 @@
             started_tag = ctx->far_job.gate_tag;
             ctx->gate_signal_queued = true;
         }
+        FlattenJobs fj;
+        ForwardState& lf = ctx->latest;
+        if (ctx->knob_bwd_flat_jobs && lf.lpt && lf.jobs.ckpt && lf.jobs.flat && lf.out.num_intersections > 0) {
+            fj.counters = lf.lpt;
+            fj.per = band_slots(lf.uniforms.tile_bw * (lf.uniforms.tile_y1 - lf.uniforms.tile_y0));
+            fj.jobs = lf.jobs;
+        }
+        const FlattenJobs* flatten = fj.counters ? &fj : nullptr;
         if (tile_mode && batch->strip_loss) {
             const ViewUniforms wu = make_uniforms(batch->camera);
-            return launch_image_loss_fused_window(ctx, ro.out_img, batch->gt_packed, H, W, lc, alpha_match, dl_rgb, dl_alpha, wu.tile_y0, wu.tile_y1,
-                                                  loss_dev, v_output, loss_host, started_host, started_tag);
+            BH_TRY(launch_image_loss_fused_window(ctx, ro.out_img, batch->gt_packed, H, W, lc, alpha_match, dl_rgb, dl_alpha, wu.tile_y0, wu.tile_y1,
+                                                  loss_dev, v_output, loss_host, started_host, started_tag, flatten));
+            lf.flat_valid = flatten != nullptr;
+            return 0;
         }
         if (exposed) {
             ProfScope ps(ctx, "Exposure");
             BH_TRY(launch_exposure_apply(ctx, exposure, batch->view_id, ro.out_img, H, W, exposed));
         }
-        return launch_image_loss_fused(ctx, exposed ? exposed : ro.out_img, batch->gt_packed, H, W, lc, alpha_match, dl_rgb, dl_alpha, loss_dev, v_output, loss_host, started_host,
-                                       started_tag);
+        BH_TRY(launch_image_loss_fused(ctx, exposed ? exposed : ro.out_img, batch->gt_packed, H, W, lc, alpha_match, dl_rgb, dl_alpha, loss_dev, v_output, loss_host, started_host,
+                                       started_tag, flatten));
+        lf.flat_valid = flatten != nullptr;
+        return 0;
     };
 #ifdef BH_TEST_HOOKS
     if (ctx->knob_fail_loss_at && ++ctx->train_steps_seen == ctx->knob_fail_loss_at)
diff --git a/brush_amd/csrc/context.h b/brush_amd/csrc/context.h
--- a/brush_amd/csrc/context.h
+++ b/brush_amd/csrc/context.h
@@ -144,16 +144,66 @@
 constexpr uint32_t LPT_HEADER_WORDS = 8 * LPT_CLASSES + 64;
 constexpr uint32_t BWD_SEG = 128;
 constexpr uint32_t BWD_MAX_SEGS = 64;
+struct alignas(16) BwdJobRec {
+    uint32_t entry;
+    uint32_t lo, hi;
+    uint32_t slot;
+};
+constexpr uint32_t BWD_NO_CKPT = 0xFFFFFFFFu;
 struct BwdJobs {
     float4* ckpt = nullptr;
     uint32_t ckpt_cap = 0;
-    uint32_t* top_list = nullptr;
+    BwdJobRec* top_list = nullptr;
     uint32_t top_cap = 0;
+    BwdJobRec* cls_list = nullptr;
+    BwdJobRec* flat = nullptr;
+    uint32_t* flat_total = nullptr;
 };
 constexpr uint32_t BAND_CHUNK = 4;
 inline __host__ __device__ uint32_t band_slots(uint32_t num_tiles) {
     const uint32_t p = (num_tiles + 7u) / 8u;
     return ((p + BAND_CHUNK - 1u) / BAND_CHUNK) * BAND_CHUNK;
+}
+struct FlattenJobs {
+    const uint32_t* counters = nullptr;
+    uint32_t per = 0;
+    BwdJobs jobs{};
+};
+__device__ inline void flatten_jobs(const FlattenJobs& d, uint32_t band, uint32_t tid, uint32_t nthreads, uint32_t* s) {
+    uint32_t* s_cnt = s;
+    uint32_t* s_beg = s + LPT_CLASSES;
+    __syncthreads();
+    if (tid < LPT_CLASSES) s_cnt[tid] = min(d.counters[band * LPT_CLASSES + tid], tid == LPT_CLASSES - 1u ? d.jobs.top_cap : d.per);
+    __syncthreads();
+    if (tid < LPT_CLASSES) {
+        uint32_t b = 0;
+        for (uint32_t c = tid + 1u; c < LPT_CLASSES; ++c) b += s_cnt[c];
+        s_beg[tid] = b;
+    }
+    __syncthreads();
+    const uint32_t total = min(s_beg[0] + s_cnt[0], d.jobs.top_cap);
+    const uint4* top = reinterpret_cast<const uint4*>(d.jobs.top_list) + (size_t)band * d.jobs.top_cap;
+    const uint4* low = reinterpret_cast<const uint4*>(d.jobs.cls_list) + (size_t)band * (LPT_CLASSES - 1u) * d.per;
+    uint4* dst = reinterpret_cast<uint4*>(d.jobs.flat) + (size_t)band * d.jobs.top_cap;
+    auto fetch = [&](uint32_t i) {
+        uint32_t c = 0;
+#pragma unroll
+        for (uint32_t step = LPT_CLASSES / 2u; step; step >>= 1)
+            if (s_beg[c + step - 1u] > i) c += step;
+        const uint32_t k = i - s_beg[c];
+        return c == LPT_CLASSES - 1u ? top[k] : low[(size_t)c * d.per + k];
+    };
+    for (uint32_t i0 = tid; i0 < total; i0 += 4u * nthreads) {
+        uint4 r[4];
+#pragma unroll
+        for (uint32_t k = 0; k < 4u; ++k)
+            if (i0 + k * nthreads < total) r[k] = fetch(i0 + k * nthreads);
+#pragma unroll
+        for (uint32_t k = 0; k < 4u; ++k)
+            if (i0 + k * nthreads < total) dst[i0 + k * nthreads] = r[k];
+    }
+    if (tid == 0u) d.jobs.flat_total[band] = total;
+    __syncthreads();
 }
 inline __host__ __device__ uint32_t band_tile(uint32_t band, uint32_t i, uint32_t per, uint32_t mode) {
     return mode ? ((i / BAND_CHUNK) * 8u + band) * BAND_CHUNK + (i % BAND_CHUNK) : band * per + i;
@@ -272,6 +322,7 @@
     float bg[3] = {0, 0, 0};
     uint32_t* lpt = nullptr;
     BwdJobs jobs{};
+    bool flat_valid = false;
 };
 constexpr int RETAIN_SLOTS = 14;
 struct Retained {
@@ -364,6 +415,7 @@
     uint32_t knob_k16_split = 250;
     uint32_t knob_k16_split_min = bh::SPLIT_MIN_WORK;
     uint32_t knob_k16_split_of_max = 45;
+    uint32_t debug_ckpt_cap = 0;
     const uint32_t* last_split = nullptr;
     uint32_t knob_k16_order = 1;
     uint32_t knob_cut_margin_pct = 150;
@@ -381,6 +433,7 @@
     size_t lds_optin_max = 0;
     bool knob_no_lpt = false;
     bool knob_bwd_wide_rows = false;
+    bool knob_bwd_flat_jobs = true;
     bool knob_bwd_jobs = true;
     bool knob_lpt_linear = false;
     bool knob_force_exchange = false;
@@ -568,7 +621,8 @@
                               const uint32_t* isect_gids, const uint32_t* tile_offsets, const float* projected,
                               const float* out_img, const float* v_output, float* v_combined, const uint32_t* lpt,
                               const uint32_t* tile_offsets_far = nullptr, bool want_refine = true, const BwdJobs* jobs = nullptr,
-                              uint32_t accum_rows = 0u);
+                              uint32_t accum_rows = 0u,
+                              bool flat_jobs = false);
 int launch_image_loss_forward(bh_ctx* ctx, const float* pred, const uint32_t* gt, uint32_t channels, uint32_t h,
                               uint32_t w, const BhLossConfig& cfg, float* loss_map);
 int launch_image_loss_backward(bh_ctx* ctx, const float* pred, const uint32_t* gt, const float* dl_dmap,
diff --git a/brush_amd/csrc/loss_fused.hip b/brush_amd/csrc/loss_fused.hip
--- a/brush_amd/csrc/loss_fused.hip
+++ b/brush_amd/csrc/loss_fused.hip
@@ -65,6 +65,7 @@
     float* loss_host;
     uint32_t* started_host;
     uint32_t started_tag;
+    FlattenJobs flatten;
     uint32_t gx, gy_blocks, band_w;
 };
 
@@ -107,6 +108,11 @@
     float* s_red = s_h;
     if (a.started_host && blockIdx.x == 0 && blockIdx.y == 0 && threadIdx.x == 0 && threadIdx.y == 0)
         *reinterpret_cast<volatile uint32_t*>(a.started_host) = a.started_tag;
+    if (a.flatten.counters) {
+        const uint32_t nblk = gridDim.x * gridDim.y, blk = blockIdx.y * gridDim.x + blockIdx.x;
+        for (uint32_t band = blk; band < 8u; band += nblk)
+            flatten_jobs(a.flatten, band, threadIdx.y * TW + threadIdx.x, 256u, reinterpret_cast<uint32_t*>(s_h));
+    }
     uint32_t bx, by, blin;
     if (!loss_tile(a, bx, by, blin)) return;
     const int tx0 = (int)bx * TW, ty0 = (int)a.ty_base * LB + (int)by * TH;
@@ -446,7 +452,7 @@
 
 int launch_image_loss_fused_window(bh_ctx* ctx, const float* img_hwc4, const uint32_t* gt, uint32_t h, uint32_t w, const BhLossConfig& cfg,
                                    bool alpha_match, float dl_rgb, float dl_alpha, uint32_t tile_y0, uint32_t tile_y1, float* loss_out,
-                                   float* v_output, float* loss_host, uint32_t* started_host, uint32_t started_tag) {
+                                   float* v_output, float* loss_host, uint32_t* started_host, uint32_t started_tag, const FlattenJobs* flatten) {
     const uint32_t gx = (w + LB - 1) / LB, gy = (h + LB - 1) / LB;
     if (tile_y1 > gy) tile_y1 = gy;
     if (tile_y0 >= tile_y1) return set_error(ctx, BH_ERR_INVALID_ARG, "image loss: empty tile-row window");
@@ -476,6 +482,7 @@
         a.row_end = h;
         a.sum_src = nullptr; a.sum_n = 0; a.loss_out = nullptr; a.loss_host = nullptr;
         a.started_host = started_host; a.started_tag = started_tag;
+        a.flatten = flatten ? *flatten : FlattenJobs{};
         a.gx = gx; a.gy_blocks = (a1 - a0 + 1) / 2;
         a.band_w = banded ? (gx + 7u) / 8u : 0u;
         const dim3 grid_a = banded ? dim3(8u * a.band_w * a.gy_blocks) : dim3(gx, a.gy_blocks);
@@ -491,6 +498,7 @@
         a.loss_out = loss_out;
         a.loss_host = loss_host;
         a.started_host = nullptr; a.started_tag = 0;
+        a.flatten = FlattenJobs{};
         a.gy_blocks = (tile_y1 - tile_y0 + 1) / 2;
         const dim3 grid_b = banded ? dim3(8u * a.band_w * a.gy_blocks) : dim3(gx, a.gy_blocks);
         hipLaunchKernelGGL(loss_fused_backward_kernel, grid_b, block, 0, ctx->stream, img_hwc4, gt, partials, v_output, a);
@@ -501,9 +509,9 @@
 
 int launch_image_loss_fused(bh_ctx* ctx, const float* img_hwc4, const uint32_t* gt, uint32_t h, uint32_t w, const BhLossConfig& cfg,
                             bool alpha_match, float dl_rgb, float dl_alpha, float* loss_out, float* v_output, float* loss_host, uint32_t* started_host,
-                            uint32_t started_tag) {
+                            uint32_t started_tag, const FlattenJobs* flatten) {
     return launch_image_loss_fused_window(ctx, img_hwc4, gt, h, w, cfg, alpha_match, dl_rgb, dl_alpha, 0, (h + LB - 1) / LB, loss_out, v_output, loss_host,
-                                          started_host, started_tag);
-}
-
-}
+                                          started_host, started_tag, flatten);
+}
+
+}
diff --git a/brush_amd/csrc/rasterize.hip b/brush_amd/csrc/rasterize.hip
--- a/brush_amd/csrc/rasterize.hip
+++ b/brush_amd/csrc/rasterize.hip
@@ -92,6 +92,16 @@
 
 
 
+template <bool SMOOTH, bool HALF_CONIC, uint32_t GID_SCALE>
+BH_DEV void stage_row(const float (&v)[9], uint32_t cg, int lane, float* s_splat) {
+    const float cut = blend_sigma_cut<SMOOTH>(v[5]);
+    const uint32_t gate = (v[6] >= 0.0f ? 1u : 0u) | (v[7] >= 0.0f ? 2u : 0u) | (v[8] >= 0.0f ? 4u : 0u);
+    float4* d = reinterpret_cast<float4*>(s_splat + lane * SPLAT_STRIDE);
+    const float diag = HALF_CONIC ? 0.5f : 1.0f;
+    d[0] = make_float4(v[0], v[1], diag * v[2], v[3]);
+    d[1] = make_float4(diag * v[4], v[5], __builtin_fmaxf(v[6], 0.0f), __builtin_fmaxf(v[7], 0.0f));
+    d[2] = make_float4(__builtin_fmaxf(v[8], 0.0f), cut, u2f(gate), u2f(cg * GID_SCALE));
+}
 template <bool SMOOTH, bool HALF_CONIC, uint32_t GID_SCALE = 1u>
 BH_DEV uint32_t stage_batch(const uint32_t* __restrict__ isect_gids, const float* __restrict__ projected,
                             uint32_t batch_start, uint32_t cnt, int lane, float* s_splat) {
@@ -102,13 +112,7 @@
         float v[9];
 #pragma unroll
         for (int k = 0; k < 9; ++k) v[k] = p[k];
-        const float cut = blend_sigma_cut<SMOOTH>(v[5]);
-        const uint32_t gate = (v[6] >= 0.0f ? 1u : 0u) | (v[7] >= 0.0f ? 2u : 0u) | (v[8] >= 0.0f ? 4u : 0u);
-        float4* d = reinterpret_cast<float4*>(s_splat + lane * SPLAT_STRIDE);
-        const float diag = HALF_CONIC ? 0.5f : 1.0f;
-        d[0] = make_float4(v[0], v[1], diag * v[2], v[3]);
-        d[1] = make_float4(diag * v[4], v[5], __builtin_fmaxf(v[6], 0.0f), __builtin_fmaxf(v[7], 0.0f));
-        d[2] = make_float4(__builtin_fmaxf(v[8], 0.0f), cut, u2f(gate), u2f(cg * GID_SCALE));
+        stage_row<SMOOTH, HALF_CONIC, GID_SCALE>(v, cg, lane, s_splat);
     }
     return cg;
 }
@@ -473,8 +477,9 @@
             const uint32_t band = bidx & 7u;
             const uint32_t pos = atomicAdd(&lpt[band * LPT_CLASSES + cls], 1u);
             const uint32_t entry = local_tile | ((uint32_t)lane << JOB_SEG_SHIFT) | (last ? JOB_LAST_BIT : 0u);
-            if (cls == LPT_CLASSES - 1u) sl.jobs.top_list[(size_t)band * sl.jobs.top_cap + pos] = entry;
-            else lpt[lpt_list_offset(u.num_tiles, band, cls) + pos] = entry;
+            BwdJobRec* dst = cls == LPT_CLASSES - 1u ? sl.jobs.top_list + ((size_t)band * sl.jobs.top_cap + pos)
+                                                     : sl.jobs.cls_list + (((size_t)band * (LPT_CLASSES - 1u) + cls) * lpt_band_tiles(u.num_tiles) + pos);
+            *reinterpret_cast<uint4*>(dst) = make_uint4(entry, range_lo + lo, last ? last_useful : range_lo + lo + BWD_SEG, lane ? slot0 + (uint32_t)lane - 1u : BWD_NO_CKPT);
         }
     }
     if (lane == 0) {
@@ -628,19 +633,37 @@
 }
 
 constexpr int BWD_WAVES = 5;
-template <bool SMOOTH, bool REFINE, bool JOBS, bool WIDE>
+template <bool SMOOTH, bool REFINE, bool JOBS, bool WIDE, bool FLAT = false>
 __global__ __launch_bounds__(64, (BWD_WAVES - (SMOOTH ? 1 : 0) + (REFINE ? 0 : 1))) void rasterize_backward_kernel(RasterUniforms u, const uint32_t* __restrict__ isect_gids,
                                                                const uint32_t* __restrict__ tile_offsets,
                                                                const float* __restrict__ projected,
                                                                const float* __restrict__ out_img,
                                                                const float* __restrict__ v_output,
                                                                float* __restrict__ v_combined, const uint32_t* __restrict__ lpt,
-                                                               const uint32_t* __restrict__ tile_offsets_far, BwdJobs jb) {
+                                                               const uint32_t* __restrict__ tile_offsets_far, BwdJobs jb,
+                                                               const BwdJobRec* __restrict__ flat, const uint32_t* __restrict__ flat_total) {
+    static_assert(JOBS || !FLAT, "the flat list holds jobs");
     __shared__ __attribute__((aligned(16))) float s_splat[BATCH * SPLAT_STRIDE];
+    uint32_t flat_n = 0u;
+    uint4 next_rec = make_uint4(0u, 0u, 0u, 0u);
+    const uint4* flat_band = nullptr;
+    if (FLAT) {
+        flat_band = reinterpret_cast<const uint4*>(flat) + (size_t)(blockIdx.x & 7u) * jb.top_cap;
+        flat_n = flat_total[blockIdx.x & 7u];
+        next_rec = flat_band[min(blockIdx.x >> 3, jb.top_cap - 1u)];
+    }
   for (uint32_t jidx = blockIdx.x >> 3;; jidx += gridDim.x >> 3) {
     uint32_t local_tile, seg = 0u;
     bool to_end = true;
-    if (lpt) {
+    uint32_t rec_lo = 0u, rec_hi = 0u, rec_slot = 0u;
+    if (FLAT) {
+        if (jidx >= flat_n) return;
+        const uint4 rec = next_rec;
+        next_rec = flat_band[min(jidx + (gridDim.x >> 3), jb.top_cap - 1u)];
+        local_tile = rec.x & JOB_TILE_MASK;
+        seg = (rec.x >> JOB_SEG_SHIFT) & JOB_SEG_MASK;
+        rec_lo = rec.y; rec_hi = rec.z; rec_slot = rec.w;
+    } else if (lpt) {
         const uint32_t xcd = blockIdx.x & 7u;
         uint32_t j = jidx;
         const uint32_t* cnt = lpt + xcd * LPT_CLASSES;
@@ -660,7 +683,9 @@
             }
         }
         if (!found) return;
-        const uint32_t entry = (JOBS && cls == LPT_CLASSES - 1u) ? jb.top_list[(size_t)xcd * jb.top_cap + j] : lpt[lpt_list_offset(u.num_tiles, xcd, cls) + j];
+        const uint32_t entry = !JOBS ? lpt[lpt_list_offset(u.num_tiles, xcd, cls) + j]
+                               : cls == LPT_CLASSES - 1u ? jb.top_list[(size_t)xcd * jb.top_cap + j].entry
+                                                         : jb.cls_list[((size_t)xcd * (LPT_CLASSES - 1u) + cls) * lpt_band_tiles(u.num_tiles) + j].entry;
         local_tile = entry & JOB_TILE_MASK;
         if (JOBS) { seg = (entry >> JOB_SEG_SHIFT) & JOB_SEG_MASK; to_end = (entry & JOB_LAST_BIT) != 0u; }
     } else {
@@ -668,11 +693,13 @@
         if (local_tile >= u.num_tiles) return;
     }
     const uint32_t tile = u.tile_begin + local_tile;
-    uint32_t seg_lo0 = tile_offsets[tile * 2], seg_hi0 = tile_offsets[tile * 2 + 1];
+    uint32_t seg_lo0 = FLAT ? rec_lo : tile_offsets[tile * 2], seg_hi0 = FLAT ? rec_hi : tile_offsets[tile * 2 + 1];
     const uint32_t list_lo = seg_lo0;
     uint32_t seg_lo1 = 0, seg_hi1 = 0;
     if (!JOBS && tile_offsets_far) { seg_lo1 = tile_offsets_far[tile * 2]; seg_hi1 = tile_offsets_far[tile * 2 + 1]; }
-    if (JOBS) {
+    if (FLAT) {
+        if (seg_hi0 <= seg_lo0) continue;
+    } else if (JOBS) {
         seg_lo0 += seg * BWD_SEG;
         if (!to_end) seg_hi0 = seg_lo0 + BWD_SEG;
         if (seg_hi0 <= seg_lo0) continue;
@@ -687,6 +714,9 @@
     float sS[4], sw[4];
     float vox[4], voy[4], voz[4], w2q[4], h2q[4];
     float4 o4[4], vo4[4];
+    const uint32_t cnt0 = FLAT ? min((uint32_t)BATCH, seg_hi0 - seg_lo0) : 0u;
+    uint32_t cg0 = 0u;
+    if (FLAT && (uint32_t)lane < cnt0) cg0 = isect_gids[seg_lo0 + (uint32_t)lane];
 #pragma unroll
     for (int q = 0; q < 4; ++q) {
         const uint32_t px = px0 + 8 * (q & 1), py = py0 + 8 * (q >> 1);
@@ -694,6 +724,15 @@
         const size_t pix = ((size_t)pxc + (size_t)pyc * u.img_w) * 4;
         o4[q] = *reinterpret_cast<const float4*>(&out_img[pix]);
         vo4[q] = *reinterpret_cast<const float4*>(&v_output[pix]);
+    }
+    float4 c4f[4] = {};
+    if (FLAT) {
+        if (seg != 0u) {
+            const float4* ck = jb.ckpt + (size_t)rec_slot * 256u + (uint32_t)lane;
+#pragma unroll
+            for (int q = 0; q < 4; ++q) c4f[q] = ck[q * 64];
+        }
+        asm volatile("" ::: "memory");
     }
 #pragma unroll
     for (int q = 0; q < 4; ++q) {
@@ -718,8 +757,12 @@
             vox[q] = voy[q] = voz[q] = 0.0f;
             w2q[q] = h2q[q] = 0.0f;
         }
-    }
-    if (JOBS && seg != 0u) {
+        if (FLAT && seg != 0u) {
+            sS[q] -= __builtin_fmaf(c4f[q].z, voz[q], __builtin_fmaf(c4f[q].y, voy[q], c4f[q].x * vox[q]));
+            sw[q] = (sw[q] != 0.0f && c4f[q].w > 0.0f) ? c4f[q].w : 0.0f;
+        }
+    }
+    if (JOBS && !FLAT && seg != 0u) {
         const float4* ck = jb.ckpt + (size_t)ckpt_slot(list_lo, tile, seg) * 256u + (uint32_t)lane;
         float4 c4[4];
 #pragma unroll
@@ -822,10 +865,25 @@
 #pragma nounroll
     for (int part = 0; part < (JOBS ? 1 : 2); ++part) {
         const uint32_t range_lo = part ? seg_lo1 : seg_lo0, range_hi = part ? seg_hi1 : seg_hi0;
+        bool staged = false;
+        if (FLAT) {
+            __syncthreads();
+            if ((uint32_t)lane < cnt0) {
+                const float* p = projected + (size_t)cg0 * 9;
+                float row0[9];
+#pragma unroll
+                for (int k = 0; k < 9; ++k) row0[k] = p[k];
+                stage_row<SMOOTH, true, WIDE ? 1u : 40u>(row0, cg0, lane, s_splat);
+            }
+            staged = true;
+        }
         for (uint32_t batch_start = range_lo; batch_start < range_hi; batch_start += BATCH) {
             const uint32_t cnt = min((uint32_t)BATCH, range_hi - batch_start);
-            __syncthreads();
-            stage_batch<SMOOTH, true, WIDE ? 1u : 40u>(isect_gids, projected, batch_start, cnt, lane, s_splat);
+            if (!staged) {
+                __syncthreads();
+                stage_batch<SMOOTH, true, WIDE ? 1u : 40u>(isect_gids, projected, batch_start, cnt, lane, s_splat);
+            }
+            staged = false;
             __syncthreads();
             const bool mine_clamps = (uint32_t)lane < cnt && s_splat[lane * SPLAT_STRIDE + 5] > 0.999f;
             if (__ballot(mine_clamps) != 0ull) run_batch(std::true_type{}, cnt);
@@ -836,21 +894,21 @@
   }
 }
 
-template <bool SMOOTH, bool REFINE, bool JOBS, bool WIDE>
+template <bool SMOOTH, bool REFINE, bool JOBS, bool WIDE, bool FLAT>
 static void launch_rasterize_backward_t(hipStream_t stream, dim3 grid, hipEvent_t ea, hipEvent_t eb, const RasterUniforms& u, const uint32_t* isect_gids,
                                         const uint32_t* tile_offsets, const float* projected, const float* out_img, const float* v_output, float* v_combined,
                                         const uint32_t* lpt, const uint32_t* tile_offsets_far, const BwdJobs& jb) {
     const dim3 block(64);
     if (ea)
-        hipExtLaunchKernelGGL((rasterize_backward_kernel<SMOOTH, REFINE, JOBS, WIDE>), grid, block, 0, stream, ea, eb, 0, u, isect_gids, tile_offsets, projected, out_img, v_output, v_combined, lpt, tile_offsets_far, jb);
+        hipExtLaunchKernelGGL((rasterize_backward_kernel<SMOOTH, REFINE, JOBS, WIDE, FLAT>), grid, block, 0, stream, ea, eb, 0, u, isect_gids, tile_offsets, projected, out_img, v_output, v_combined, lpt, tile_offsets_far, jb, jb.flat, jb.flat_total);
     else
-        hipLaunchKernelGGL((rasterize_backward_kernel<SMOOTH, REFINE, JOBS, WIDE>), grid, block, 0, stream, u, isect_gids, tile_offsets, projected, out_img, v_output, v_combined, lpt, tile_offsets_far, jb);
+        hipLaunchKernelGGL((rasterize_backward_kernel<SMOOTH, REFINE, JOBS, WIDE, FLAT>), grid, block, 0, stream, u, isect_gids, tile_offsets, projected, out_img, v_output, v_combined, lpt, tile_offsets_far, jb, jb.flat, jb.flat_total);
 }
 
 int launch_rasterize_backward(bh_ctx* ctx, const ViewUniforms& vu, const float bg[3], bool smooth,
                               const uint32_t* isect_gids, const uint32_t* tile_offsets, const float* projected,
                               const float* out_img, const float* v_output, float* v_combined, const uint32_t* lpt,
-                              const uint32_t* tile_offsets_far, bool want_refine, const BwdJobs* jobs, uint32_t accum_rows) {
+                              const uint32_t* tile_offsets_far, bool want_refine, const BwdJobs* jobs, uint32_t accum_rows, bool flat_jobs) {
     RasterUniforms u;
     u.band_mode = ctx->knob_band_mode;
     u.rcp_class_width = 1.0f;
@@ -863,12 +921,14 @@
     const bool by_jobs = jobs && jobs->ckpt && lpt;
     const BwdJobs jb = by_jobs ? *jobs : BwdJobs{};
     const uint32_t per = band_slots(u.num_tiles);
+    const bool flat = by_jobs && flat_jobs && !smooth && jb.flat && jb.flat_total;
     const uint32_t nblocks = (by_jobs ? 2u : 1u) * per * 8u;
     const dim3 grid(nblocks);
     const bool wide = ctx->knob_bwd_wide_rows || accum_rows == 0u || (uint64_t)accum_rows * 40ull > (1ull << 32);
     hipEvent_t ea = ctx->prof.ext_a, eb = ctx->prof.ext_b;
     ctx->prof.ext_a = ctx->prof.ext_b = nullptr;
-#define BH_K17_W(S, R, J, W) launch_rasterize_backward_t<S, R, J, W>(ctx->stream, grid, ea, eb, u, isect_gids, tile_offsets, projected, out_img, v_output, v_combined, lpt, tile_offsets_far, jb)
+#define BH_K17_F(S, R, J, W, F) launch_rasterize_backward_t<S, R, J, W, F>(ctx->stream, grid, ea, eb, u, isect_gids, tile_offsets, projected, out_img, v_output, v_combined, lpt, tile_offsets_far, jb)
+#define BH_K17_W(S, R, J, W) do { if (J && !S && flat) BH_K17_F(S, R, J, W, (J && !S)); else BH_K17_F(S, R, J, W, false); } while (0)
 #define BH_K17(S, R, J) do { if (wide) BH_K17_W(S, R, J, true); else BH_K17_W(S, R, J, false); } while (0)
     if (by_jobs) {
         if (smooth && want_refine) BH_K17(true, true, true);
@@ -883,6 +943,7 @@
     }
 #undef BH_K17
 #undef BH_K17_W
+#undef BH_K17_F
     BH_LAUNCH_CHECK(ctx, "rasterize_backward_kernel");
     return 0;
 }
```

After: 1326 (median of 6 runs). No clear change (+0.3%).
